# zju3dv/clean-pvnet

Hardware: AMD Instinct MI355X
Metric: images/sec RANSAC-vote (480x640, K=9, 512 hyp) (higher is better)
Workload: dtype f32; 1 GPU; BASELINE config 3 (cfg3): 480x640, K=9, 512 hypotheses, ~2% foreground, int64 mask, contiguous [B,H,W,K,2] f32 vertex; global batch 64 in contiguous shards of 64 images per GPU; ransac_voting_layer_v3 (+ one RCCL all_gather of [B,K,2] per step for N>1, see extra.exchange); steps cycle over 3 distinct device-resident batches; batch_per_gpu=64, global_batch=64, H=480, W=640, K=9, hn=512, parallelism=batch-sharded x1 (strong scaling: 64 images in total)

## Files before the change

### clean-pvnet_amd/csrc/compaction.hpp

```cpp
#pragma once

struct MaskArgs {
    const void *mask;
    const float *selection;
    int64_t sb, sh, sw;
    int es;
    int contig;
    int mode;
    int W, HW, T;
    int min_num, max_num, cap;
    uint64_t seed;
    int b0;
    int *tn_user;
    int *status;
    int fuse_sub;
    int want_draws;
    const float *seg;
    long long *mask_out;
    int64_t gb, gc, gh, gw;
    int C;
};

constexpr uint32_t kTileNzMask = 0xfffu;

enum { kElemF32 = 0, kElemF16 = 1, kElemBF16 = 2 };
template <int ET> struct Elem;
template <> struct Elem<kElemF32> { typedef float raw; };
template <> struct Elem<kElemF16> { typedef _Float16 raw; };
template <> struct Elem<kElemBF16> { typedef uint16_t raw; };

__device__ __forceinline__ float widen(float v) { return v; }
__device__ __forceinline__ float widen(_Float16 v) { return (float)v; }
__device__ __forceinline__ float widen(uint16_t v) { return __builtin_bit_cast(float, (uint32_t)v << 16); }

template <int ET>
__device__ __forceinline__ float2 widen_pair(uint32_t w)
{
    static_assert(ET != kElemF32, "2-byte elements only");
    if constexpr (ET == kElemF16)
        return make_float2((float)__builtin_bit_cast(_Float16, (uint16_t)w), (float)__builtin_bit_cast(_Float16, (uint16_t)(w >> 16)));
    else
        return make_float2(__builtin_bit_cast(float, w << 16), __builtin_bit_cast(float, w & 0xffff0000u));
}

template <int ES>
__device__ __forceinline__ uint64_t load_elem(const void *base, int64_t off)
{
    if (ES == 1) return ((const uint8_t *)base)[off];
    if (ES == 2) return ((const uint16_t *)base)[off];
    if (ES == 4) return ((const uint32_t *)base)[off];
    return ((const uint64_t *)base)[off];
}

template <int ST>
__device__ __forceinline__ int argmax_class(const MaskArgs &a, int b, int p)
{
    typedef typename Elem<ST>::raw raw_t;
    const int y = p / a.W;
    const int x = p - y * a.W;
    const raw_t *q = (const raw_t *)a.seg + (int64_t)b * a.gb + (int64_t)y * a.gh + (int64_t)x * a.gw;
    float best = widen(q[0]);
    int idx = 0;
    for (int c = 1; c < a.C; ++c) {
        const float v = widen(q[(int64_t)c * a.gc]);
        if (v > best || (v != v && best == best)) { best = v; idx = c; }
    }
    return idx;
}

template <int ES, int ST>
__device__ __forceinline__ int mask_weight(const MaskArgs &a, int b, int p)
{
    if (a.seg) {
        const int idx = argmax_class<ST>(a, b, p);
        if (a.mask_out) a.mask_out[(int64_t)b * a.HW + p] = idx;
        return a.mode == 0 ? (idx & 0xFF) : (idx == 1 ? 1 : 0);
    }
    int64_t off;
    if (a.contig) {
        off = (int64_t)b * a.sb + p;
    } else {
        int y = p / a.W;
        int x = p - y * a.W;
        off = (int64_t)b * a.sb + (int64_t)y * a.sh + (int64_t)x * a.sw;
    }
    uint64_t v = load_elem<ES>(a.mask, off);
    if (a.mode == 0) return (int)(v & 0xFF);
    return v == 1 ? 1 : 0;
}

__device__ __forceinline__ float selection_draw(const MaskArgs &a, int b, int p)
{
    if (a.selection) return a.selection[(int64_t)b * a.HW + p];
    return (float)(rng_u32(a.seed, 0u, (uint32_t)(a.b0 + b), (uint32_t)p) >> 8) * 0x1p-24f;
}

__device__ __forceinline__ float list_draw(const MaskArgs &a, int b, int i, int e, const unsigned short *__restrict__ lists ,
                                           const float *__restrict__ draws )
{
    if (draws) return draws[(size_t)i * kTile + e];
    return selection_draw(a, b, i * kTile + (int)lists[(size_t)i * kTile + e]);
}

__device__ __forceinline__ void scan_segments(int *seg)
{
    __syncthreads();
    if (threadIdx.x < 64) {
        const int lane = threadIdx.x;
        const int c = lane < kTileSteps * 4 ? seg[lane] : 0;
        const int inc = wave_incl_scan(c);
        if (lane < kTileSteps * 4) seg[lane] = inc - c;
        if (lane == kTileSteps * 4 - 1) seg[kTileSteps * 4] = inc;
    }
    __syncthreads();
}

template <int ES> struct RawElem;
template <> struct RawElem<1> { typedef uint8_t type; };
template <> struct RawElem<2> { typedef uint16_t type; };
template <> struct RawElem<4> { typedef uint32_t type; };
template <> struct RawElem<8> { typedef uint64_t type; };

template <int ES, bool AHEAD, int MODE , int ST = kElemF32 >
__global__ __launch_bounds__(kBlock) void k_tile_scan(MaskArgs a, uint32_t *__restrict__ tiles,
                                                      unsigned short *__restrict__ tile_list,
                                                      float *__restrict__ tile_draw, int total_tiles)
{
    typedef typename RawElem<ES>::type raw_t;
    __shared__ int seg2[2][kTileSteps * 4 + 1];
    __shared__ int red2[2][4];
    const int lane = lane_id(), wave = threadIdx.x >> 6;
    raw_t cur[AHEAD ? kTileSteps : 1] = {};
    int g = blockIdx.x;
    int b = g / a.T, t = g - b * a.T;
    const int step_b = (int)gridDim.x / a.T, step_t = (int)gridDim.x - step_b * a.T;
    [[maybe_unused]] auto load_tile = [&](raw_t (&dst)[AHEAD ? kTileSteps : 1], int bi, int ti) {
        const raw_t *src = (const raw_t *)a.mask + (int64_t)bi * a.sb + (int64_t)ti * kTile + threadIdx.x;
        if ((ti + 1) * kTile <= a.HW) {
#pragma unroll
            for (int s = 0; s < kTileSteps; ++s) dst[AHEAD ? s : 0] = src[s * kBlock];
        } else {
#pragma unroll
            for (int s = 0; s < kTileSteps; ++s)
                dst[AHEAD ? s : 0] = ti * kTile + s * kBlock + (int)threadIdx.x < a.HW ? src[s * kBlock] : (raw_t)0;
        }
    };
    if constexpr (AHEAD) if (g < total_tiles) load_tile(cur, b, t);
    for (int it = 0; g < total_tiles; ++it) {
        int *seg = seg2[it & 1], *red = red2[it & 1];
        raw_t nxt[AHEAD ? kTileSteps : 1] = {};
        const int gn = g + gridDim.x;
        int bn = b + step_b, tn = t + step_t;
        if (tn >= a.T) { tn -= a.T; ++bn; }
        if constexpr (AHEAD) if (gn < total_tiles) load_tile(nxt, bn, tn);
        unsigned long long m[kTileSteps];
        int pc[kTileSteps];
        int sum = 0;
#pragma unroll
        for (int s = 0; s < kTileSteps; ++s) {
            const int p = t * kTile + s * kBlock + threadIdx.x;
            int w = 0;
            if constexpr (AHEAD) {
                const uint64_t v = (uint64_t)cur[s];
                w = MODE == 0 ? (int)(v & 0xFF) : (v == 1 ? 1 : 0);
            } else if (p < a.HW) {
                w = mask_weight<ES, ST>(a, b, p);
            }
            m[s] = __ballot(w != 0);
            pc[s] = __popcll(m[s]);
            sum += w;
        }
        if (MODE == 0) sum = wave_total(sum);
        else sum = pc[0] + pc[1] + pc[2] + pc[3] + pc[4] + pc[5] + pc[6] + pc[7];
        if (lane == 0) {
#pragma unroll
            for (int s = 0; s < kTileSteps; ++s) seg[s * 4 + wave] = pc[s];
            red[wave] = sum;
        }
        scan_segments(seg);
        if (threadIdx.x == 0)
            tiles[b * a.T + t] = (uint32_t)seg[kTileSteps * 4] | ((uint32_t)(red[0] + red[1] + red[2] + red[3]) << 12);
        unsigned short *list = tile_list + ((size_t)b * a.T + t) * kTile;
        float *draw = tile_draw + ((size_t)b * a.T + t) * kTile;
        if (seg[kTileSteps * 4] != 0) {
#pragma unroll
            for (int s = 0; s < kTileSteps; ++s)
                if ((m[s] >> lane) & 1ull) {
                    const int r = seg[s * 4 + wave] + __popcll(m[s] & ((1ull << lane) - 1ull));
                    list[r] = (unsigned short)(s * kBlock + threadIdx.x);
                    if (a.want_draws) draw[r] = selection_draw(a, b, t * kTile + s * kBlock + threadIdx.x);
                }
        }
        if constexpr (AHEAD) {
#pragma unroll
            for (int s = 0; s < kTileSteps; ++s) cur[s] = nxt[s];
        }
        g = gn; b = bn; t = tn;
    }
}

typedef float f32x4 __attribute__((ext_vector_type(4)));
typedef long long i64x2 __attribute__((ext_vector_type(2)));
typedef uint32_t u32x2 __attribute__((ext_vector_type(2)));

template <int ST>
__device__ __forceinline__ f32x4 widen_logits4(u32x2 w)
{
    const float2 lo = widen_pair<ST>(w.x), hi = widen_pair<ST>(w.y);
    return f32x4{lo.x, lo.y, hi.x, hi.y};
}

template <bool WRITE_MASK, int ST = kElemF32>
__global__ __launch_bounds__(kBlock) void k_tile_scan_seg2(MaskArgs a, uint32_t *__restrict__ tiles,
                                                           unsigned short *__restrict__ tile_list,
                                                           float *__restrict__ tile_draw)
{
    typedef typename Elem<ST>::raw raw_t;
    __shared__ int seg[8];
    const int g = blockIdx.x;
    const int b = g / a.T, t = g - b * a.T;
    const int lane = lane_id(), wave = threadIdx.x >> 6;
    const raw_t *p0 = (const raw_t *)a.seg + (int64_t)b * a.gb + (int64_t)t * kTile + 4 * threadIdx.x;
    const raw_t *p1 = p0 + a.gc;
    constexpr int kHalf = kTile / 2;
    f32x4 v0[2], v1[2];
    if constexpr (ST == kElemF32) {
#pragma unroll
        for (int s = 0; s < 2; ++s) {
            const bool in = t * kTile + s * kHalf + 4 * (int)threadIdx.x < a.HW;
            v0[s] = in ? __builtin_nontemporal_load((const f32x4 *)(p0 + s * kHalf)) : f32x4{0.f, 0.f, 0.f, 0.f};
            v1[s] = in ? __builtin_nontemporal_load((const f32x4 *)(p1 + s * kHalf)) : f32x4{0.f, 0.f, 0.f, 0.f};
        }
    } else {
        u32x2 w0[2], w1[2];
#pragma unroll
        for (int s = 0; s < 2; ++s) {
            const bool in = t * kTile + s * kHalf + 4 * (int)threadIdx.x < a.HW;
            w0[s] = in ? __builtin_nontemporal_load((const u32x2 *)(p0 + s * kHalf)) : u32x2{0u, 0u};
            w1[s] = in ? __builtin_nontemporal_load((const u32x2 *)(p1 + s * kHalf)) : u32x2{0u, 0u};
        }
#pragma unroll
        for (int s = 0; s < 2; ++s) {
            v0[s] = widen_logits4<ST>(w0[s]);
            v1[s] = widen_logits4<ST>(w1[s]);
        }
    }
    unsigned m4[2];
    int excl[2];
#pragma unroll
    for (int s = 0; s < 2; ++s) {
        unsigned m = 0u;
#pragma unroll
        for (int j = 0; j < 4; ++j) {
            const float x0 = v0[s][j], x1 = v1[s][j];
            m |= ((x1 > x0) || (x1 != x1 && x0 == x0)) ? (1u << j) : 0u;
        }
        m4[s] = m;
        const int c = __popc(m);
        const int inc = wave_incl_scan(c);
        excl[s] = inc - c;
        if (lane == 63) seg[s * 4 + wave] = inc;
    }
    __syncthreads();
    int cnt[8];
#pragma unroll
    for (int i = 0; i < 8; ++i) cnt[i] = seg[i];
    int nz = 0, base[2] = {0, 0};
#pragma unroll
    for (int i = 0; i < 8; ++i) {
        if (i < wave) base[0] += cnt[i];
        if (i < 4 + wave) base[1] += cnt[i];
        nz += cnt[i];
    }
    if (threadIdx.x == 0) tiles[g] = (uint32_t)nz | ((uint32_t)nz << 12);
    if (WRITE_MASK && a.mask_out) {
        long long *mo = a.mask_out + (int64_t)b * a.HW + (int64_t)t * kTile + 4 * threadIdx.x;
#pragma unroll
        for (int s = 0; s < 2; ++s)
            if (t * kTile + s * kHalf + 4 * (int)threadIdx.x < a.HW) {
                __builtin_nontemporal_store(i64x2{(long long)(m4[s] & 1u), (long long)((m4[s] >> 1) & 1u)}, (i64x2 *)(mo + s * kHalf));
                __builtin_nontemporal_store(i64x2{(long long)((m4[s] >> 2) & 1u), (long long)((m4[s] >> 3) & 1u)}, (i64x2 *)(mo + s * kHalf + 2));
            }
    }
    if (nz == 0) return;
    unsigned short *list = tile_list + (size_t)g * kTile;
    float *draw = tile_draw + (size_t)g * kTile;
#pragma unroll
    for (int s = 0; s < 2; ++s) {
        int r = base[s] + excl[s];
#pragma unroll
        for (int j = 0; j < 4; ++j)
            if ((m4[s] >> j) & 1u) {
                const int off = s * kHalf + 4 * (int)threadIdx.x + j;
                list[r] = (unsigned short)off;
                if (a.want_draws) draw[r] = selection_draw(a, b, t * kTile + off);
                ++r;
            }
    }
}

__global__ __launch_bounds__(kBlock) void k_mask_from_lists(const uint32_t *__restrict__ tiles, const unsigned short *__restrict__ tile_list,
                                                            long long *__restrict__ mask_out, int T, int HW, int total_tiles)
{
    __shared__ unsigned bm[kTile / 32];
    uint32_t word = (int)blockIdx.x < total_tiles ? tiles[blockIdx.x] : 0u;
    for (int g = blockIdx.x; g < total_tiles; g += gridDim.x) {
        const int b = g / T, t = g - b * T;
        const int nz = (int)(word & kTileNzMask);
        if (g + (int)gridDim.x < total_tiles) word = tiles[g + gridDim.x];
        if (nz) {
            __syncthreads();
            if (threadIdx.x < kTile / 32) bm[threadIdx.x] = 0u;
            __syncthreads();
            const unsigned short *list = tile_list + (size_t)g * kTile;
            for (int e = threadIdx.x; e < nz; e += kBlock) {
                const unsigned off = list[e];
                atomicOr(&bm[off >> 5], 1u << (off & 31u));
            }
            __syncthreads();
        }
        long long *dst = mask_out + (int64_t)b * HW + (int64_t)t * kTile;
#pragma unroll
        for (int j = 0; j < kTile / (2 * kBlock); ++j) {
            const int px = (j * kBlock + (int)threadIdx.x) * 2;
            if (t * kTile + px >= HW) break;
            const unsigned w = nz ? bm[px >> 5] >> (px & 31) : 0u;
#ifdef PVV_MASK_PLAIN_STORE
            *(i64x2 *)(dst + px) = i64x2{(long long)(w & 1u), (long long)((w >> 1) & 1u)};
#else
            __builtin_nontemporal_store(i64x2{(long long)(w & 1u), (long long)((w >> 1) & 1u)}, (i64x2 *)(dst + px));
#endif
        }
    }
}

struct ImageTotals { long long fg; int total; int before; };

__device__ __forceinline__ ImageTotals image_totals(const uint32_t *__restrict__ tiles, int b, int T, int t,
                                                    long long *redl, int *red)
{
    long long fgs = 0;
    int before = 0, total = 0;
    for (int i = threadIdx.x; i < T; i += kBlock) {
        const uint32_t w = tiles[b * T + i];
        fgs += w >> 12;
        const int c = (int)(w & kTileNzMask);
        total += c;
        if (i < t) before += c;
    }
    fgs = wave_total(fgs);
    before = wave_total(before);
    total = wave_total(total);
    const int wave = threadIdx.x >> 6;
    __syncthreads();
    if (lane_id() == 0) { redl[wave] = fgs; red[wave] = before; red[4 + wave] = total; }
    __syncthreads();
    ImageTotals r;
    r.fg = redl[0] + redl[1] + redl[2] + redl[3];
    r.before = red[0] + red[1] + red[2] + red[3];
    r.total = red[4] + red[5] + red[6] + red[7];
    return r;
}

__device__ __forceinline__ int filter_tile_list(const MaskArgs &a, int b, int t, int nz, float prob,
                                                const unsigned short *__restrict__ img_lists, const float *__restrict__ img_draws ,
                                                unsigned short *out, int *seg)
{
    const int lane = lane_id(), wave = threadIdx.x >> 6;
    const unsigned short *list = img_lists + (size_t)t * kTile;
    unsigned long long m[kTileSteps];
    unsigned short off[kTileSteps];
#pragma unroll
    for (int s = 0; s < kTileSteps; ++s) {
        const int e = s * kBlock + threadIdx.x;
        bool f = false;
        off[s] = 0;
        if (e < nz) {
            off[s] = list[e];
            f = (img_draws ? img_draws[(size_t)t * kTile + e] : selection_draw(a, b, t * kTile + (int)off[s])) < prob;
        }
        m[s] = __ballot(f);
        if (lane == 0) seg[s * 4 + wave] = __popcll(m[s]);
    }
    scan_segments(seg);
#pragma unroll
    for (int s = 0; s < kTileSteps; ++s)
        if ((m[s] >> lane) & 1ull) out[seg[s * 4 + wave] + __popcll(m[s] & ((1ull << lane) - 1ull))] = off[s];
    return seg[kTileSteps * 4];
}

__global__ __launch_bounds__(kBlock) void k_tile_subsample(MaskArgs a, uint32_t *__restrict__ tiles,
                                                           unsigned short *__restrict__ tile_list,
                                                           const float *__restrict__ tile_draw)
{
    __shared__ long long redl[4];
    __shared__ int red[8];
    __shared__ int seg[kTileSteps * 4 + 1];
    __shared__ unsigned short keep[kTile];
    const int t = blockIdx.x, b = blockIdx.y;
    const uint32_t w = tiles[b * a.T + t];
    const int nz = (int)(w & kTileNzMask);
    if (nz == 0) return;
    const ImageTotals tot = image_totals(tiles, b, a.T, t, redl, red);
    if (tot.fg <= (long long)a.max_num) return;
    const float prob = (float)a.max_num / (float)tot.fg;
    unsigned short *list = tile_list + ((size_t)b * a.T + t) * kTile;
    const int n = filter_tile_list(a, b, t, nz, prob, tile_list + (size_t)b * a.T * kTile, tile_draw + (size_t)b * a.T * kTile, keep, seg);
    __syncthreads();
    for (int i = threadIdx.x; i < n; i += kBlock) list[i] = keep[i];
    if (threadIdx.x == 0) tiles[b * a.T + t] = (uint32_t)n | (w & ~kTileNzMask);
}

struct VertexArgs {
    const float *vertex;
    int64_t sb, sh, sw, sk, sc;
    int K;
    int vec2;
};

template <int VT> struct VertexRaw { typedef uint2 type; };
template <> struct VertexRaw<kElemF32> { typedef float2 type; };

template <int VT>
__device__ __forceinline__ typename VertexRaw<VT>::type load_vertex(const VertexArgs &v, int b, int y, int x, int vi)
{
    if constexpr (VT == kElemF32) {
        const float *src = v.vertex + (int64_t)b * v.sb + (int64_t)y * v.sh + (int64_t)x * v.sw + (int64_t)vi * v.sk;
        if (v.vec2) return *(const float2 *)src;
        return make_float2(src[0], src[v.sc]);
    } else {
        const uint16_t *src = (const uint16_t *)v.vertex + (int64_t)b * v.sb + (int64_t)y * v.sh + (int64_t)x * v.sw + (int64_t)vi * v.sk;
        if (v.vec2) return make_uint2(*(const uint32_t *)src, 0u);
        return make_uint2(src[0], src[v.sc]);
    }
}

template <int VT>
__device__ __forceinline__ float2 widen_vertex(const VertexArgs &v, typename VertexRaw<VT>::type r)
{
    if constexpr (VT == kElemF32) {
        return r;
    } else {
        typedef typename Elem<VT>::raw raw_t;
        if (v.vec2) return widen_pair<VT>(r.x);
        return make_float2(widen(__builtin_bit_cast(raw_t, (uint16_t)r.x)), widen(__builtin_bit_cast(raw_t, (uint16_t)r.y)));
    }
}

struct HypArgs {
    const int32_t *idxs;
    const int32_t *idxs2;
    int hn, hn_first;
    uint32_t stream, stream2;
    float2 *hyps;
    int *counts;
    int32_t *draws_out;
    int blocks;
    int *surv;
    int *lead;
    int *miss;
};

constexpr int kHypRejectTries = 1 << 12;
constexpr float kSurvMinProb = 1.f / 64.f;
constexpr int kSurvCap = 8192;

__device__ __forceinline__ int select_pixel(const int *prefix, int T, const unsigned short *__restrict__ lists , int t,
                                            size_t *entry = nullptr )
{
    int lo = 0, hi = T - 1;
    while (lo < hi) {
        const int mid = (lo + hi) >> 1;
        if (prefix[mid] > t) hi = mid; else lo = mid + 1;
    }
    const int r = t - (lo ? prefix[lo - 1] : 0);
    const size_t e = (size_t)lo * kTile + r;
    if (entry) *entry = e;
    return lo * kTile + (int)lists[e];
}

template <int VT>
__global__ __launch_bounds__(kBlock) void k_compact_hyp(MaskArgs a, VertexArgs v, HypArgs h,
                                                        const uint32_t *__restrict__ tiles,
                                                        const unsigned short *__restrict__ tile_list,
                                                        const float *__restrict__ tile_draw,
                                                        int *__restrict__ tn_out, float2 *__restrict__ coords,
                                                        float2 *__restrict__ dirs)
{
    extern __shared__ int s_prefix[];
    __shared__ long long redl[4];
    __shared__ int red[8];
    __shared__ int seg[kTileSteps * 4 + 1];
    __shared__ unsigned short list[kTile];
    const int b = blockIdx.y;
    const int lane = lane_id(), wave = threadIdx.x >> 6;
    const unsigned short *img_lists = tile_list + (size_t)b * a.T * kTile;
    const float *img_draws = a.want_draws ? tile_draw + (size_t)b * a.T * kTile : nullptr;

    if ((int)blockIdx.x < h.blocks) {
        const int j = blockIdx.x;
        long long fgs = 0;
        int carry = 0;
        for (int base = 0; base < a.T; base += kBlock) {
            const int i = base + threadIdx.x;
            const uint32_t w = i < a.T ? tiles[b * a.T + i] : 0u;
            fgs += w >> 12;
            const int inc = wave_incl_scan((int)(w & kTileNzMask));
            __syncthreads();
            if (lane == 63) red[wave] = inc;
            __syncthreads();
            int off = carry;
            for (int w2 = 0; w2 < wave; ++w2) off += red[w2];
            if (i < a.T) s_prefix[i] = inc + off;
            carry += red[0] + red[1] + red[2] + red[3];
        }
        fgs = wave_total(fgs);
        __syncthreads();
        if (lane == 0) redl[wave] = fgs;
        __syncthreads();
        const long long fg = redl[0] + redl[1] + redl[2] + redl[3];
        const int total = carry;
        int tn = total < a.cap ? total : a.cap;
        if (fg < (long long)a.min_num) tn = 0;
        const bool sub = a.fuse_sub && fg > (long long)a.max_num;
        const float prob = sub ? (float)a.max_num / (float)fg : 2.f;
        int nsurv = -1;
        if (sub && prob < kSurvMinProb) {
            int *sv = h.surv + (size_t)b * kSurvCap;
            nsurv = 0;
            for (int i = 0; i < a.T; ++i) {
                const int ni = s_prefix[i] - (i ? s_prefix[i - 1] : 0);
                for (int e0 = 0; e0 < ni; e0 += kBlock) {
                    const int e = e0 + threadIdx.x;
                    const bool keep = e < ni && list_draw(a, b, i, e, img_lists, img_draws) < prob;
                    const unsigned long long m = __ballot(keep);
                    __syncthreads();
                    if (lane == 0) red[wave] = __popcll(m);
                    __syncthreads();
                    int off = nsurv;
                    for (int w2 = 0; w2 < wave; ++w2) off += red[w2];
                    off += __popcll(m & ((1ull << lane) - 1ull));
                    if (keep && off < kSurvCap) sv[off] = i * kTile + (int)img_lists[(size_t)i * kTile + e];
                    nsurv += red[0] + red[1] + red[2] + red[3];
                }
            }
            __threadfence_block();
            __syncthreads();
            if (nsurv > kSurvCap) nsurv = -1;
            else if (nsurv < tn) tn = nsurv;
        }

        const int gid = j * kBlock + threadIdx.x;
        if (gid >= v.K * h.hn) return;
        const int vi = gid / h.hn, hi = gid - vi * h.hn;
        const size_t o = ((size_t)b * v.K + vi) * h.hn + hi;
        h.counts[o] = 0;
        if (h.miss) h.miss[o] = 0;
        if (h.lead && hi == 0) {
            int *lw = h.lead + ((size_t)b * v.K + vi) * 8 + 4;
            lw[0] = 0; lw[1] = 0; lw[2] = 0; lw[3] = 0;
        }
        if (tn <= 0) {
            h.hyps[o] = make_float2(0.f, 0.f);
            if (h.draws_out) { h.draws_out[2 * o] = -1; h.draws_out[2 * o + 1] = -1; }
            return;
        }
        const bool first = hi < h.hn_first;
        const int32_t *src = first ? h.idxs : h.idxs2;
        int p0, p1;
        if (src) {
            const int32_t *ip = first ? h.idxs + (((size_t)b * h.hn_first + hi) * v.K + vi) * 2
                                      : h.idxs2 + (((size_t)b * (h.hn - h.hn_first) + (hi - h.hn_first)) * v.K + vi) * 2;
            int t0 = ip[0], t1 = ip[1];
            t0 = t0 < 0 ? 0 : (t0 >= tn ? tn - 1 : t0);
            t1 = t1 < 0 ? 0 : (t1 >= tn ? tn - 1 : t1);
            p0 = select_pixel(s_prefix, a.T, img_lists, t0);
            p1 = select_pixel(s_prefix, a.T, img_lists, t1);
        } else {
            const uint32_t stream = first ? h.stream : h.stream2;
            const uint32_t c = (uint32_t)((first ? hi : hi - h.hn_first) * v.K + vi) * 2u;
            const uint32_t img = (uint32_t)(a.b0 + b);
            if (!sub) {
                p0 = select_pixel(s_prefix, a.T, img_lists, (int)(rng_u32(a.seed, stream, img, c) % (uint32_t)tn));
                p1 = select_pixel(s_prefix, a.T, img_lists, (int)(rng_u32(a.seed, stream, img, c + 1u) % (uint32_t)tn));
            } else if (nsurv >= 0) {
                const int *sv = h.surv + (size_t)b * kSurvCap;
                p0 = sv[rng_u32(a.seed, stream, img, c) % (uint32_t)tn];
                p1 = sv[rng_u32(a.seed, stream, img, c + 1u) % (uint32_t)tn];
            } else {
                p0 = p1 = -1;
                for (int tr = 0; tr < kHypRejectTries && (p0 < 0 || p1 < 0); ++tr) {
                    size_t e;
                    const uint32_t stry = stream + 16u + 4u * (uint32_t)tr;
                    if (p0 < 0) {
                        const int p = select_pixel(s_prefix, a.T, img_lists, (int)(rng_u32(a.seed, stry, img, c) % (uint32_t)total), &e);
                        if ((img_draws ? img_draws[e] : selection_draw(a, b, p)) < prob) p0 = p;
                    }
                    if (p1 < 0) {
                        const int p = select_pixel(s_prefix, a.T, img_lists, (int)(rng_u32(a.seed, stry, img, c + 1u) % (uint32_t)total), &e);
                        if ((img_draws ? img_draws[e] : selection_draw(a, b, p)) < prob) p1 = p;
                    }
                }
                if (p0 < 0 || p1 < 0) {
                    h.hyps[o] = make_float2(0.f, 0.f);
                    if (h.draws_out) { h.draws_out[2 * o] = p0; h.draws_out[2 * o + 1] = p1; }
                    return;
                }
            }
        }
        const int y0 = p0 / a.W, x0 = p0 - y0 * a.W, y1 = p1 / a.W, x1 = p1 - y1 * a.W;
        const typename VertexRaw<VT>::type r0 = load_vertex<VT>(v, b, y0, x0, vi), r1 = load_vertex<VT>(v, b, y1, x1, vi);
        const float2 d0 = widen_vertex<VT>(v, r0), d1 = widen_vertex<VT>(v, r1);
        h.hyps[o] = hypothesis_exact(d0.x, d0.y, (float)x0, (float)y0, d1.x, d1.y, (float)x1, (float)y1);
        if (h.draws_out) { h.draws_out[2 * o] = p0; h.draws_out[2 * o + 1] = p1; }
        return;
    }

    const int t = blockIdx.x - h.blocks;
    const int nz = (int)(tiles[b * a.T + t] & kTileNzMask);
    if (t != 0 && !(a.fuse_sub && t == a.T - 1) && nz == 0) return;
    const unsigned short *my_list = img_lists + (size_t)t * kTile;
    unsigned short mine[kTileSteps];
#pragma unroll
    for (int s = 0; s < kTileSteps; ++s) {
        const int e = s * kBlock + threadIdx.x;
        mine[s] = e < nz ? my_list[e] : (unsigned short)0;
    }
    const ImageTotals tot = image_totals(tiles, b, a.T, t, redl, red);
    if (tot.fg < (long long)a.min_num) {
        if (t == 0 && threadIdx.x == 0) {
            tn_out[b] = 0;
            if (a.tn_user) a.tn_user[b] = 0;
            if (a.status) a.status[b] = PVV_STATUS_SKIPPED;
        }
        return;
    }
    int before = tot.before, tile_n = nz;
    const bool sub = a.fuse_sub && tot.fg > (long long)a.max_num;
    if (sub) {
        const float prob = (float)a.max_num / (float)tot.fg;
        int cnt = 0;
        if (img_draws || a.T > kBlock) {
            for (int i = 0; i < t; ++i) {
                const int ni = (int)(tiles[b * a.T + i] & kTileNzMask);
                for (int e = threadIdx.x; e < ni; e += kBlock)
                    cnt += list_draw(a, b, i, e, img_lists, img_draws) < prob ? 1 : 0;
            }
        } else {
            const int ti = threadIdx.x;
            const int nzi = ti < t ? (int)(tiles[b * a.T + ti] & kTileNzMask) : 0;
            const int inc = wave_incl_scan((nzi + 7) >> 3);
            __syncthreads();
            if (lane == 63) red[wave] = inc;
            __syncthreads();
            int goff = 0;
            for (int w2 = 0; w2 < wave; ++w2) goff += red[w2];
            if (ti < a.T) s_prefix[ti] = inc + goff;
            list[ti] = (unsigned short)nzi;
            __syncthreads();
            const int groups = t ? s_prefix[t - 1] : 0;
            constexpr int kAhead = 4;
            int tile = 0;
            for (int g0 = threadIdx.x; g0 < groups; g0 += kAhead * kBlock) {
                uint4 ent[kAhead];
                int left[kAhead], pix0[kAhead];
#pragma unroll
                for (int u = 0; u < kAhead; ++u) {
                    const int g = g0 + u * kBlock;
                    left[u] = 0;
                    if (g < groups) {
                        while (s_prefix[tile] <= g) ++tile;
                        const int e0 = (g - (tile ? s_prefix[tile - 1] : 0)) * 8;
                        ent[u] = *(const uint4 *)(img_lists + (size_t)tile * kTile + e0);
                        left[u] = (int)list[tile] - e0;
                        pix0[u] = tile * kTile;
                    }
                }
#pragma unroll
                for (int u = 0; u < kAhead; ++u) {
                    const uint32_t wds[4] = {ent[u].x, ent[u].y, ent[u].z, ent[u].w};
#pragma unroll
                    for (int q = 0; q < 8; ++q)
                        if (q < left[u]) {
                            const int off = (int)((wds[q >> 1] >> (16 * (q & 1))) & 0xffffu);
                            cnt += selection_draw(a, b, pix0[u] + off) < prob ? 1 : 0;
                        }
                }
            }
        }
        before = block_sum(cnt, red);
        __syncthreads();
        tile_n = filter_tile_list(a, b, t, nz, prob, img_lists, img_draws, list, seg);
        __syncthreads();
        if (t == a.T - 1 && threadIdx.x == 0) {
            const int all = before + tile_n;
            tn_out[b] = all < a.cap ? all : a.cap;
            if (a.tn_user) a.tn_user[b] = tn_out[b];
            if (a.status) a.status[b] = PVV_STATUS_SUBSAMPLED | (all > a.cap ? PVV_STATUS_TRUNCATED : 0);
        }
    } else {
        if (t == 0 && threadIdx.x == 0) {
            tn_out[b] = tot.total < a.cap ? tot.total : a.cap;
            if (a.tn_user) a.tn_user[b] = tn_out[b];
            if (a.status) a.status[b] = (tot.fg > (long long)a.max_num ? PVV_STATUS_SUBSAMPLED : 0) |
                                        (tot.total > a.cap ? PVV_STATUS_TRUNCATED : 0);
        }
#pragma unroll
        for (int s = 0; s < kTileSteps; ++s) {
            const int e = s * kBlock + threadIdx.x;
            if (e < nz) list[e] = mine[s];
        }
        __syncthreads();
    }
    const int room = a.cap - before;
    const int n = tile_n < room ? tile_n : (room > 0 ? room : 0);
    constexpr int kKeys = 12;
    for (int li = threadIdx.x; li < n; li += kBlock) {
        const int p = t * kTile + list[li];
        const int y = p / a.W, x = p - y * a.W;
        coords[(size_t)b * a.cap + before + li] = make_float2((float)x, (float)y);
        float2 *drow = dirs + (size_t)b * v.K * a.cap + before + li;
        for (int v0 = 0; v0 < v.K; v0 += kKeys) {
            typename VertexRaw<VT>::type d[kKeys];
#pragma unroll
            for (int u = 0; u < kKeys; ++u)
                if (v0 + u < v.K) d[u] = load_vertex<VT>(v, b, y, x, v0 + u);
#pragma unroll
            for (int u = 0; u < kKeys; ++u)
                if (v0 + u < v.K) {
                    if constexpr (VT == kElemF32) drow[(size_t)(v0 + u) * a.cap] = d[u];
                    else drow[(size_t)(v0 + u) * a.cap] = widen_vertex<VT>(v, d[u]);
                }
        }
    }
}
```

### clean-pvnet_amd/csrc/count_bf16.hpp

```cpp
#pragma once

typedef __bf16 bf16x8 __attribute__((ext_vector_type(8)));
typedef float float16v __attribute__((ext_vector_type(16)));

#define kDdAlive __uint_as_float(0x2b8cbcceu)
constexpr int kBfPixPerWave = 128;
constexpr int kBfMaxHt = 16;

struct Bf16Consts {
    float beta;
    float eps_c;
    float eps0;
    float kappa;
    float beta2;
};

__device__ __forceinline__ void split3(float x, __bf16 (&p)[3])
{
    p[0] = (__bf16)x;
    float r = x - (float)p[0];
    p[1] = (__bf16)r;
    r = r - (float)p[1];
    p[2] = (__bf16)r;
}

__device__ __forceinline__ int stage_hypothesis(bf16x8 *sB, int *sCnt, int i, float2 hp, float2 org, int cnt_init = 0)
{
    __bf16 qx[3], qy[3];
    split3(hp.x - org.x, qx);
    split3(hp.y - org.y, qy);
    const __bf16 one = (__bf16)1.f, zero = (__bf16)0.f;
    const bf16x8 lo8 = {qx[0], qy[0], qx[1], qx[2], qx[0], qy[1], qy[2], qy[0]};
    const bf16x8 hi8 = {qx[0], qy[0], qx[1], qy[1], one, one, one, zero};
    sB[(i >> 5) * 64 + (i & 31)] = lo8;
    sB[(i >> 5) * 64 + 32 + (i & 31)] = hi8;
    sCnt[i] = cnt_init;
    return !(fabsf(hp.x) < 1e15f && fabsf(hp.y) < 1e15f);
}

#ifdef PVV_STAMPS
#define PVV_STAMP(i) do { if (dbg && threadIdx.x == 0 && (blockIdx.x == 0 || blockIdx.x == 97 || blockIdx.x == 401)) \
    dbg[((blockIdx.x == 0 ? 0 : (blockIdx.x == 97 ? 1 : 2)) * 16) + (i)] = wall_clock64(); } while (0)
enum { kCsTable = 0, kCsItemPrologue, kCsAOperands, kCsNextGroup, kCsLoop, kCsLoopWait, kCsFlush, kCsOther, kCensusPhases };
#define PVV_CENSUS_IN() long long cs_last = 0; __shared__ long long s_cs[16]; \
    do { if (threadIdx.x == 0) { for (int i_ = 0; i_ < 16; ++i_) s_cs[i_] = 0; s_cs[0] = wall_clock64(); \
    s_cs[2] = (long long)__builtin_amdgcn_s_getreg(63492) | ((long long)__builtin_amdgcn_s_getreg(63508) << 32); \
    cs_last = (long long)__builtin_readcyclecounter(); } } while (0)
#define PVV_CS(i) do { if (threadIdx.x == 0) { const long long t_ = (long long)__builtin_readcyclecounter(); s_cs[4 + (i)] += t_ - cs_last; cs_last = t_; } } while (0)
#define PVV_CS_RT_IN() long long cs_rt = 0; do { if (threadIdx.x == 0) cs_rt = wall_clock64(); } while (0)
#define PVV_CS_RT_OUT(tiles) do { if (threadIdx.x == 0) { s_cs[12] += wall_clock64() - cs_rt; s_cs[13] += (tiles); } } while (0)
#define PVV_CENSUS_OUT(n) do { if (dbg && threadIdx.x == 0) { s_cs[1] = wall_clock64(); s_cs[3] = (n); \
    for (int i_ = 0; i_ < 16; ++i_) dbg[64 + 16 * (size_t)blockIdx.x + i_] = s_cs[i_]; } } while (0)
#else
#define PVV_STAMP(i) do { } while (0)
#define PVV_CENSUS_IN() do { } while (0)
#define PVV_CS(i) do { } while (0)
#define PVV_CS_RT_IN() do { } while (0)
#define PVV_CS_RT_OUT(tiles) do { } while (0)
#define PVV_CENSUS_OUT(n) do { } while (0)
#endif

enum { kCountFull = 0, kCountFirst = 1, kCountFilter = 2 };

#ifndef PVV_STAGE_M
#define PVV_STAGE_M 8
#define PVV_STAGE_FIRST 0x22u
#endif
constexpr int kStageM = PVV_STAGE_M;
constexpr uint32_t kStageFirst = PVV_STAGE_FIRST;
constexpr uint32_t kStageFirstEighth = 0x02u;
constexpr uint32_t stage_rest_of(uint32_t first) { return ((1u << kStageM) - 1u) & ~first; }
constexpr int kStageMinChunks = 8;

struct StageArgs {
    const int *lead;
    int *any_staged;
    int *miss;
    int sub_tenth;
    const float2 *mean;
    int hstride;
#ifdef PVV_STAMPS
    long long *dbg;
#endif
};

__device__ __forceinline__ int stage_bound(int lstar, int tn, int sub_tenth)
{
    if (sub_tenth && lstar >= 0) lstar -= (tn + 9) / 10 + 2 + (tn >> 20);
    return lstar;
}

template <uint32_t MASK>
__device__ __forceinline__ int stage_chunks(int n)
{
    return (n / kStageM) * __builtin_popcount(MASK) + __popc(MASK & ((1u << (n % kStageM)) - 1u));
}
template <uint32_t MASK>
__device__ __forceinline__ int stage_chunk_at(int j)
{
    constexpr int m = __builtin_popcount(MASK);
    const int per = j / m;
    uint32_t t = MASK;
    for (int k = j - per * m; k > 0; --k) t &= t - 1u;
    return per * kStageM + __builtin_ctz(t);
}
template <uint32_t MASK>
__device__ __forceinline__ int stage_pixels(int tn, int nch, int PC)
{
    return stage_chunks<MASK>(nch) * PC - (((MASK >> ((nch - 1) % kStageM)) & 1u) ? nch * PC - tn : 0);
}

template <int MODE, uint32_t FIRST = kStageFirst>
__global__ __launch_bounds__(kBlock) __attribute__((amdgpu_waves_per_eu(5, 5))) void k_count_bf16(
    const float2 *__restrict__ coords , const float2 *__restrict__ dirs ,
    const float2 *__restrict__ hyps , int *__restrict__ counts ,
    const int *__restrict__ tn_arr, int B, int K, int hn, int cap, float thresh, Bf16Consts fc, int target_items,
    long long *__restrict__ dbg , StageArgs sa)
{
    PVV_STAMP(0);
    PVV_CENSUS_IN();
    int n_items_done = 0;
    __shared__ int chunk_end[kMaxBatchLds];
    __shared__ int s_htpi, s_gpi, s_chunks;
    __shared__ bf16x8 sB[kBfMaxHt * 64];
    __shared__ float4 sP[4 * kBfPixPerWave];
    __shared__ int sCnt[kBfMaxHt * 32];
    __shared__ float sRed[4];
    __shared__ unsigned long long s_small[kMaxBatchLds / 64];
    __shared__ int s_keep[8];
    constexpr bool STAGED = MODE != kCountFull;
    constexpr bool FILTER = MODE == kCountFilter;
    constexpr uint32_t REST = stage_rest_of(FIRST);
    const int lane = lane_id(), wave = wave_id();
    constexpr int PC = 4 * kBfPixPerWave;
    const int nt = (hn + 31) >> 5;
    const int hs = sa.hstride > 0 ? sa.hstride : hn;
    if constexpr (FILTER) if (*sa.any_staged == 0) return;

    if (wave == 0) {
        int carry = 0;
        [[maybe_unused]] bool any_staged = false;
        for (int b0 = 0; b0 < B; b0 += 64) {
            const int b = b0 + lane;
            int inc = b < B ? (tn_arr[b] + PC - 1) / PC : 0;
            if constexpr (STAGED) {
                const bool small = inc < kStageMinChunks;
                const unsigned long long sm = __ballot(small);
                any_staged |= sm != ~0ull;
                if (lane == 0) s_small[b0 >> 6] = sm;
                inc = small ? (MODE == kCountFirst ? inc : 0) : stage_chunks<MODE == kCountFirst ? FIRST : REST>(inc);
            }
            inc = wave_incl_scan(inc) + carry;
            if (b < B) chunk_end[b] = inc;
            carry = __builtin_amdgcn_readlane(inc, 63);
        }
        const long long chunks = (long long)carry * K;
        int htpi = min(nt, kBfMaxHt);
        int nhg = (nt + htpi - 1) / htpi;
        int gpi = nhg;
#ifndef PVV_GPI_FACTOR
#define PVV_GPI_FACTOR 3
#endif
        const long long gpi_target = (B > 8 && nhg >= 4) ? (long long)PVV_GPI_FACTOR * target_items : (long long)target_items;
        while (gpi > 1 && chunks * ((nhg + gpi - 1) / gpi) < gpi_target) gpi = (gpi + 1) >> 1;
        const int htpi_min = chunks < 128 ? 2 : 4;
        if (gpi == 1 && !FILTER)
            while (htpi > htpi_min && chunks * ((nt + htpi - 1) / htpi) < target_items) htpi = (htpi + 1) >> 1;
        if (lane == 0) { s_htpi = htpi; s_gpi = gpi; s_chunks = carry; }
        if constexpr (MODE == kCountFirst) if (blockIdx.x == 0 && lane == 0) *sa.any_staged = any_staged ? 1 : 0;
    }
    __syncthreads();
    PVV_STAMP(1);
    const int htpi = __builtin_amdgcn_readfirstlane(s_htpi);
    const int gpi = __builtin_amdgcn_readfirstlane(s_gpi);
    const int nhg = (nt + htpi - 1) / htpi;
    const int nruns = (nhg + gpi - 1) / gpi;
    const int per_chunk = K * nruns;
    const int total = __builtin_amdgcn_readfirstlane(s_chunks) * per_chunk;
    const int col = lane & 31, kslice = lane >> 5;
    PVV_STAMP(2);
    PVV_CS(kCsTable);

    const int nblk = (total <= target_items + (target_items >> 1) + (target_items >> 2) && (int)gridDim.x > target_items &&
                      (int)gridDim.x <= 3 * target_items) ? target_items : (int)gridDim.x;
    if ((int)blockIdx.x >= nblk) return;
    const int step_q = nblk / per_chunk, step_r = nblk - step_q * per_chunk;
    int gchunk = (int)blockIdx.x / per_chunk, rem = (int)blockIdx.x - gchunk * per_chunk;
    for (int item = blockIdx.x; item < total;
         item += nblk, gchunk += step_q + (rem + step_r >= per_chunk ? 1 : 0), rem += step_r - (rem + step_r >= per_chunk ? per_chunk : 0)) {
        int local;
        const int b = locate_item(chunk_end, B, gchunk, &local);
        int chunk = local;
        if constexpr (STAGED)
            if (!((s_small[b >> 6] >> (b & 63)) & 1ull)) chunk = stage_chunk_at<MODE == kCountFirst ? FIRST : REST>(local);
        const int vi = nruns == 1 ? rem : rem / nruns;
        const int run = rem - vi * nruns;
        const int bk = b * K + vi;
        const float2 *hyp_k = hyps + (size_t)bk * hs;
        const float2 *crd = coords + (size_t)b * cap;
        const float2 *dir_k = dirs + (size_t)bk * cap;
        const int pb = chunk * PC;
        const int g0 = run * gpi, g1 = min(nhg, g0 + gpi);

        __syncthreads();
        int tid = threadIdx.x;
        asm volatile("" : "+v"(tid));
        PVV_STAMP(3);
        PVV_CS(kCsOther);
        ++n_items_done;
        const int tn_v = tn_arr[b];
        int lead_p = -1, lead_r = 0;
        if constexpr (FILTER) {
            lead_p = sa.lead[(size_t)bk * 8 + (lane & 3)];
            lead_r = sa.lead[(size_t)bk * 8 + 4 + (lane & 3)];
        }
        const float2 org = crd[pb];
        float2 pc[2], pd[2];
#pragma unroll
        for (int q = 0; q < 2; ++q) {
            const int p = min(pb + tid + q * kBlock, cap - 1);
            pc[q] = crd[p];
            pd[q] = dir_k[p];
        }
        const int nht0 = min(nt, (g0 + 1) * htpi) - g0 * htpi;
        float2 hp0[2];
#pragma unroll
        for (int q = 0; q < 2; ++q) {
            const int i = tid + q * kBlock;
            const int h = (g0 * htpi + (i >> 5)) * 32 + (i & 31);
            hp0[q] = (i < nht0 * 32 && h < hn) ? hyp_k[h] : make_float2(0.f, 0.f);
        }
        int cnt0[2] = {0, 0};
        if constexpr (FILTER) {
#pragma unroll
            for (int q = 0; q < 2; ++q) {
                const int i = tid + q * kBlock;
                const int h = g0 * htpi * 32 + i;
                if (i < nht0 * 32 && h < hn) cnt0[q] = counts[(size_t)bk * hs + h];
            }
        }
        const int tn = __builtin_amdgcn_readfirstlane(tn_v);
        int R_rem = 0, lstar = 0, ns_g = 0;
        if constexpr (FILTER) {
            R_rem = stage_pixels<REST>(tn, (tn + PC - 1) / PC, PC);
            int full = lead_p >= 0 ? lead_p + lead_r : -1;
            full = max(full, PVV_DPP(full, full, 0xB1, 0xf, false));
            full = max(full, PVV_DPP(full, full, 0x4E, 0xf, false));
            lstar = stage_bound(__builtin_amdgcn_readfirstlane(full), tn, sa.sub_tenth);
        }
        auto stage_kept = [&](int g, const int (&cnt)[2], const float2 (&hp)[2]) -> int {
            bool keep[2];
            unsigned long long m[2];
#pragma unroll
            for (int q = 0; q < 2; ++q) {
                const int i = tid + q * kBlock;
                keep[q] = i < htpi * 32 && g * htpi * 32 + i < hn && cnt[q] + R_rem >= lstar;
                m[q] = __ballot(keep[q]);
                if (lane == 0) s_keep[q * 4 + wave] = __popcll(m[q]);
            }
            __syncthreads();
            int tot = 0, base[2] = {0, 0};
#pragma unroll
            for (int j = 0; j < 8; ++j) {
                const int v = s_keep[j];
                tot += v;
                if (j < wave) base[0] += v;
                if (j < 4 + wave) base[1] += v;
            }
            int f = 0;
#pragma unroll
            for (int q = 0; q < 2; ++q)
                if (keep[q])
                    f |= stage_hypothesis(sB, sCnt, base[q] + (int)__builtin_amdgcn_mbcnt_hi((unsigned)(m[q] >> 32), __builtin_amdgcn_mbcnt_lo((unsigned)m[q], 0u)), hp[q], org,
                                          (int)(tid + q * kBlock) << 16);
            const int pad = ((tot + 31) & ~31) - tot;
            if (tid < pad) stage_hypothesis(sB, sCnt, tot + tid, make_float2(0.f, 0.f), org, 0);
            ns_g = tot;
            return f;
        };

        float c1 = 0.f;
#pragma unroll
        for (int q = 0; q < 2; ++q) {
            const int pl = tid + q * kBlock, p = pb + pl;
            float4 rec = make_float4(__builtin_nanf(""), 0.f, 0.f, 0.f);
            if (p < tn) {
                const float2 c = pc[q], d = pd[q];
                const float cx = c.x - org.x, cy = c.y - org.y;
                c1 = fmaxf(c1, fabsf(cx) + fabsf(cy));
                const float dd = d.x * d.x + d.y * d.y;
                if (dd >= kDdAlive && dd < INFINITY) {
                    const float rinv = __builtin_amdgcn_rsqf(dd);
                    rec = make_float4(d.x * rinv, d.y * rinv, cx, cy);
                }
            }
            sP[pl] = rec;
        }
        c1 = wave_max(c1);
        if (lane == 0) sRed[wave] = c1;
        int far = 0;
        if constexpr (FILTER) {
            far = stage_kept(g0, cnt0, hp0);
        } else {
#pragma unroll
            for (int q = 0; q < 2; ++q) {
                const int i = tid + q * kBlock;
                if (i < nht0 * 32) far |= stage_hypothesis(sB, sCnt, i, hp0[q], org);
            }
        }
        far = __syncthreads_or(far);
        PVV_STAMP(4);
        PVV_CS(kCsItemPrologue);
        const float C1 = fmaxf(fmaxf(sRed[0], sRed[1]), fmaxf(sRed[2], sRed[3]));
        const float eps = fc.eps0 + fc.eps_c * C1;
        const float epsw = __builtin_fmaf(fc.beta * 1.02f, C1, eps);

        const int ntile_c = (min(tn - pb, PC) + 15) >> 4;
        const int ntile_w = (ntile_c - wave + 3) >> 2;

        bf16x8 A[8];
        if (ntile_w > 0) {
            const int form = (lane >> 4) & 1, prow = lane & 15;
#pragma unroll
            for (int i = 0; i < 4; ++i) {
                const int j = kslice * 4 + i;
                const float4 rec = sP[(j * 4 + wave) * 16 + prow];
                const bool dead = rec.x != rec.x;
                float rx = form ? -fc.kappa * rec.y : rec.x;
                float ry = form ? fc.kappa * rec.x : rec.y;
                float rz = -(rec.z * rx + rec.w * ry);
                if (dead) { rx = 0.f; ry = 0.f; rz = form ? 0.f : -1e30f; }
                __bf16 vx[3], vy[3], cv[3];
                split3(rx, vx);
                split3(ry, vy);
                split3(rz, cv);
                const __bf16 zero = (__bf16)0.f;
                const bf16x8 lo8 = {vx[0], vy[0], vx[0], vx[0], vx[1], vy[0], vy[0], vy[1]};
                const bf16x8 hi8 = {vx[2], vy[2], vx[1], vy[1], cv[0], cv[1], cv[2], zero};
                uint4 x = __builtin_bit_cast(uint4, lo8), y = __builtin_bit_cast(uint4, hi8);
                {
                    const auto r0 = __builtin_amdgcn_permlane32_swap(x.x, y.x, false, false);
                    const auto r1 = __builtin_amdgcn_permlane32_swap(x.y, y.y, false, false);
                    const auto r2 = __builtin_amdgcn_permlane32_swap(x.z, y.z, false, false);
                    const auto r3 = __builtin_amdgcn_permlane32_swap(x.w, y.w, false, false);
                    x = make_uint4(r0[0], r1[0], r2[0], r3[0]);
                    y = make_uint4(r0[1], r1[1], r2[1], r3[1]);
                }
                A[i] = __builtin_bit_cast(bf16x8, x);
                A[4 + i] = __builtin_bit_cast(bf16x8, y);
            }
        }
        PVV_STAMP(5);
        PVV_CS(kCsAOperands);
        const int ebase = kslice * 4;
        const float16v zero16 = {0.f, 0.f, 0.f, 0.f, 0.f, 0.f, 0.f, 0.f, 0.f, 0.f, 0.f, 0.f, 0.f, 0.f, 0.f, 0.f};

        for (int g = g0; g < g1; ++g) {
            const int ht0 = g * htpi;
            if (g > g0) {
                far = 0;
                if constexpr (FILTER) {
                    int cnt[2] = {0, 0};
                    float2 hp[2] = {make_float2(0.f, 0.f), make_float2(0.f, 0.f)};
#pragma unroll
                    for (int q = 0; q < 2; ++q) {
                        const int i = threadIdx.x + q * kBlock;
                        const int h = ht0 * 32 + i;
                        if (i < htpi * 32 && h < hn) { cnt[q] = counts[(size_t)bk * hs + h]; hp[q] = hyp_k[h]; }
                    }
                    far = stage_kept(g, cnt, hp);
                } else {
                    const int nhtg = min(nt, ht0 + htpi) - ht0;
                    for (int i = threadIdx.x; i < nhtg * 32; i += kBlock) {
                        const int h = (ht0 + (i >> 5)) * 32 + (i & 31);
                        far |= stage_hypothesis(sB, sCnt, i, h < hn ? hyp_k[h] : make_float2(0.f, 0.f), org);
                    }
                }
                far = __syncthreads_or(far);
            }
            const int nht = FILTER ? (ns_g + 31) >> 5 : min(nt, ht0 + htpi) - ht0;
            const int nslot = FILTER ? ns_g : min(hn - ht0 * 32, nht * 32);
            PVV_STAMP(6);
            PVV_CS(kCsNextGroup);
            PVV_CS_RT_IN();

            if (__builtin_expect(far, 0)) {
                for (int ht = 0; ht < nht; ++ht) {
                    const int slot = ht * 32 + col;
                    if (slot >= nslot) continue;
                    const float2 hp = hyp_k[ht0 * 32 + (FILTER ? sCnt[slot] >> 16 : slot)];
                    int inl = 0;
                    for (int p = pb + wave * 2 + kslice; p < min(tn, pb + PC); p += 8) {
                        const float2 c = crd[p], d = dir_k[p];
                        inl += vote_exact(c.x, c.y, hp.x, hp.y, d.x, d.y, thresh) ? 1 : 0;
                    }
                    if (inl) atomicAdd(&sCnt[ht * 32 + col], inl);
                }
            } else if (ntile_w > 0) {
                for (int ht = 0; ht < nht; ++ht) {
                    const bf16x8 Bop = sB[ht * 64 + lane];
                    unsigned flagged = 0u;
                    const unsigned q01 = __builtin_bit_cast(uint4, Bop).x;
                    const float wband = __builtin_fmaf(fc.beta * 1.02f,
                                                       fabsf(__uint_as_float(q01 << 16)) + fabsf(__uint_as_float(q01 & 0xffff0000u)),
                                                       epsw);
                    unsigned qs[2] = {0u, 0u};
                    unsigned mb[2] = {0u, 0u};
                    int ntw = ntile_w;
                    asm volatile("" : "+s"(ntw));
#pragma unroll
                    for (int j = 0; j < 8; ++j) {
                        if (j < ntw) {
                            const float16v acc = __builtin_amdgcn_mfma_f32_32x32x16_bf16(A[j], Bop, zero16, 0, 0, 0);
                            float tmin = INFINITY;
                            float t[8];
#pragma unroll
                            for (int e = 0; e < 8; ++e) {
                                t[e] = acc[e] - fabsf(acc[8 + e]);
                                qs[j >> 2] = __builtin_amdgcn_alignbit(qs[j >> 2], __float_as_uint(t[e]), 31);
                                tmin = fminf(tmin, fabsf(t[e]));
                            }
                            if (__builtin_expect(__ballot(tmin <= wband) != 0, 0)) {
                                unsigned out_of_band = 0u;
#pragma unroll
                                for (int e = 0; e < 8; ++e)
                                    out_of_band = __builtin_amdgcn_alignbit(
                                        out_of_band, __float_as_uint(eps - __builtin_fmaf(-fc.beta, acc[e], fabsf(t[e]))), 31);
                                mb[j >> 2] |= (~out_of_band & 0xffu) << (8 * (j & 3));
                                flagged |= 1u << j;
                            }
                        }
                    }
                    int inl = 8 * ntile_w - __popc(qs[0]) - __popc(qs[1]);
                    if (__builtin_expect(flagged != 0u, 0) && __any((mb[0] | mb[1]) != 0u)) {
                        const int slot = ht * 32 + col;
                        const float2 hp = slot < nslot ? hyp_k[ht0 * 32 + (FILTER ? sCnt[slot] >> 16 : slot)] : make_float2(0.f, 0.f);
                        do {
                            const int j = __builtin_ctz(flagged);
                            flagged &= flagged - 1;
                            const unsigned m = mb[j >> 2] >> (8 * (j & 3));
                            if (!__any((m & 0xffu) != 0u)) continue;
                            const int after = min(ntile_w - (j & 4), 4) - 1 - (j & 3);
                            const unsigned sgn = qs[j >> 2] >> (8 * after);
#pragma unroll
                            for (int e = 0; e < 8; ++e) {
                                const bool marked = (m >> (7 - e)) & 1u;
                                if (!__any(marked)) continue;
                                const int prow = (j * 4 + wave) * 16 + ebase + (e & 3) + 8 * (e >> 2);
                                const int p = pb + prow;
                                const int fast = ((sgn >> (7 - e)) & 1u) ? 0 : 1;
                                const float4 rec = sP[prow];
                                const float dx = hp.x - (rec.z + org.x), dy = hp.y - (rec.w + org.y);
                                const float a2 = __builtin_fmaf(dx, rec.x, dy * rec.y);
                                const float b2 = __builtin_fmaf(dx, -fc.kappa * rec.y, dy * (fc.kappa * rec.x));
                                const float t2 = a2 - fabsf(b2);
                                int decided = t2 > 0.f ? 1 : 0;
                                const bool unsure = marked && (!(__builtin_fmaf(-fc.beta2, a2, fabsf(t2)) > fc.eps0) || rec.x != rec.x);
                                if (__any(unsure)) {
                                    int exact = 0;
                                    if (unsure && p < tn) {
                                        const float2 c = crd[p], d = dir_k[p];
                                        exact = vote_exact(c.x, c.y, hp.x, hp.y, d.x, d.y, thresh) ? 1 : 0;
                                    }
                                    if (unsure) decided = exact;
                                }
                                if (p >= tn) decided = 0;
                                if (marked) inl += decided - fast;
                            }
                        } while (flagged != 0u);
                    }
                    if (inl) atomicAdd(&sCnt[ht * 32 + col], inl);
                }
            }
            PVV_STAMP(7);
            PVV_CS(kCsLoop);
            PVV_CS_RT_OUT(nht * ntile_w);
            __syncthreads();
            PVV_CS(kCsLoopWait);
            for (int i = threadIdx.x; i < nslot; i += kBlock) {
                const int v = sCnt[i];
                const int c = FILTER ? v & 0xffff : v;
                if (c != 0) atomicAdd(&counts[(size_t)bk * hs + ht0 * 32 + (FILTER ? v >> 16 : i)], c);
            }
            PVV_STAMP(8);
            PVV_CS(kCsFlush);
        }
    }
    PVV_STAMP(9);
    PVV_CS(kCsOther);
    PVV_CENSUS_OUT(n_items_done);
    (void)n_items_done;
}
```

### clean-pvnet_amd/csrc/count_filter_runs.hpp

```cpp
#pragma once

constexpr int kRunMaxChunks = 64;
constexpr int kRunSlots = kBfMaxHt * 32;

#ifdef PVV_STAMPS
#define PVV_FS_DECL() __shared__ long long s_fs[16]; long long fs_last = 0; \
    if (threadIdx.x == 0) { for (int i_ = 0; i_ < 16; ++i_) s_fs[i_] = 0; s_fs[14] = wall_clock64(); fs_last = (long long)__builtin_readcyclecounter(); }
#define PVV_FS(i) do { if (threadIdx.x == 0) { const long long t_ = (long long)__builtin_readcyclecounter(); s_fs[i] += t_ - fs_last; fs_last = t_; } } while (0)
#define PVV_FS_ADD(i, n) do { if (threadIdx.x == 0) s_fs[i] += (n); } while (0)
#define PVV_FS_OUT() do { if (sa.dbg && threadIdx.x == 0) { s_fs[15] = wall_clock64(); \
    for (int i_ = 0; i_ < 16; ++i_) sa.dbg[(size_t)blockIdx.x * 16 + i_] = s_fs[i_]; } } while (0)
#else
#define PVV_FS_DECL() do { } while (0)
#define PVV_FS(i) do { } while (0)
#define PVV_FS_ADD(i, n) do { } while (0)
#define PVV_FS_OUT() do { } while (0)
#endif

__device__ __forceinline__ int stage_hypothesis_b(bf16x8 *sB, int i, float2 hp, float2 org)
{
    __bf16 qx[3], qy[3];
    split3(hp.x - org.x, qx);
    split3(hp.y - org.y, qy);
    const __bf16 one = (__bf16)1.f, zero = (__bf16)0.f;
    const bf16x8 lo8 = {qx[0], qy[0], qx[1], qx[2], qx[0], qy[1], qy[2], qy[0]};
    const bf16x8 hi8 = {qx[0], qy[0], qx[1], qy[1], one, one, one, zero};
    sB[(i >> 5) * 64 + (i & 31)] = lo8;
    sB[(i >> 5) * 64 + 32 + (i & 31)] = hi8;
    return !(fabsf(hp.x) < 1e15f && fabsf(hp.y) < 1e15f);
}

template <uint32_t FIRST>
__global__ __launch_bounds__(kBlock) __attribute__((amdgpu_waves_per_eu(5, 5))) void k_count_filter_runs(
    const float2 *__restrict__ coords , const float2 *__restrict__ dirs ,
    const float2 *__restrict__ hyps , int *__restrict__ counts ,
    const int *__restrict__ tn_arr, int B, int K, int hn, int cap, float thresh, Bf16Consts fc, int target_items, int run_r, StageArgs sa)
{
    extern __shared__ int run_end[];
    __shared__ int s_R, s_runs, s_gpi;
    __shared__ bf16x8 sB[kBfMaxHt * 64];
    __shared__ float4 sP[4 * kBfPixPerWave];
    __shared__ int sCnt[kRunSlots];
    __shared__ unsigned short sPrev[kRunSlots];
    __shared__ float sRed[4];
    __shared__ int s_keep[8];
    __shared__ unsigned short s_order[64];
    const int lane = lane_id(), wave = wave_id();
    constexpr int PC = 4 * kBfPixPerWave;
    constexpr int GH = kRunSlots;
    constexpr uint32_t REST = stage_rest_of(FIRST);
    const int nhg = (hn + GH - 1) / GH;
    const int hs = sa.hstride > 0 ? sa.hstride : hn;
    if (*sa.any_staged == 0) return;
    PVV_FS_DECL();

    if (wave == 0) {
        int total = 0;
        for (int b0 = 0; b0 < B; b0 += 64) {
            const int b = b0 + lane;
            int n = 0;
            if (b < B) {
                const int nch = (tn_arr[b] + PC - 1) / PC;
                n = nch < kStageMinChunks ? 0 : stage_chunks<REST>(nch);
                run_end[b] = n;
            }
            total += wave_total(n);
        }
        const int gpi = sa.sub_tenth ? 1 : nhg;
        const int ngr = (nhg + gpi - 1) / gpi;
        int R = run_r;
        if (R <= 0) {
            const long long r = target_items > 0 ? ((long long)total * K * ngr) / target_items : 1;
            R = (int)(r < 1 ? 1 : r);
        }
        R = R < 1 ? 1 : (R > kRunMaxChunks ? kRunMaxChunks : R);
        int carry = 0;
        for (int b0 = 0; b0 < B; b0 += 64) {
            const int b = b0 + lane;
            const int n = b < B ? run_end[b] : 0;
            int inc = (n + R - 1) / R;
            inc = wave_incl_scan(inc) + carry;
            if (b < B) run_end[b] = inc;
            carry = __builtin_amdgcn_readlane(inc, 63);
        }
        if (lane == 0) { s_R = R; s_runs = carry; s_gpi = gpi; }
    }
    __syncthreads();
    PVV_FS(0);
    const int R = __builtin_amdgcn_readfirstlane(s_R);
    const int gpi = __builtin_amdgcn_readfirstlane(s_gpi), ngr = (nhg + gpi - 1) / gpi;
    const int per_run = K * ngr;
    const int total = __builtin_amdgcn_readfirstlane(s_runs) * per_run;
    const int col = lane & 31, kslice = lane >> 5;
    const int ebase = kslice * 4;
    const float16v zero16 = {0.f, 0.f, 0.f, 0.f, 0.f, 0.f, 0.f, 0.f, 0.f, 0.f, 0.f, 0.f, 0.f, 0.f, 0.f, 0.f};

    for (int item = blockIdx.x; item < total; item += gridDim.x) {
        const int grun = item / per_run, rem_i = item - grun * per_run;
        const int vi = ngr == 1 ? rem_i : rem_i / ngr, gr = rem_i - vi * ngr;
        const int g_begin = gr * gpi, g_end = min(nhg, g_begin + gpi);
        int r_img;
        const int b = locate_item(run_end, B, grun, &r_img);
        const int bk = b * K + vi;
        const float2 *hyp_k = hyps + (size_t)bk * hs;
        const float2 *crd = coords + (size_t)b * cap;
        const float2 *dir_k = dirs + (size_t)bk * cap;
        int *cnt_k = counts + (size_t)bk * hs;
        int *miss_k = sa.miss + (size_t)bk * hs;
        const int tn = __builtin_amdgcn_readfirstlane(tn_arr[b]);
        const int nch = (tn + PC - 1) / PC;
        const int nrest = stage_chunks<REST>(nch);
        const int nruns = (nrest + R - 1) / R;
        const int j0 = (int)((long long)r_img * nrest / nruns), j1 = (int)((long long)(r_img + 1) * nrest / nruns);
        const int R_rem = stage_pixels<REST>(tn, nch, PC);
        int lstar;
        {
            const int lead_p = sa.lead[(size_t)bk * 8 + (lane & 3)], lead_r = sa.lead[(size_t)bk * 8 + 4 + (lane & 3)];
            int full = lead_p >= 0 ? lead_p + lead_r : -1;
            full = max(full, PVV_DPP(full, full, 0xB1, 0xf, false));
            full = max(full, PVV_DPP(full, full, 0x4E, 0xf, false));
            lstar = stage_bound(__builtin_amdgcn_readfirstlane(full), tn, sa.sub_tenth);
        }

        const bool prox = sa.mean != nullptr && nrest <= 64;
        if (prox && wave == 0) {
            float key = INFINITY;
            if (lane < nrest) {
                const int pm = min(stage_chunk_at<REST>(lane) * PC + PC / 2, tn - 1);
                key = fabsf(crd[pm].y - sa.mean[bk].y);
                if (!(key == key)) key = INFINITY;
            }
            int rank = 0;
            for (int o = 0; o < nrest; ++o) {
                const float ko = __int_as_float(__builtin_amdgcn_readlane(__float_as_int(key), o));
                rank += (ko < key || (ko == key && o < lane)) ? 1 : 0;
            }
            if (lane < nrest) s_order[rank] = (unsigned short)lane;
        }
        const int nmine = prox ? (nrest - r_img + nruns - 1) / nruns : j1 - j0;
        PVV_FS(1);
        PVV_FS_ADD(10, 1);
        for (int g = g_begin; g < g_end;) {
            const int gp0 = g;
            int ns = 0;
            __syncthreads();
            for (; g < g_end && g - gp0 < 63; ++g) {
                bool keep[2];
                int slack[2];
                unsigned long long m[2];
#pragma unroll
                for (int q = 0; q < 2; ++q) {
                    const int i = (int)threadIdx.x + q * kBlock, h = g * GH + i;
                    const int c = h < hn ? cnt_k[h] : 0;
                    const int m0 = h < hn ? miss_k[h] : 0;
                    slack[q] = c + R_rem - lstar - m0;
                    keep[q] = h < hn && slack[q] >= 0;
                    m[q] = __ballot(keep[q]);
                    if (lane == 0) s_keep[q * 4 + wave] = __popcll(m[q]);
                }
                __syncthreads();
                int tot = 0, base[2] = {0, 0};
#pragma unroll
                for (int j = 0; j < 8; ++j) {
                    const int v = s_keep[j];
                    tot += v;
                    if (j < wave) base[0] += v;
                    if (j < 4 + wave) base[1] += v;
                }
                const bool fits = ns + tot <= kRunSlots;
                if (fits) {
#pragma unroll
                    for (int q = 0; q < 2; ++q)
                        if (keep[q]) {
                            const int slot = ns + base[q] + (int)__builtin_amdgcn_mbcnt_hi((unsigned)(m[q] >> 32), __builtin_amdgcn_mbcnt_lo((unsigned)m[q], 0u));
                            sCnt[slot] = ((g - gp0) * GH + (int)threadIdx.x + q * kBlock) << 16;
                            sPrev[slot] = 0;
                        }
                    ns += tot;
                }
                __syncthreads();
                if (!fits) break;
            }
            PVV_FS(2);
            if (ns == 0) continue;

            for (int it = 0; it < nmine && ns > 0; ++it) {
                const int j = prox ? __builtin_amdgcn_readfirstlane((int)s_order[r_img + it * nruns]) : j0 + it;
                const int chunk = stage_chunk_at<REST>(j);
                const int pb = chunk * PC;
                int tid = threadIdx.x;
                asm volatile("" : "+v"(tid));
                const float2 org = crd[pb];
                float2 pc[2], pd[2];
#pragma unroll
                for (int q = 0; q < 2; ++q) {
                    const int p = min(pb + tid + q * kBlock, cap - 1);
                    pc[q] = crd[p];
                    pd[q] = dir_k[p];
                }
                const int ns_pad = (ns + 31) & ~31;
                float2 hp[2];
#pragma unroll
                for (int q = 0; q < 2; ++q) {
                    const int i = tid + q * kBlock;
                    hp[q] = i < ns ? hyp_k[gp0 * GH + (int)((unsigned)sCnt[i] >> 16)] : make_float2(0.f, 0.f);
                }
                float c1 = 0.f;
#pragma unroll
                for (int q = 0; q < 2; ++q) {
                    const int pl = tid + q * kBlock, p = pb + pl;
                    float4 rec = make_float4(__builtin_nanf(""), 0.f, 0.f, 0.f);
                    if (p < tn) {
                        const float2 c = pc[q], d = pd[q];
                        const float cx = c.x - org.x, cy = c.y - org.y;
                        c1 = fmaxf(c1, fabsf(cx) + fabsf(cy));
                        const float dd = d.x * d.x + d.y * d.y;
                        if (dd >= kDdAlive && dd < INFINITY) {
                            const float rinv = __builtin_amdgcn_rsqf(dd);
                            rec = make_float4(d.x * rinv, d.y * rinv, cx, cy);
                        }
                    }
                    sP[pl] = rec;
                }
                c1 = wave_max(c1);
                if (lane == 0) sRed[wave] = c1;
                int far = 0;
#pragma unroll
                for (int q = 0; q < 2; ++q) {
                    const int i = tid + q * kBlock;
                    if (i < ns_pad) far |= stage_hypothesis_b(sB, i, hp[q], org);
                }
                far = __syncthreads_or(far);
                PVV_FS(3);
                PVV_FS_ADD(11, 1);
                PVV_FS_ADD(12, ns);
                const float C1 = fmaxf(fmaxf(sRed[0], sRed[1]), fmaxf(sRed[2], sRed[3]));
                const float eps = fc.eps0 + fc.eps_c * C1;
                const float epsw = __builtin_fmaf(fc.beta * 1.02f, C1, eps);
                const int npx = min(tn - pb, PC);
                const int ntile_c = (npx + 15) >> 4;
                const int ntile_w = (ntile_c - wave + 3) >> 2;
                bf16x8 A[8];
                if (ntile_w > 0) {
                    const int form = (lane >> 4) & 1, prow = lane & 15;
#pragma unroll
                    for (int i = 0; i < 4; ++i) {
                        const int jt = kslice * 4 + i;
                        const float4 rec = sP[(jt * 4 + wave) * 16 + prow];
                        const bool dead = rec.x != rec.x;
                        float rx = form ? -fc.kappa * rec.y : rec.x;
                        float ry = form ? fc.kappa * rec.x : rec.y;
                        float rz = -(rec.z * rx + rec.w * ry);
                        if (dead) { rx = 0.f; ry = 0.f; rz = form ? 0.f : -1e30f; }
                        __bf16 vx[3], vy[3], cv[3];
                        split3(rx, vx);
                        split3(ry, vy);
                        split3(rz, cv);
                        const __bf16 zero = (__bf16)0.f;
                        const bf16x8 lo8 = {vx[0], vy[0], vx[0], vx[0], vx[1], vy[0], vy[0], vy[1]};
                        const bf16x8 hi8 = {vx[2], vy[2], vx[1], vy[1], cv[0], cv[1], cv[2], zero};
                        uint4 x = __builtin_bit_cast(uint4, lo8), y = __builtin_bit_cast(uint4, hi8);
                        {
                            const auto r0 = __builtin_amdgcn_permlane32_swap(x.x, y.x, false, false);
                            const auto r1 = __builtin_amdgcn_permlane32_swap(x.y, y.y, false, false);
                            const auto r2 = __builtin_amdgcn_permlane32_swap(x.z, y.z, false, false);
                            const auto r3 = __builtin_amdgcn_permlane32_swap(x.w, y.w, false, false);
                            x = make_uint4(r0[0], r1[0], r2[0], r3[0]);
                            y = make_uint4(r0[1], r1[1], r2[1], r3[1]);
                        }
                        A[i] = __builtin_bit_cast(bf16x8, x);
                        A[4 + i] = __builtin_bit_cast(bf16x8, y);
                    }
                }
                const int nht = ns_pad >> 5, nslot = ns;
                const float2 *hyp_p = hyp_k + gp0 * GH;
                PVV_FS(4);
                PVV_FS_ADD(13, nht * ntile_w);

                if (__builtin_expect(far, 0)) {
                    for (int ht = 0; ht < nht; ++ht) {
                        const int slot = ht * 32 + col;
                        if (slot >= nslot) continue;
                        const float2 hq = hyp_p[(unsigned)sCnt[slot] >> 16];
                        int inl = 0;
                        for (int p = pb + wave * 2 + kslice; p < min(tn, pb + PC); p += 8) {
                            const float2 c = crd[p], d = dir_k[p];
                            inl += vote_exact(c.x, c.y, hq.x, hq.y, d.x, d.y, thresh) ? 1 : 0;
                        }
                        if (inl) atomicAdd(&sCnt[slot], inl);
                    }
                } else if (ntile_w > 0) {
                    for (int ht = 0; ht < nht; ++ht) {
                        const bf16x8 Bop = sB[ht * 64 + lane];
                        unsigned flagged = 0u;
                        const unsigned q01 = __builtin_bit_cast(uint4, Bop).x;
                        const float wband = __builtin_fmaf(fc.beta * 1.02f,
                                                           fabsf(__uint_as_float(q01 << 16)) + fabsf(__uint_as_float(q01 & 0xffff0000u)),
                                                           epsw);
                        unsigned qs[2] = {0u, 0u};
                        unsigned mb[2] = {0u, 0u};
                        int ntw = ntile_w;
                        asm volatile("" : "+s"(ntw));
#pragma unroll
                        for (int jt = 0; jt < 8; ++jt) {
                            if (jt < ntw) {
                                const float16v acc = __builtin_amdgcn_mfma_f32_32x32x16_bf16(A[jt], Bop, zero16, 0, 0, 0);
                                float tmin = INFINITY;
                                float t[8];
#pragma unroll
                                for (int e = 0; e < 8; ++e) {
                                    t[e] = acc[e] - fabsf(acc[8 + e]);
                                    qs[jt >> 2] = __builtin_amdgcn_alignbit(qs[jt >> 2], __float_as_uint(t[e]), 31);
                                    tmin = fminf(tmin, fabsf(t[e]));
                                }
                                if (__builtin_expect(__ballot(tmin <= wband) != 0, 0)) {
                                    unsigned out_of_band = 0u;
#pragma unroll
                                    for (int e = 0; e < 8; ++e)
                                        out_of_band = __builtin_amdgcn_alignbit(
                                            out_of_band, __float_as_uint(eps - __builtin_fmaf(-fc.beta, acc[e], fabsf(t[e]))), 31);
                                    mb[jt >> 2] |= (~out_of_band & 0xffu) << (8 * (jt & 3));
                                    flagged |= 1u << jt;
                                }
                            }
                        }
                        int inl = 8 * ntile_w - __popc(qs[0]) - __popc(qs[1]);
                        if (__builtin_expect(flagged != 0u, 0) && __any((mb[0] | mb[1]) != 0u)) {
                            const int slot = ht * 32 + col;
                            const float2 hq = slot < nslot ? hyp_p[(unsigned)sCnt[slot] >> 16] : make_float2(0.f, 0.f);
                            do {
                                const int jt = __builtin_ctz(flagged);
                                flagged &= flagged - 1;
                                const unsigned m = mb[jt >> 2] >> (8 * (jt & 3));
                                if (!__any((m & 0xffu) != 0u)) continue;
                                const int after = min(ntile_w - (jt & 4), 4) - 1 - (jt & 3);
                                const unsigned sgn = qs[jt >> 2] >> (8 * after);
#pragma unroll
                                for (int e = 0; e < 8; ++e) {
                                    const bool marked = (m >> (7 - e)) & 1u;
                                    if (!__any(marked)) continue;
                                    const int prow = (jt * 4 + wave) * 16 + ebase + (e & 3) + 8 * (e >> 2);
                                    const int p = pb + prow;
                                    const int fast = ((sgn >> (7 - e)) & 1u) ? 0 : 1;
                                    const float4 rec = sP[prow];
                                    const float dx = hq.x - (rec.z + org.x), dy = hq.y - (rec.w + org.y);
                                    const float a2 = __builtin_fmaf(dx, rec.x, dy * rec.y);
                                    const float b2 = __builtin_fmaf(dx, -fc.kappa * rec.y, dy * (fc.kappa * rec.x));
                                    const float t2 = a2 - fabsf(b2);
                                    int decided = t2 > 0.f ? 1 : 0;
                                    const bool unsure = marked && (!(__builtin_fmaf(-fc.beta2, a2, fabsf(t2)) > fc.eps0) || rec.x != rec.x);
                                    if (__any(unsure)) {
                                        int exact = 0;
                                        if (unsure && p < tn) {
                                            const float2 c = crd[p], d = dir_k[p];
                                            exact = vote_exact(c.x, c.y, hq.x, hq.y, d.x, d.y, thresh) ? 1 : 0;
                                        }
                                        if (unsure) decided = exact;
                                    }
                                    if (p >= tn) decided = 0;
                                    if (marked) inl += decided - fast;
                                }
                            } while (flagged != 0u);
                        }
                        if (inl) atomicAdd(&sCnt[ht * 32 + col], inl);
                    }
                }
                PVV_FS(5);
                __syncthreads();
                PVV_FS(6);
                {
                    const bool last = it + 1 >= nmine;
                    bool keep[2];
                    int w[2];
                    unsigned long long m[2];
#pragma unroll
                    for (int q = 0; q < 2; ++q) {
                        const int i = (int)threadIdx.x + q * kBlock;
                        keep[q] = false;
                        w[q] = 0;
                        if (i < ns) {
                            w[q] = sCnt[i];
                            const int c = w[q] & 0xffff, h = gp0 * GH + (int)((unsigned)w[q] >> 16);
                            const int dmiss = npx - (c - (int)sPrev[i]);
                            sPrev[i] = (unsigned short)c;
                            if (last) {
                                if (dmiss) atomicAdd(&miss_k[h], dmiss);
                            } else {
                                const int seen = atomicAdd(&miss_k[h], dmiss) + dmiss;
                                keep[q] = cnt_k[h] + R_rem - lstar - seen >= 0;
                            }
                        }
                        m[q] = __ballot(keep[q]);
                        if (lane == 0) s_keep[q * 4 + wave] = __popcll(m[q]);
                    }
                    if (!last) {
                        __syncthreads();
                        int tot = 0, base[2] = {0, 0};
#pragma unroll
                        for (int jj = 0; jj < 8; ++jj) {
                            const int v = s_keep[jj];
                            tot += v;
                            if (jj < wave) base[0] += v;
                            if (jj < 4 + wave) base[1] += v;
                        }
                        if (((tot + 31) >> 5) < ((ns + 31) >> 5)) {
#pragma unroll
                            for (int q = 0; q < 2; ++q)
                                if (keep[q]) {
                                    const int slot = base[q] + (int)__builtin_amdgcn_mbcnt_hi((unsigned)(m[q] >> 32), __builtin_amdgcn_mbcnt_lo((unsigned)m[q], 0u));
                                    sCnt[slot] = w[q];
                                    sPrev[slot] = (unsigned short)(w[q] & 0xffff);
                                }
                            ns = tot;
                        }
                        __syncthreads();
                    }
                }
                PVV_FS(7);
            }
            __syncthreads();
            for (int i = threadIdx.x; i < ns; i += kBlock) {
                const int v = sCnt[i];
                if (v & 0xffff) atomicAdd(&cnt_k[gp0 * GH + (int)((unsigned)v >> 16)], v & 0xffff);
            }
            PVV_FS(8);
        }
    }
    PVV_FS(9);
    PVV_FS_OUT();
}
```

### clean-pvnet_amd/csrc/count_prune.hpp

```cpp
#pragma once

struct LeadArgs {
    const int *tn_arr;
    const float2 *coords;
    const float2 *dirs;
    const float2 *hyps;
    const int *counts;
    int *lead;
    const int *any_staged;
    int K, hn, cap;
    int hstride;
    float kappa, beta, eps;
    int nsplit;
};

constexpr int kLead = 2;

template <uint32_t FIRST>
__global__ __launch_bounds__(kBlock) void k_lead(LeadArgs a)
{
    constexpr uint32_t REST = stage_rest_of(FIRST);
    __shared__ int s_cnt[4], s_idx[4], s_sum[4][4];
    const int vi = blockIdx.x / a.nsplit, split = blockIdx.x - vi * a.nsplit, b = blockIdx.y, bk = b * a.K + vi;
    const int lane = lane_id(), wave = threadIdx.x >> 6;
    constexpr int PC = 4 * kBfPixPerWave;
    if (*a.any_staged == 0) return;
    const int tn = a.tn_arr[b];
    const int nch = (tn + PC - 1) / PC;
    if (tn <= 0 || nch < kStageMinChunks) return;
    constexpr int kTrip = 10;
    const int rem_px = stage_pixels<REST>(tn, nch, PC);
    const int per = (rem_px + a.nsplit - 1) / a.nsplit;
    const int r1 = min(rem_px, (split + 1) * per);
    const float2 *crd = a.coords + (size_t)b * a.cap;
    const float2 *dir = a.dirs + (size_t)bk * a.cap;
    float2 cc[kTrip], dd_[kTrip];
    auto load_trip = [&](int r0) {
#pragma unroll
        for (int u = 0; u < kTrip; ++u) {
            const int r = r0 + u * kBlock;
            cc[u] = dd_[u] = make_float2(0.f, 0.f);
            if (r < r1) {
                const int p = stage_chunk_at<REST>(r / PC) * PC + (r & (PC - 1));
                cc[u] = crd[p];
                dd_[u] = dir[p];
            }
        }
    };
    int r0 = split * per + threadIdx.x;
    load_trip(r0);
    const int *cp = a.counts + (size_t)bk * a.hstride;
    int best = -1, besth = 0x7fffffff;
    for (int h = threadIdx.x; h < a.hn; h += kBlock) {
        const int c = cp[h];
        if (c > best) { best = c; besth = h; }
    }
    wave_argmax_first(best, besth);
    if (lane == 0) { s_cnt[wave] = best; s_idx[wave] = besth; }
    __syncthreads();
    int lc[4], li[4];
#pragma unroll
    for (int w = 0; w < 4; ++w) { lc[w] = s_cnt[w]; li[w] = s_idx[w]; }
#pragma unroll
    for (int i = 0; i < kLead; ++i)
#pragma unroll
        for (int j = 3; j > i; --j)
            if (lc[j] > lc[j - 1] || (lc[j] == lc[j - 1] && li[j] < li[j - 1])) {
                const int tc = lc[j], ti = li[j];
                lc[j] = lc[j - 1]; li[j] = li[j - 1]; lc[j - 1] = tc; li[j - 1] = ti;
            }
    float2 ld[kLead];
#pragma unroll
    for (int w = 0; w < kLead; ++w) ld[w] = lc[w] >= 0 ? a.hyps[(size_t)bk * a.hstride + li[w]] : make_float2(0.f, 0.f);
    if (split == 0 && threadIdx.x < 4) {
        int v = -1;
#pragma unroll
        for (int w = 0; w < kLead; ++w) if ((int)threadIdx.x == w) v = lc[w];
        a.lead[(size_t)bk * 8 + threadIdx.x] = v;
    }
    int inl[kLead];
    bool lnear[kLead];
#pragma unroll
    for (int w = 0; w < kLead; ++w) { inl[w] = 0; lnear[w] = lc[w] >= 0 && fabsf(ld[w].x) < 1e15f && fabsf(ld[w].y) < 1e15f; }
    for (;;) {
#pragma unroll
        for (int u = 0; u < kTrip; ++u) {
            const float dd = dd_[u].x * dd_[u].x + dd_[u].y * dd_[u].y;
            const bool ok = dd > 4e-12f && dd < INFINITY;
            const float r = __builtin_amdgcn_rsqf(dd);
            const float nx = dd_[u].x * r, ny = dd_[u].y * r;
            const float bx = -a.kappa * ny, by = a.kappa * nx;
#pragma unroll
            for (int w = 0; w < kLead; ++w) {
                const float dx = ld[w].x - cc[u].x, dy = ld[w].y - cc[u].y;
                const float av = __builtin_fmaf(dx, nx, dy * ny);
                const float bv = __builtin_fmaf(dx, bx, dy * by);
                const float t = av - fabsf(bv);
                inl[w] += (ok && lnear[w] && t > 0.f && __builtin_fmaf(-a.beta, av, t) > a.eps) ? 1 : 0;
            }
        }
        r0 += kTrip * kBlock;
        if (r0 - (int)threadIdx.x >= r1) break;
        load_trip(r0);
    }
#pragma unroll
    for (int w = 0; w < kLead; ++w) {
        const int s = wave_total(inl[w]);
        if (lane == 0) s_sum[wave][w] = s;
    }
    __syncthreads();
    if ((int)threadIdx.x < kLead) {
        const int s = s_sum[0][threadIdx.x] + s_sum[1][threadIdx.x] + s_sum[2][threadIdx.x] + s_sum[3][threadIdx.x];
        if (s) atomicAdd(&a.lead[(size_t)bk * 8 + 4 + threadIdx.x], s);
    }
}
```

### clean-pvnet_amd/csrc/covariance.hpp

```cpp
#pragma once

__global__ __launch_bounds__(kBlock) void k_covariance(
    const int *__restrict__ tn_arr, const float2 *__restrict__ hyps, const int *__restrict__ counts,
    const float2 *__restrict__ mean, float *__restrict__ cov ,
    float2 *__restrict__ hyp_out , int *__restrict__ counts_out,
    float *__restrict__ weights , int K, int hn, int hstride ,
    int hoff )
{
    __shared__ int redi[4];
    __shared__ double redd[4];
    const int vi = blockIdx.x, b = blockIdx.y;
    const int bk = b * K + vi;
    const int tn = tn_arr[b];
    const float2 m = mean[bk];
    const float2 *hp = hyps + (size_t)bk * hstride + hoff;
    const int *cp = counts + (size_t)bk * hstride + hoff;
    if (hyp_out || counts_out)
        for (int h = threadIdx.x; h < hn; h += kBlock) {
            if (hyp_out) hyp_out[(size_t)bk * hn + h] = tn > 0 ? hp[h] : make_float2(0.f, 0.f);
            if (counts_out) counts_out[(size_t)bk * hn + h] = tn > 0 ? cp[h] : 0;
        }
    double sxx = 0, sxy = 0, syy = 0, sw = 0;
    if (tn <= 0) {
        if (threadIdx.x == 0) {
            double dx = (double)(0.f - m.x), dy = (double)(0.f - m.y);
            sxx = dx * dx * hn; sxy = dx * dy * hn; syy = dy * dy * hn; sw = (double)hn;
        }
    } else {
        int mx = 0;
        for (int h = threadIdx.x; h < hn; h += kBlock) mx = max(mx, cp[h]);
        mx = wave_max(mx);
        __syncthreads();
        if (lane_id() == 0) redi[threadIdx.x >> 6] = mx;
        __syncthreads();
        mx = max(max(redi[0], redi[1]), max(redi[2], redi[3]));
        const float ftn = (float)tn;
        const float thr = (float)mx / ftn - 0.1f;
        for (int h = threadIdx.x; h < hn; h += kBlock) {
            float r = (float)cp[h] / ftn;
            if (r < thr) r = 0.f;
            float2 q = hp[h];
            double dx = (double)(q.x - m.x), dy = (double)(q.y - m.y);
            sxx += (double)r * dx * dx; sxy += (double)r * dx * dy; syy += (double)r * dy * dy;
            sw += (double)r;
        }
    }
    sxx = block_sum(sxx, redd); sxy = block_sum(sxy, redd);
    syy = block_sum(syy, redd); sw = block_sum(sw, redd);
    if (threadIdx.x == 0) {
        double den = sw + 1e-3;
        float *c = cov + (size_t)bk * 4;
        c[0] = (float)(sxx / den); c[1] = (float)(sxy / den);
        c[2] = (float)(sxy / den); c[3] = (float)(syy / den);
        if (weights) {
            const double a = (double)c[0], b = (double)c[1], d = (double)c[3];
            double wxx = 0.0, wxy = 0.0, wyy = 0.0;
            const double det = a * d - b * b;
            if (!(c[0] < 1e-6f) && a == a && b == b && d == d && det > 0.0 && a > 0.0) {
                const double s = sqrt(det), t = sqrt(a + d + 2.0 * s);
                const double q = t / ((a + s) * (d + s) - b * b);
                wxx = q * (d + s); wxy = -q * b; wyy = q * (a + s);
            }
            float *w = weights + (size_t)bk * 3;
            w[0] = (float)wxx; w[1] = (float)wxy; w[2] = (float)wyy;
        }
    }
}
```

### clean-pvnet_amd/csrc/pvnet_vote.hip

```cpp
#include <hip/hip_runtime.h>

#include <algorithm>
#include <cmath>
#include <cstdio>
#include <cstdlib>
#include <cstring>
#include <mutex>
#include <type_traits>

#include "pvnet_vote.h"

#pragma clang fp contract(off)

#define PVV_EXPORT extern "C" __attribute__((visibility("default")))

namespace {

constexpr int kBlock = 256;
constexpr int kTileSteps = 8;
constexpr int kTile = kBlock * kTileSteps;
constexpr int kFuseSubTiles = 160;
constexpr int kMaxTiles = 16000;
constexpr int kPixPerWave = 64;

thread_local char g_err[512] = "";

int fail(int code, const char *msg)
{
    snprintf(g_err, sizeof(g_err), "%s", msg);
    return code;
}

int check_launch(const char *what)
{
    hipError_t e = hipGetLastError();
    if (e != hipSuccess) {
        snprintf(g_err, sizeof(g_err), "%s: %s", what, hipGetErrorString(e));
        return (int)e;
    }
    return PVV_OK;
}

#include "vote_common.hpp"
#include "compaction.hpp"
#include "count_exact.hpp"
#include "count_bf16.hpp"
#include "count_filter_runs.hpp"
#include "count_prune.hpp"
#include "refit.hpp"
#include "covariance.hpp"
#include "legacy_kernels.hpp"

size_t align_up(size_t x) { return (x + 255) & ~(size_t)255; }

struct Layout {
    int T;
    size_t tiles, tile_list, tile_draw, tn, surv, coords, dirs, hyps, counts, sums, total;
    size_t lead;
    size_t ratio;
    size_t miss;
};

bool use_bf16_count(const pvv_problem *p);
bool may_stage(const pvv_problem *p);

bool fuse_sub_shape(const pvv_problem *p, int T)
{
    return T <= kFuseSubTiles && (long long)p->max_num * 16 >= (long long)p->H * p->W;
}

bool may_store_draws(const pvv_problem *p, int T)
{
    const long long max_weight = std::max(255ll, (long long)p->seg_classes - 1);
    if ((long long)p->max_num >= max_weight * p->H * p->W) return false;
    return !((p->flags & PVV_FLAG_DEVICE_RNG) && fuse_sub_shape(p, T));
}

size_t lead_set_words(const pvv_problem *p) { return (size_t)p->B * p->K * 8 + 1; }

Layout make_layout(const pvv_problem *p)
{
    Layout L;
    const size_t HW = (size_t)p->H * p->W;
    L.T = (int)((HW + kTile - 1) / kTile);
    size_t off = 0;
    auto take = [&](size_t bytes) { size_t o = off; off = align_up(off + bytes); return o; };
    L.tiles = take(sizeof(uint32_t) * (size_t)p->B * L.T);
    L.tile_list = take(sizeof(unsigned short) * (size_t)p->B * L.T * kTile);
    L.tile_draw = may_store_draws(p, L.T) ? take(sizeof(float) * (size_t)p->B * L.T * kTile) : 0;
    L.tn = take(sizeof(int) * (size_t)p->B);
    L.surv = take(sizeof(int) * (size_t)p->B * kSurvCap);
    L.coords = take(sizeof(float2) * (size_t)p->B * p->cap);
    L.dirs = take(sizeof(float2) * (size_t)p->B * p->K * p->cap);
    L.hyps = take(sizeof(float2) * (size_t)p->B * p->K * p->hn);
    L.counts = take(sizeof(int) * (size_t)p->B * p->K * p->hn);
    L.sums = take(sizeof(double) * (size_t)p->B * p->K * kRefitSplitMax * 5);
    L.ratio = take(sizeof(float) * (size_t)p->B * p->K);
    L.lead = may_stage(p) ? take(sizeof(int) * 2 * lead_set_words(p)) : 0;
    L.miss = may_stage(p) ? take(sizeof(int) * (size_t)p->B * p->K * p->hn) : 0;
    L.total = off;
    return L;
}

int validate(const pvv_problem *p)
{
    if (!p) return fail(PVV_E_ARG, "problem is NULL");
    if (p->B <= 0 || p->H <= 0 || p->W <= 0 || p->K <= 0 || p->hn <= 0)
        return fail(PVV_E_ARG, "B, H, W, K, hn must be positive");
    if (p->B > kMaxBatchLds) return fail(PVV_E_ARG, "B > 1024: split the batch");
    if (((long long)p->H * p->W + kTile - 1) / kTile > kMaxTiles) return fail(PVV_E_ARG, "H*W too large (more than 16000 tiles of 2048 pixels)");
    if ((long long)p->K * p->hn >= (1ll << 23)) return fail(PVV_E_ARG, "K*hn must be < 2^23");
    if (p->count_kernel < PVV_COUNT_AUTO || p->count_kernel > PVV_COUNT_STAGED_ESTIMATE) return fail(PVV_E_ARG, "unknown count_kernel");
    if (p->flags & ~(PVV_FLAG_DEVICE_RNG | PVV_FLAG_VERTEX_F16 | PVV_FLAG_VERTEX_BF16 | PVV_FLAG_SEG_F16 | PVV_FLAG_SEG_BF16))
        return fail(PVV_E_ARG, "unknown bits in flags");
    if ((p->flags & PVV_FLAG_VERTEX_F16) && (p->flags & PVV_FLAG_VERTEX_BF16))
        return fail(PVV_E_ARG, "flags: PVV_FLAG_VERTEX_F16 and PVV_FLAG_VERTEX_BF16 are exclusive");
    if ((p->flags & PVV_FLAG_SEG_F16) && (p->flags & PVV_FLAG_SEG_BF16))
        return fail(PVV_E_ARG, "flags: PVV_FLAG_SEG_F16 and PVV_FLAG_SEG_BF16 are exclusive");
    if (p->mask_elem_size != 1 && p->mask_elem_size != 2 && p->mask_elem_size != 4 &&
        p->mask_elem_size != 8)
        return fail(PVV_E_ARG, "mask_elem_size must be 1, 2, 4 or 8");
    if (p->cap <= 0 || (long long)p->cap > (long long)p->H * p->W)
        return fail(PVV_E_ARG, "cap must be in [1, H*W]");
    if ((long long)p->B * p->K * p->hn >= (1ll << 31) || (long long)p->B * p->K * p->cap >= (1ll << 40))
        return fail(PVV_E_ARG, "problem too large for one call");
    if (p->singular_policy < PVV_SINGULAR_REFERENCE || p->singular_policy > PVV_SINGULAR_IMAGE_ZERO)
        return fail(PVV_E_ARG, "unknown singular_policy");
    return PVV_OK;
}

int num_cus()
{
    static int cus[64] = {0};
    int dev = 0;
    if (hipGetDevice(&dev) != hipSuccess || dev < 0 || dev >= 64) return 256;
    if (!cus[dev]) {
        hipDeviceProp_t prop;
        int n = 0;
        if (hipGetDeviceProperties(&prop, dev) == hipSuccess) n = prop.multiProcessorCount;
        cus[dev] = n > 0 ? n : 256;
    }
    return cus[dev];
}

int launch_count(const CountArgs &a, hipStream_t st)
{
    const int grid = num_cus() * 8;
    if (a.hn <= 64)
        hipLaunchKernelGGL(k_count_inliers<1>, dim3(grid), dim3(kBlock), 0, st, a);
    else if (a.hn <= 128)
        hipLaunchKernelGGL(k_count_inliers<2>, dim3(grid), dim3(kBlock), 0, st, a);
    else if (a.hn <= 256)
        hipLaunchKernelGGL(k_count_inliers<4>, dim3(grid), dim3(kBlock), 0, st, a);
    else
        hipLaunchKernelGGL(k_count_inliers<8>, dim3(grid), dim3(kBlock), 0, st, a);
    return check_launch("k_count_inliers");
}

bool use_bf16_count(const pvv_problem *p)
{
    return p->count_kernel != PVV_COUNT_EXACT && p->inlier_thresh >= 0.5f && p->inlier_thresh <= 0.99995f &&
           p->H <= 16384 && p->W <= 16384;
}

constexpr double kStageMinWork = 2e10;
constexpr double kStageProxyFg = 0.02;
bool may_stage(const pvv_problem *p)
{
    if (!use_bf16_count(p) || p->count_kernel == PVV_COUNT_FULL) return false;
    if (p->count_kernel == PVV_COUNT_STAGED || p->count_kernel == PVV_COUNT_STAGED_ESTIMATE) return true;
    const double rows = std::min((double)p->H * p->W, (double)p->cap);
    return p->hn >= 128 && p->cap >= kStageMinChunks * 4 * kBfPixPerWave &&
           (double)p->B * p->K * p->hn * rows >= kStageMinWork * kStageProxyFg;
}
double stage_proxy_work(const pvv_problem *p) { return (double)p->B * p->K * p->hn * p->H * p->W; }

struct StageHint {
    float *ratio = nullptr;
    int n = 0;
    int shape[5] = {0, 0, 0, 0, 0};
    bool tried = false;
};
StageHint g_hint[64];
std::mutex g_hint_mu;

int stream_device(hipStream_t st)
{
    int dev = -1;
    if (st) {
        hipDevice_t d;
        if (hipStreamGetDevice(st, &d) == hipSuccess) dev = (int)d; else (void)hipGetLastError();
    }
    if (dev < 0 && hipGetDevice(&dev) != hipSuccess) { (void)hipGetLastError(); return -1; }
    return dev >= 0 && dev < 64 ? dev : -1;
}

StageHint *stage_hint_locked(hipStream_t st, bool allocate)
{
    const int dev = stream_device(st);
    if (dev < 0) return nullptr;
    StageHint *g = &g_hint[dev];
    if (!g->tried && allocate) {
        hipStreamCaptureStatus cs = hipStreamCaptureStatusNone;
        if (hipStreamIsCapturing(st, &cs) != hipSuccess) { (void)hipGetLastError(); return nullptr; }
        if (cs != hipStreamCaptureStatusNone) return nullptr;
        g->tried = true;
        void *q = nullptr;
        if (hipHostMalloc(&q, sizeof(float) * 2 * kMaxBatchLds, hipHostMallocDefault) != hipSuccess) { (void)hipGetLastError(); q = nullptr; }
        g->ratio = (float *)q;
        if (g->ratio) for (int i = 0; i < 2 * kMaxBatchLds; ++i) g->ratio[i] = -2.f;
    }
    return g->ratio ? g : nullptr;
}

bool hint_same_shape(const StageHint *g, const pvv_problem *p, bool any_hn = false)
{
    return g->shape[1] == p->H && g->shape[2] == p->W && g->shape[3] == p->K && (any_hn || g->shape[4] == p->hn);
}

float *stage_hint_claim(const pvv_problem *p, hipStream_t st)
{
    std::lock_guard<std::mutex> lock(g_hint_mu);
    StageHint *g = stage_hint_locked(st, true);
    if (!g) return nullptr;
    const int shape[5] = {p->B, p->H, p->W, p->K, p->hn};
    if (!hint_same_shape(g, p)) {
        for (int i = 0; i < p->B; ++i) g->ratio[i] = -2.f;
    } else {
        for (int i = g->n; i < p->B; ++i) g->ratio[i] = -2.f;
    }
    memcpy(g->shape, shape, sizeof(shape));
    g->n = p->B;
    return g->ratio;
}

float stage_hint_mean(const pvv_problem *p, hipStream_t st, float *max_tn = nullptr, double *sum_tn = nullptr, bool any_hn = false)
{
    if (max_tn) *max_tn = -1.f;
    if (sum_tn) *sum_tn = -1.0;
    std::lock_guard<std::mutex> lock(g_hint_mu);
    StageHint *g = stage_hint_locked(st, false);
    if (!g || g->n <= 0) return -1.f;
    if (p && !hint_same_shape(g, p, any_hn)) return -1.f;
    double sum = 0, stn = 0;
    int cnt = 0;
    float mt = 0.f;
    const volatile float *r = g->ratio;
    for (int i = 0; i < g->n; ++i) {
        const float v = r[i];
        if (v < -1.5f) return -1.f;
        if (v >= 0.f) { sum += v; ++cnt; }
        mt = std::max(mt, (float)r[kMaxBatchLds + i]);
        stn += std::max(0.f, (float)r[kMaxBatchLds + i]);
    }
    if (max_tn) *max_tn = mt;
    if (sum_tn && cnt) *sum_tn = p ? stn * (double)p->B / (double)g->n : stn;
    return cnt ? (float)(sum / cnt) : -1.f;
}

long long stage_hint_rest_chunks(const pvv_problem *p, hipStream_t st, uint32_t rest_mask)
{
    std::lock_guard<std::mutex> lock(g_hint_mu);
    StageHint *g = stage_hint_locked(st, false);
    if (!g || g->n <= 0) return -1;
    if (!hint_same_shape(g, p)) return -1;
    const volatile float *r = g->ratio;
    long long total = 0;
    constexpr int PC = 4 * kBfPixPerWave;
    for (int i = 0; i < g->n; ++i) {
        if (r[i] < -1.5f) return -1;
        const int nch = ((int)r[kMaxBatchLds + i] + PC - 1) / PC;
        if (nch >= kStageMinChunks)
            total += (nch / kStageM) * __builtin_popcount(rest_mask) + __builtin_popcount(rest_mask & ((1u << (nch % kStageM)) - 1u));
    }
    return total * p->B / g->n;
}

float stage_hint_threshold(const pvv_problem *p, double work)
{
    static const double xs[6] = {0.0, 0.585, 1.0, 1.585, 2.0, 3.0}, ys[6] = {0.990, 0.966, 0.957, 0.910, 0.765, 0.50};
    const double x = std::log2(std::max(work, 1.0) / 2.26e10);
    double thr;
    if (x <= xs[0]) thr = ys[0] + (ys[1] - ys[0]) / (xs[1] - xs[0]) * (x - xs[0]);
    else if (x >= xs[5]) thr = ys[5];
    else {
        int i = 0;
        while (x > xs[i + 1]) ++i;
        thr = ys[i] + (ys[i + 1] - ys[i]) * (x - xs[i]) / (xs[i + 1] - xs[i]);
    }
    thr -= 0.1 * std::log2(std::max(p->hn, 512) / 512.0);
    return (float)std::min(0.995, std::max(0.5, thr));
}

double stage_work(const pvv_problem *p, hipStream_t st, float *mean = nullptr, float *max_tn = nullptr)
{
    double sum_tn = -1.0;
    float mt = -1.f;
    const float m = stage_hint_mean(p, st, &mt, &sum_tn);
    if (mean) *mean = m;
    if (max_tn) *max_tn = mt;
    if (m < 0.f || sum_tn < 0.0) return stage_proxy_work(p);
    return (double)p->K * p->hn * sum_tn / kStageProxyFg;
}

bool stage_hint_allows(const pvv_problem *p, hipStream_t st)
{
    if (p->count_kernel != PVV_COUNT_AUTO) return true;
    float max_tn = -1.f, m = -1.f;
    const double work = stage_work(p, st, &m, &max_tn);
    if (work < kStageMinWork) return false;
    if (m < 0.f) return true;
    return m >= stage_hint_threshold(p, work) && max_tn > (float)((kStageMinChunks - 1) * 4 * kBfPixPerWave);
}

Bf16Consts bf16_consts(float thresh)
{
    const double T = (double)thresh, s2 = 1.0 - T * T, kappa = T / std::sqrt(s2);
    const double u = 0x1p-24;
    Bf16Consts fc;
    fc.beta = (float)(1.25 * (33.0 * (1.0 + kappa) + 8.0 / s2) * u / T);
    fc.eps_c = (float)(1.25 * (1.0 + kappa) * 35.0 * u);
    fc.eps0 = (float)(1.5e-6 * (1.0 + kappa));
    fc.kappa = (float)kappa;
    fc.beta2 = (float)(1.25 * (8.0 * (1.0 + kappa) + 8.0 / s2) * u / T);
#ifdef PVV_TUNING
    static const char *dbg = getenv("PVV_DEBUG_BAND_SCALE");
    if (dbg && *dbg) {
        const float k = (float)atof(dbg);
        fc.beta *= k; fc.eps_c *= k; fc.eps0 *= k;
    }
#endif
    return fc;
}

int tuning_int(const char *name, int dflt)
{
#ifdef PVV_TUNING
    static const char *names[32];
    static int vals[32], n = 0;
    for (int i = 0; i < n; ++i) if (!strcmp(names[i], name)) return vals[i] == INT32_MIN ? dflt : vals[i];
    const char *e = getenv(name);
    if (n < 32) { names[n] = name; vals[n] = e && *e ? atoi(e) : INT32_MIN; ++n; }
    return e && *e ? atoi(e) : dflt;
#else
    (void)name;
    return dflt;
#endif
}

long long *tuning_ptr(const char *name)
{
#ifdef PVV_TUNING
    const char *e = getenv(name);
    return e && *e ? (long long *)strtoull(e, nullptr, 0) : nullptr;
#else
    (void)name;
    return nullptr;
#endif
}

int mark(const pvv_problem *p, int i, hipStream_t st)
{
    if (!p->ev_marks || !p->ev_marks[i]) return PVV_OK;
    if (hipEventRecord((hipEvent_t)p->ev_marks[i], st) != hipSuccess) return fail(PVV_E_ARG, "ev_marks holds an invalid hipEvent_t");
    return PVV_OK;
}

struct StagedLaunch {
    const pvv_problem *p;
    char *ws;
    const Layout *L;
    hipStream_t st;
    Bf16Consts fc;
    long long *dbg;
    int per_cu_first, per_cu_filter, target_first, target_filter;
    int sub_tenth;
    int col0, hstride, lead_set;
    const float *mean;
};

template <uint32_t FIRST>
int launch_staged(const StagedLaunch &a)
{
    const pvv_problem *p = a.p;
    const Layout &L = *a.L;
    char *ws = a.ws;
    hipStream_t st = a.st;
    const Bf16Consts fc = a.fc;
    const float2 *coords = (const float2 *)(ws + L.coords), *dirs = (const float2 *)(ws + L.dirs);
    const float2 *hyps = (const float2 *)(ws + L.hyps) + a.col0;
    int *counts = (int *)(ws + L.counts) + a.col0;
    const int *tn = (const int *)(ws + L.tn);
    int *lead = (int *)(ws + L.lead) + (size_t)a.lead_set * lead_set_words(p);
    StageArgs sa;
    sa.lead = nullptr;
    sa.any_staged = lead + (size_t)p->B * p->K * 8;
    sa.miss = (int *)(ws + L.miss) + a.col0;
    sa.sub_tenth = a.sub_tenth;
    sa.hstride = a.hstride;
    sa.mean = (a.sub_tenth && tuning_int("PVV_PROX", 1) != 0) ? (const float2 *)a.mean : nullptr;
#ifdef PVV_STAMPS
    sa.dbg = tuning_ptr("PVV_DBG_PTR_FILTER");
#endif
    hipLaunchKernelGGL((k_count_bf16<kCountFirst, FIRST>), dim3(a.per_cu_first * num_cus()), dim3(kBlock), 0, st, coords, dirs, hyps, counts, tn,
                       p->B, p->K, p->hn, p->cap, p->inlier_thresh, fc, a.target_first, a.dbg, sa);
    if (int e = check_launch("k_count_bf16<first>")) return e;
    if (int e = mark(p, PVV_MARK_STAGE0, st)) return e;
    LeadArgs la;
    la.tn_arr = tn; la.coords = coords; la.dirs = dirs; la.hyps = hyps; la.counts = counts; la.lead = lead;
    la.K = p->K; la.hn = p->hn; la.cap = p->cap;
    la.hstride = a.hstride > 0 ? a.hstride : p->hn;
    la.kappa = fc.kappa; la.beta = 2.f * fc.beta2; la.eps = 2.f * fc.eps0;
    la.any_staged = sa.any_staged;
    la.nsplit = 16;
    while (la.nsplit > 1 && (long long)p->B * p->K * la.nsplit > 8ll * num_cus()) la.nsplit >>= 1;
    la.nsplit = tuning_int("PVV_LEAD_SPLIT", la.nsplit);
    hipLaunchKernelGGL(k_lead<FIRST>, dim3(p->K * la.nsplit, p->B), dim3(kBlock), 0, st, la);
    if (int e = check_launch("k_lead")) return e;
    if (int e = mark(p, PVV_MARK_PRUNE0, st)) return e;
    sa.lead = lead;
    const long long rest = p->count_kernel == PVV_COUNT_AUTO ? stage_hint_rest_chunks(p, st, stage_rest_of(FIRST)) : -1;
    const bool runs = rest < 0 || rest * p->K >= 2ll * a.target_filter || p->hn > 512;
    if (tuning_int("PVV_FILTER_OLD", runs ? 0 : 1) == 0) {
        hipLaunchKernelGGL(k_count_filter_runs<FIRST>, dim3(tuning_int("PVV_GRID_PER_CU_FILTER", 5) * num_cus()), dim3(kBlock), sizeof(int) * (size_t)p->B, st, coords, dirs,
                           hyps, counts, tn, p->B, p->K, p->hn, p->cap, p->inlier_thresh, fc, a.target_filter, tuning_int("PVV_RUN_R", 0), sa);
        return check_launch("k_count_filter_runs");
    }
    hipLaunchKernelGGL((k_count_bf16<kCountFilter, FIRST>), dim3(a.per_cu_filter * num_cus()), dim3(kBlock), 0, st, coords, dirs, hyps, counts, tn,
                       p->B, p->K, p->hn, p->cap, p->inlier_thresh, fc, a.target_filter, a.dbg, sa);
    return check_launch("k_count_bf16<filter>");
}

struct CountCols {
    int col0 = 0;
    int hstride = 0;
    int lead_set = 0;
    const float *mean = nullptr;
};

int launch_count_bf16(const pvv_problem *p, const Layout &L, char *ws, hipStream_t st, int staged ,
                      const CountCols &cc = CountCols())
{
    const int per_cu_t = tuning_int("PVV_GRID_PER_CU", 0);
    const int items_per_cu = tuning_int("PVV_ITEMS_PER_CU", 5);
    bool few = p->B <= 8;
    if (p->count_kernel == PVV_COUNT_AUTO) {
        double sum_tn = -1.0;
        if (stage_hint_mean(p, st, nullptr, &sum_tn) >= 0.f && sum_tn >= 0.0)
            few = sum_tn / (4 * kBfPixPerWave) * p->K * ((p->hn + 511) / 512) <= 2000.0;
    }
    const int per_cu = per_cu_t > 0 ? per_cu_t : (few ? 5 : ((p->hn < 2048 || p->B <= 8) ? 15 : 48));
    const float2 *coords = (const float2 *)(ws + L.coords), *dirs = (const float2 *)(ws + L.dirs);
    const float2 *hyps = (const float2 *)(ws + L.hyps) + cc.col0;
    int *counts = (int *)(ws + L.counts) + cc.col0;
    const int *tn = (const int *)(ws + L.tn);
    const Bf16Consts fc = bf16_consts(p->inlier_thresh);
    const int target = tuning_int("PVV_TARGET_ITEMS", items_per_cu * num_cus());
    const int target_first = tuning_int("PVV_TARGET_ITEMS_FIRST", target), target_filter = tuning_int("PVV_TARGET_ITEMS_FILTER", target);
    const int per_cu_first = tuning_int("PVV_GRID_PER_CU_FIRST", per_cu);
    const int per_cu_filter = tuning_int("PVV_GRID_PER_CU_FILTER", p->hn < 2048 ? 5 : per_cu);
    long long *dbg = tuning_ptr("PVV_DBG_PTR");
    if (!staged) {
        StageArgs full{};
        full.hstride = cc.hstride;
        hipLaunchKernelGGL(k_count_bf16<kCountFull>, dim3(per_cu * num_cus()), dim3(kBlock), 0, st, coords, dirs, hyps, counts, tn,
                           p->B, p->K, p->hn, p->cap, p->inlier_thresh, fc, target, dbg, full);
        return check_launch("k_count_bf16");
    }
    StagedLaunch sl;
    sl.p = p; sl.ws = ws; sl.L = &L; sl.st = st; sl.fc = fc; sl.dbg = dbg;
    sl.per_cu_first = per_cu_first; sl.per_cu_filter = per_cu_filter; sl.target_first = target_first; sl.target_filter = target_filter;
    sl.sub_tenth = staged == 2 ? 1 : 0;
    sl.col0 = cc.col0; sl.hstride = cc.hstride; sl.lead_set = cc.lead_set; sl.mean = cc.mean;
    const double sum_tn = (p->count_kernel == PVV_COUNT_AUTO ? stage_work(p, st) : stage_proxy_work(p)) * kStageProxyFg / ((double)p->K * p->hn);
    const double chunks_per_slot = (double)p->K * sum_tn / (4.0 * kBfPixPerWave) / (5.0 * num_cus());
    const bool eighth = tuning_int("PVV_STAGE_EIGHTH", (staged != 2 && chunks_per_slot >= 5.8) ? 1 : 0) != 0;
    return eighth ? launch_staged<kStageFirstEighth>(sl) : launch_staged<kStageFirst>(sl);
}

CountArgs planar_count_args(const pvv_problem *p, const Layout &L, char *ws)
{
    CountArgs a;
    a.coords = (const float2 *)(ws + L.coords);
    a.dirs = (const float2 *)(ws + L.dirs);
    a.hyps = (const float2 *)(ws + L.hyps);
    a.counts = (int *)(ws + L.counts);
    a.tn_arr = (const int *)(ws + L.tn);
    a.c_b = p->cap;
    a.d_b = (long long)p->K * p->cap; a.d_v = p->cap; a.d_p = 1;
    a.h_b = (long long)p->K * p->hn; a.h_v = p->hn; a.h_h = 1;
    a.tn_fixed = 0;
    a.B = p->B; a.K = p->K; a.hn = p->hn;
    a.thresh = p->inlier_thresh;
    return a;
}

constexpr double kEstStageMinWork = 2e11;
bool est_stage_auto(const pvv_problem *p, hipStream_t st)
{
    if (p->hn < 1024) return false;
    double sum_tn = -1.0;
    float max_tn = -1.f;
    const float rho = stage_hint_mean(p, st, &max_tn, &sum_tn, true);
    if (rho < 0.f || sum_tn < 0.0) return stage_proxy_work(p) >= kEstStageMinWork;
    if (!(max_tn > (float)((kStageMinChunks - 1) * 4 * kBfPixPerWave))) return false;
    const double work = (double)p->K * p->hn * sum_tn / kStageProxyFg;
    return work >= (rho >= 0.95f ? 6e10 : (rho >= 0.85f ? 9e10 : kEstStageMinWork));
}
int decide_staged(const pvv_problem *p, const Layout &L, hipStream_t st, int kind)
{
    if (!may_stage(p) || L.lead == 0) return 0;
    if (kind == 1 && stage_hint_allows(p, st)) return 1;
    if (kind == 2 && (p->count_kernel == PVV_COUNT_STAGED_ESTIMATE || (p->count_kernel == PVV_COUNT_AUTO && est_stage_auto(p, st)))) return 2;
    return 0;
}

int launch_count_any(const pvv_problem *p, const Layout &L, char *ws, hipStream_t st, int staged, const CountCols &cc = CountCols())
{
    if (p->ev_count_begin && hipEventRecord((hipEvent_t)p->ev_count_begin, st) != hipSuccess)
        return fail(PVV_E_ARG, "ev_count_begin is not a valid hipEvent_t");
    if (!use_bf16_count(p) && (cc.col0 || cc.hstride)) return fail(PVV_E_ARG, "internal: a column range needs the bf16 count kernel");
    const int e = use_bf16_count(p) ? launch_count_bf16(p, L, ws, st, staged, cc) : launch_count(planar_count_args(p, L, ws), st);
    if (e) return e;
    if (p->ev_count_end && hipEventRecord((hipEvent_t)p->ev_count_end, st) != hipSuccess)
        return fail(PVV_E_ARG, "ev_count_end is not a valid hipEvent_t");
    return PVV_OK;
}

template <int ES, int MODE, int ST = kElemF32>
void launch_scan(const MaskArgs &m, const Layout &L, char *ws, int B, hipStream_t st)
{
    const long long total = (long long)L.T * B;
    uint32_t *tiles = (uint32_t *)(ws + L.tiles);
    unsigned short *lists = (unsigned short *)(ws + L.tile_list);
    float *draws = (float *)(ws + L.tile_draw);
    if (!(m.contig && !m.seg)) {
        hipLaunchKernelGGL((k_tile_scan<ES, false, MODE, ST>), dim3((unsigned)total), dim3(kBlock), 0, st, m, tiles, lists, draws, (int)total);
        return;
    }
    const int per_cu_t = tuning_int("PVV_SCAN_PER_CU", 0);
    long long per_block = 1;
    if (per_cu_t > 0) per_block = (total + (long long)per_cu_t * num_cus() - 1) / ((long long)per_cu_t * num_cus());
    const int grid = (int)((total + per_block - 1) / per_block);
    hipLaunchKernelGGL((k_tile_scan<ES, true, MODE>), dim3(grid), dim3(kBlock), 0, st, m, tiles, lists, draws, (int)total);
}

struct Front {
    MaskArgs m;
    VertexArgs v;
    HypArgs h;
    bool can_subsample;
    bool seg2;
    int vt, st;
    long long *mask_deferred;
};

Front make_front(const pvv_problem *p, int mode, const void *d_mask, const float *d_vertex, const int32_t *d_idxs,
                 const float *d_selection, char *ws, const Layout &L, int32_t *d_tn, const float *d_seg,
                 int64_t *d_mask_out, const int32_t *d_idxs2, int hn_first, uint32_t stream_first, uint32_t stream_rest)
{
    Front f;
    MaskArgs &m = f.m;
    m.mask = d_mask;
    m.seg = d_seg;
    m.mask_out = (long long *)d_mask_out;
    m.gb = p->seg_stride[0]; m.gc = p->seg_stride[1]; m.gh = p->seg_stride[2]; m.gw = p->seg_stride[3];
    m.C = p->seg_classes;
    m.selection = d_selection;
    m.sb = p->mask_stride[0]; m.sh = p->mask_stride[1]; m.sw = p->mask_stride[2];
    m.es = p->mask_elem_size;
    m.contig = (m.sw == 1 && m.sh == p->W) ? 1 : 0;
    m.mode = mode;
    m.W = p->W; m.HW = p->H * p->W; m.T = L.T;
    m.min_num = p->min_num; m.max_num = p->max_num; m.cap = p->cap;
    m.seed = p->seed;
    m.b0 = p->first_image;
    m.tn_user = d_tn;
    m.status = p->d_status;
    m.fuse_sub = (fuse_sub_shape(p, L.T) && !d_idxs && !d_idxs2) ? 1 : 0;
    const long long max_weight = mode == 1 ? 1 : (d_seg ? (p->seg_classes > 1 ? p->seg_classes - 1 : 1) : 255);
    f.can_subsample = (long long)p->max_num < max_weight * (long long)p->H * p->W;
    m.want_draws = (f.can_subsample && !m.fuse_sub) ? 1 : 0;
    f.vt = (p->flags & PVV_FLAG_VERTEX_F16) ? kElemF16 : (p->flags & PVV_FLAG_VERTEX_BF16) ? kElemBF16 : kElemF32;
    f.st = (p->flags & PVV_FLAG_SEG_F16) ? kElemF16 : (p->flags & PVV_FLAG_SEG_BF16) ? kElemBF16 : kElemF32;
    const int seg_es = f.st == kElemF32 ? 4 : 2, vertex_es = f.vt == kElemF32 ? 4 : 2;
    f.seg2 = d_seg && p->seg_classes == 2 && m.gw == 1 && m.gh == p->W && (((long long)p->H * p->W) & 3) == 0 && (m.gb & 3) == 0 &&
             (m.gc & 3) == 0 && ((uintptr_t)d_seg % (4 * seg_es)) == 0;
    f.mask_deferred = nullptr;
    if (f.seg2 && d_mask_out && !(f.can_subsample && !m.fuse_sub) && (long long)p->B * p->H * p->W >= (1ll << 21) &&
        ((uintptr_t)d_mask_out & 15) == 0)
        f.mask_deferred = (long long *)d_mask_out;
    VertexArgs &v = f.v;
    v.vertex = d_vertex;
    v.sb = p->vertex_stride[0]; v.sh = p->vertex_stride[1]; v.sw = p->vertex_stride[2];
    v.sk = p->vertex_stride[3]; v.sc = p->vertex_stride[4];
    v.K = p->K;
    v.vec2 = (v.sc == 1 && !(v.sb & 1) && !(v.sh & 1) && !(v.sw & 1) && !(v.sk & 1) &&
              ((uintptr_t)d_vertex % (2 * vertex_es) == 0)) ? 1 : 0;
    HypArgs &h = f.h;
    h.idxs = d_idxs; h.idxs2 = d_idxs2;
    h.hn = p->hn; h.hn_first = hn_first < 0 ? p->hn : hn_first;
    h.stream = stream_first; h.stream2 = stream_rest;
    h.hyps = (float2 *)(ws + L.hyps);
    h.counts = (int *)(ws + L.counts);
    h.draws_out = p->d_draws_out;
    h.blocks = (int)(((long long)p->K * p->hn + kBlock - 1) / kBlock);
    h.surv = (int *)(ws + L.surv);
    h.lead = L.lead ? (int *)(ws + L.lead) : nullptr;
    h.miss = L.miss ? (int *)(ws + L.miss) : nullptr;
    return f;
}

int run_scan(const pvv_problem *p, const Front &f, char *ws, const Layout &L, hipStream_t st, bool write_mask)
{
    if (f.seg2) {
        MaskArgs m = f.m;
        if (!write_mask) m.mask_out = nullptr;
        const unsigned total = (unsigned)((long long)L.T * p->B);
        uint32_t *tiles = (uint32_t *)(ws + L.tiles);
        unsigned short *lists = (unsigned short *)(ws + L.tile_list);
        float *draws = (float *)(ws + L.tile_draw);
        auto go2 = [&](auto et) {
            constexpr int ST = decltype(et)::value;
            if (write_mask) hipLaunchKernelGGL((k_tile_scan_seg2<true, ST>), dim3(total), dim3(kBlock), 0, st, m, tiles, lists, draws);
            else hipLaunchKernelGGL((k_tile_scan_seg2<false, ST>), dim3(total), dim3(kBlock), 0, st, m, tiles, lists, draws);
        };
        if (f.st == kElemF16) go2(std::integral_constant<int, kElemF16>{});
        else if (f.st == kElemBF16) go2(std::integral_constant<int, kElemBF16>{});
        else go2(std::integral_constant<int, kElemF32>{});
        return check_launch("k_tile_scan_seg2");
    }
    if (f.m.seg && f.st != kElemF32) {
        if (f.st == kElemF16) launch_scan<8, 0, kElemF16>(f.m, L, ws, p->B, st);
        else launch_scan<8, 0, kElemBF16>(f.m, L, ws, p->B, st);
        return check_launch("k_tile_scan");
    }
    auto go = [&](auto es) {
        constexpr int ES = decltype(es)::value;
        if (f.m.mode == 0) launch_scan<ES, 0>(f.m, L, ws, p->B, st); else launch_scan<ES, 1>(f.m, L, ws, p->B, st);
    };
    switch (f.m.es) {
    case 1: go(std::integral_constant<int, 1>{}); break;
    case 2: go(std::integral_constant<int, 2>{}); break;
    case 4: go(std::integral_constant<int, 4>{}); break;
    default: go(std::integral_constant<int, 8>{}); break;
    }
    return check_launch("k_tile_scan");
}

#ifdef PVV_SIDE_EVENT_SYSTEM_FENCE
constexpr unsigned kSideEventFlags = hipEventDisableTiming;
#else
constexpr unsigned kSideEventFlags = hipEventDisableTiming | hipEventDisableSystemFence;
#endif
struct SideStream {
    hipStream_t st = nullptr;
    hipEvent_t fork[8] = {}, join[8] = {};
    int next = 0;
    bool tried = false, ok = false;
};
SideStream g_side[64];
std::mutex g_side_mu;

SideStream *side_get(hipStream_t st)
{
    int cur = -1;
    const int dev = stream_device(st);
    if (dev < 0 || hipGetDevice(&cur) != hipSuccess || cur != dev) return nullptr;
    hipStreamCaptureStatus cs = hipStreamCaptureStatusNone;
    if (hipStreamIsCapturing(st, &cs) != hipSuccess) { (void)hipGetLastError(); return nullptr; }
    if (cs != hipStreamCaptureStatusNone) return nullptr;
    std::lock_guard<std::mutex> lock(g_side_mu);
    SideStream *g = &g_side[dev];
    if (!g->tried) {
        g->tried = true;
        bool ok = hipStreamCreateWithFlags(&g->st, hipStreamNonBlocking) == hipSuccess;
        for (int i = 0; ok && i < 8; ++i)
            ok = hipEventCreateWithFlags(&g->fork[i], kSideEventFlags) == hipSuccess &&
                 hipEventCreateWithFlags(&g->join[i], kSideEventFlags) == hipSuccess;
        if (!ok) (void)hipGetLastError();
        g->ok = ok;
    }
    return g->ok ? g : nullptr;
}

bool side_fork_locked(SideStream *g, hipStream_t st, hipStream_t *side, hipEvent_t *join)
{
    const int i = g->next;
    g->next = (i + 1) & 7;
    if (hipEventRecord(g->fork[i], st) != hipSuccess || hipStreamWaitEvent(g->st, g->fork[i], 0) != hipSuccess) { (void)hipGetLastError(); return false; }
    *side = g->st;
    *join = g->join[i];
    return true;
}

struct SideJoin {
    hipStream_t st = nullptr;
    hipEvent_t join = nullptr;
    bool armed = false;
    int finish()
    {
        if (!armed) return PVV_OK;
        armed = false;
        return hipStreamWaitEvent(st, join, 0) == hipSuccess ? PVV_OK : fail(PVV_E_ARG, "side stream: hipStreamWaitEvent failed");
    }
    ~SideJoin()
    {
        if (armed && hipStreamWaitEvent(st, join, 0) != hipSuccess) (void)hipGetLastError();
    }
};

struct CountPlan {
    const pvv_problem *p;
    int staged;
    CountCols cols;
};

int run_front(const pvv_problem *p, int mode, const void *d_mask, const float *d_vertex,
              const int32_t *d_idxs, const float *d_selection, char *ws, const Layout &L,
              hipStream_t st, int32_t *d_tn, const float *d_seg = nullptr, int64_t *d_mask_out = nullptr,
              const int32_t *d_idxs2 = nullptr, int hn_first = -1, uint32_t stream_first = 1u, uint32_t stream_rest = 3u,
              int stage_kind = 0 , const CountPlan *plan = nullptr,
              const float *d_mean = nullptr )
{
    if ((p->flags & PVV_FLAG_DEVICE_RNG) && (d_idxs || d_idxs2 || d_selection))
        return fail(PVV_E_ARG, "PVV_FLAG_DEVICE_RNG promises d_idxs = d_idxs_est = d_selection = NULL");
    Front f = make_front(p, mode, d_mask, d_vertex, d_idxs, d_selection, ws, L, d_tn, d_seg, d_mask_out, d_idxs2,
                         hn_first, stream_first, stream_rest);
    if (f.m.want_draws && L.tile_draw == 0) return fail(PVV_E_WORKSPACE, "workspace holds no draw storage for this call");
    const int staged = plan ? 1 : decide_staged(p, L, st, stage_kind);
    if (!staged) { f.h.miss = nullptr; f.h.lead = nullptr; }
    if (int e = mark(p, PVV_MARK_BEGIN, st)) return e;
    SideJoin sj;
    SideStream *sg = (f.mask_deferred && tuning_int("PVV_MASK_DEFER", 1) != 0) ? side_get(st) : nullptr;
    const bool defer_mask = sg != nullptr;
    if (int e = run_scan(p, f, ws, L, st, !defer_mask)) return e;
    if (!f.m.fuse_sub && f.can_subsample) {
        hipLaunchKernelGGL(k_tile_subsample, dim3(L.T, p->B), dim3(kBlock), 0, st, f.m, (uint32_t *)(ws + L.tiles),
                           (unsigned short *)(ws + L.tile_list), (const float *)(ws + L.tile_draw));
        if (int e = check_launch("k_tile_subsample")) return e;
    }
    if (int e = mark(p, PVV_MARK_SCAN, st)) return e;
    auto compact = [&](auto et) {
        constexpr int VT = decltype(et)::value;
        hipLaunchKernelGGL(k_compact_hyp<VT>, dim3(L.T + f.h.blocks, p->B), dim3(kBlock), sizeof(int) * (size_t)L.T, st, f.m, f.v,
                           f.h, (const uint32_t *)(ws + L.tiles), (const unsigned short *)(ws + L.tile_list),
                           (const float *)(ws + L.tile_draw), (int *)(ws + L.tn), (float2 *)(ws + L.coords),
                           (float2 *)(ws + L.dirs));
    };
    if (f.vt == kElemF16) compact(std::integral_constant<int, kElemF16>{});
    else if (f.vt == kElemBF16) compact(std::integral_constant<int, kElemBF16>{});
    else compact(std::integral_constant<int, kElemF32>{});
    if (int e = check_launch("k_compact_hyp")) return e;
    if (int e = mark(p, PVV_MARK_COMPACT, st)) return e;
    if (defer_mask) {
        std::lock_guard<std::mutex> lock(g_side_mu);
        hipStream_t side = nullptr;
        hipEvent_t join = nullptr;
        const bool forked = side_fork_locked(sg, st, &side, &join);
        const hipStream_t ms = forked ? side : st;
        const long long total = (long long)L.T * p->B;
        const int grid = (int)std::min<long long>(total, (long long)tuning_int("PVV_MASK_GRID_PER_CU", 2) * num_cus());
        hipLaunchKernelGGL(k_mask_from_lists, dim3(grid), dim3(kBlock), 0, ms, (const uint32_t *)(ws + L.tiles),
                           (const unsigned short *)(ws + L.tile_list), f.mask_deferred, L.T, p->H * p->W, (int)total);
        const int le = check_launch("k_mask_from_lists");
        if (forked) {
            if (hipEventRecord(join, side) == hipSuccess) { sj.st = st; sj.join = join; sj.armed = true; }
            else {
                (void)hipGetLastError();
                (void)hipStreamSynchronize(side);
                if (!le) return fail(PVV_E_ARG, "side stream: hipEventRecord failed");
            }
        }
        if (le) return le;
    }
    CountCols whole;
    whole.mean = d_mean;
    if (int e = plan ? launch_count_any(plan->p, L, ws, st, plan->staged, plan->cols) : launch_count_any(p, L, ws, st, staged, whole)) return e;
    if (int e = sj.finish()) return e;
    return mark(p, PVV_MARK_COUNT, st);
}

int check_ptrs(const pvv_problem *p, const void *mask, const void *vertex, void *ws, size_t ws_bytes,
               Layout *L)
{
    if (int e = validate(p)) return e;
    if (!mask || !vertex || !ws) return fail(PVV_E_ARG, "mask, vertex and workspace must be non-NULL");
    if ((uintptr_t)ws % 256 != 0) return fail(PVV_E_ARG, "workspace must be 256-byte aligned");
    *L = make_layout(p);
    if (ws_bytes < L->total) return fail(PVV_E_WORKSPACE, "workspace too small");
    return PVV_OK;
}

}

PVV_EXPORT int pvv_abi_version(void) { return PVV_ABI_VERSION; }
PVV_EXPORT const char *pvv_last_error(void) { return g_err; }

PVV_EXPORT int pvv_shutdown(void)
{
    int rc = PVV_OK;
    auto note = [&](hipError_t e, const char *what) {
        if (e != hipSuccess) {
            (void)hipGetLastError();
            if (rc == PVV_OK) { snprintf(g_err, sizeof(g_err), "pvv_shutdown: %s: %s", what, hipGetErrorString(e)); rc = (int)e; }
        }
    };
    int cur = -1;
    const bool have_cur = hipGetDevice(&cur) == hipSuccess;
    if (!have_cur) (void)hipGetLastError();
    {
        std::lock_guard<std::mutex> lock(g_side_mu);
        for (int dev = 0; dev < 64; ++dev) {
            SideStream *g = &g_side[dev];
            if (g->tried) {
                if (have_cur && hipSetDevice(dev) != hipSuccess) (void)hipGetLastError();
                if (g->st) { note(hipStreamSynchronize(g->st), "hipStreamSynchronize(side stream)"); note(hipStreamDestroy(g->st), "hipStreamDestroy"); }
                for (int i = 0; i < 8; ++i) {
                    if (g->fork[i]) note(hipEventDestroy(g->fork[i]), "hipEventDestroy");
                    if (g->join[i]) note(hipEventDestroy(g->join[i]), "hipEventDestroy");
                }
            }
            *g = SideStream();
        }
    }
    {
        std::lock_guard<std::mutex> lock(g_hint_mu);
        for (int dev = 0; dev < 64; ++dev) {
            StageHint *g = &g_hint[dev];
            if (g->ratio) note(hipHostFree(g->ratio), "hipHostFree(stage hint)");
            *g = StageHint();
        }
    }
    if (have_cur && hipSetDevice(cur) != hipSuccess) (void)hipGetLastError();
    return rc;
}

PVV_EXPORT int pvv_stage_hint_query(float *mean_ratio, float *threshold, const pvv_problem *p, void *stream)
{
    float m = stage_hint_mean(p, (hipStream_t)stream);
    if (threshold) *threshold = -1.f;
    if (p) {
        const double work = stage_work(p, (hipStream_t)stream, &m);
        if (threshold) *threshold = work >= kStageMinWork ? stage_hint_threshold(p, work) : 2.f;
    }
    if (mean_ratio) *mean_ratio = m;
    return m >= 0.f ? 1 : 0;
}

PVV_EXPORT int32_t pvv_default_cap(int32_t H, int32_t W, int32_t max_num)
{
    long long hw = (long long)H * W;
    if (max_num < 0) max_num = 0;
    long long cap = (long long)max_num + (long long)(8.0 * std::sqrt((double)max_num)) + 64;
    return (int32_t)(cap < hw ? cap : hw);
}

PVV_EXPORT size_t pvv_workspace_bytes(const pvv_problem *p)
{
    if (validate(p)) return 0;
    return make_layout(p).total;
}

static int finish_v3(const pvv_problem *p, const Layout &L, char *ws, float *d_out, int32_t *d_win_counts,
                     hipStream_t st, int hstride = 0)
{
    if (hstride <= 0) hstride = p->hn;
    int nsplit = kRefitSplitMax;
    while (nsplit > 1 && (long long)p->B * p->K * nsplit > 6ll * num_cus()) nsplit >>= 1;
    nsplit = tuning_int("PVV_REFIT_SPLIT", nsplit);
    const Bf16Consts fc = bf16_consts(p->inlier_thresh);
    const bool band = use_bf16_count(p) && (long long)p->B * p->K >= 128;
    auto launch_refit = [&](auto kernel) {
        hipLaunchKernelGGL(kernel, dim3(p->K * nsplit, p->B), dim3(kBlock), 0, st,
                           (const int *)(ws + L.tn), (const float2 *)(ws + L.coords),
                           (const float2 *)(ws + L.dirs), (const float2 *)(ws + L.hyps),
                           (const int *)(ws + L.counts), (double *)(ws + L.sums), d_win_counts, p->K, p->hn, hstride,
                           p->cap, p->inlier_thresh, nsplit, (float *)(ws + L.ratio), fc);
    };
    if (band) launch_refit(k_select_refit<true>); else launch_refit(k_select_refit<false>);
    if (int e = check_launch("k_select_refit")) return e;
    if (int e = mark(p, PVV_MARK_SELECT, st)) return e;
    float *hint = (p->count_kernel == PVV_COUNT_AUTO && may_stage(p)) ? stage_hint_claim(p, st) : nullptr;
    hipLaunchKernelGGL(k_finalize_v3, dim3(p->B), dim3(64), 0, st, (const int *)(ws + L.tn),
                       (const double *)(ws + L.sums), (float2 *)d_out, p->K, p->singular_policy, nsplit,
                       (const float *)(ws + L.ratio), hint, kMaxBatchLds);
    if (int e = check_launch("k_finalize_v3")) return e;
    return mark(p, PVV_MARK_END, st);
}

PVV_EXPORT int pvv_ransac_voting_v3(const pvv_problem *p, const void *d_mask, const float *d_vertex,
                                    const int32_t *d_idxs, const float *d_selection,
                                    void *d_workspace, size_t workspace_bytes, float *d_out,
                                    int32_t *d_win_counts, int32_t *d_tn, void *stream)
{
    Layout L;
    if (int e = check_ptrs(p, d_mask, d_vertex, d_workspace, workspace_bytes, &L)) return e;
    if (!d_out) return fail(PVV_E_ARG, "d_out is NULL");
    hipStream_t st = (hipStream_t)stream;
    char *ws = (char *)d_workspace;
    if (int e = run_front(p, 0, d_mask, d_vertex, d_idxs, d_selection, ws, L, st, d_tn, nullptr, nullptr, nullptr, -1, 1u, 3u, 1))
        return e;
    return finish_v3(p, L, ws, d_out, d_win_counts, st);
}

PVV_EXPORT int pvv_decode_keypoint_v3(const pvv_problem *p, const float *d_seg, const float *d_vertex,
                                      const int32_t *d_idxs, const float *d_selection, void *d_workspace,
                                      size_t workspace_bytes, int64_t *d_mask_out, float *d_out,
                                      int32_t *d_win_counts, int32_t *d_tn, void *stream)
{
    Layout L;
    if (p && p->mask_elem_size == 0) return fail(PVV_E_ARG, "set mask_elem_size = 8 (the int64 mask this call emits)");
    if (int e = check_ptrs(p, d_seg, d_vertex, d_workspace, workspace_bytes, &L)) return e;
    if (!d_out) return fail(PVV_E_ARG, "d_out is NULL");
    if (p->seg_classes < 1 || p->seg_classes > 256) return fail(PVV_E_ARG, "seg_classes must be in [1, 256]");
    hipStream_t st = (hipStream_t)stream;
    char *ws = (char *)d_workspace;
    if (int e = run_front(p, 0, nullptr, d_vertex, d_idxs, d_selection, ws, L, st, d_tn, d_seg, d_mask_out, nullptr, -1, 1u, 3u, 1))
        return e;
    return finish_v3(p, L, ws, d_out, d_win_counts, st);
}

PVV_EXPORT int pvv_estimate_voting_distribution(const pvv_problem *p, const void *d_mask,
                                                const float *d_vertex, const int32_t *d_idxs,
                                                const float *d_selection, const float *d_mean,
                                                void *d_workspace, size_t workspace_bytes,
                                                float *d_cov, float *d_hyp, int32_t *d_counts,
                                                int32_t *d_tn, float *d_weights, void *stream)
{
    Layout L;
    if (int e = check_ptrs(p, d_mask, d_vertex, d_workspace, workspace_bytes, &L)) return e;
    if (!d_mean || !d_cov) return fail(PVV_E_ARG, "d_mean / d_cov is NULL");
    hipStream_t st = (hipStream_t)stream;
    char *ws = (char *)d_workspace;
    if (int e = run_front(p, 1, d_mask, d_vertex, d_idxs, d_selection, ws, L, st, d_tn, nullptr, nullptr, nullptr, -1, 3u, 3u, d_counts ? 0 : 2, nullptr, d_mean)) return e;
    hipLaunchKernelGGL(k_covariance, dim3(p->K, p->B), dim3(kBlock), 0, st,
                       (const int *)(ws + L.tn), (const float2 *)(ws + L.hyps),
                       (const int *)(ws + L.counts), (const float2 *)d_mean, d_cov, (float2 *)d_hyp,
                       d_counts, d_weights, p->K, p->hn, p->hn, 0);
    if (int e = check_launch("k_covariance")) return e;
    return mark(p, PVV_MARK_END, st);
}

PVV_EXPORT int pvv_estimate_counts_in_stages(const pvv_problem *p)
{
    if (int e = validate(p)) return e < 0 ? e : -e;
    if (!may_stage(p)) return 0;
    return (p->count_kernel == PVV_COUNT_STAGED_ESTIMATE || (p->count_kernel == PVV_COUNT_AUTO && est_stage_auto(p, nullptr))) ? 1 : 0;
}

static pvv_problem un_pnp_problem(const pvv_problem *p, int32_t hn_est)
{
    pvv_problem q = *p;
    q.hn = p->hn + hn_est;
    return q;
}

PVV_EXPORT size_t pvv_workspace_bytes_un_pnp(const pvv_problem *p, int32_t hn_est)
{
    if (validate(p) || hn_est <= 0) return 0;
    const pvv_problem q = un_pnp_problem(p, hn_est);
    if (validate(&q)) return 0;
    return make_layout(&q).total;
}

PVV_EXPORT int pvv_decode_keypoint_un_pnp(const pvv_problem *p, int32_t hn_est, const float *d_seg,
                                          const float *d_vertex, const int32_t *d_idxs, const int32_t *d_idxs_est,
                                          const float *d_selection, void *d_workspace, size_t workspace_bytes,
                                          int64_t *d_mask_out, float *d_kpt, float *d_cov, float *d_weights,
                                          int32_t *d_win_counts, int32_t *d_tn, void *stream)
{
    if (int e = validate(p)) return e;
    if (hn_est <= 0) return fail(PVV_E_ARG, "hn_est must be positive");
    if (p->mask_elem_size == 0) return fail(PVV_E_ARG, "set mask_elem_size = 8 (the int64 mask this call emits)");
    if (p->seg_classes != 2) return fail(PVV_E_ARG, "the fused un_pnp pass needs seg_classes == 2 (PVNet's seg_dim)");
    const pvv_problem q = un_pnp_problem(p, hn_est);
    Layout L;
    if (int e = check_ptrs(&q, d_seg, d_vertex, d_workspace, workspace_bytes, &L)) return e;
    if (!d_kpt || !d_cov) return fail(PVV_E_ARG, "d_kpt / d_cov is NULL");
    hipStream_t st = (hipStream_t)stream;
    char *ws = (char *)d_workspace;
    pvv_problem pe = *p;
    pe.hn = hn_est;
    const int est_staged = decide_staged(&pe, L, st, 2);
    if (est_staged) {
        const size_t set_bytes = sizeof(int) * lead_set_words(p);
        if (hipMemsetAsync(ws + L.lead + set_bytes, 0, set_bytes, st) != hipSuccess) return fail(PVV_E_ARG, "hipMemsetAsync(leader words) failed");
        pvv_problem p1 = *p;
        p1.ev_count_end = nullptr;
        pe.ev_count_begin = nullptr;
        CountPlan plan;
        plan.p = &p1;
        plan.staged = decide_staged(p, L, st, 1);
        plan.cols.col0 = 0; plan.cols.hstride = q.hn; plan.cols.lead_set = 0;
        if (int e = run_front(&q, 0, nullptr, d_vertex, d_idxs, d_selection, ws, L, st, d_tn, d_seg, d_mask_out, d_idxs_est,
                              p->hn, 1u, 3u, 0, &plan))
            return e;
        if (int e = finish_v3(p, L, ws, d_kpt, d_win_counts, st, q.hn)) return e;
        CountCols ec;
        ec.col0 = p->hn; ec.hstride = q.hn; ec.lead_set = 1; ec.mean = d_kpt;
        if (int e = launch_count_any(&pe, L, ws, st, est_staged, ec)) return e;
    } else {
        if (int e = run_front(&q, 0, nullptr, d_vertex, d_idxs, d_selection, ws, L, st, d_tn, d_seg, d_mask_out, d_idxs_est,
                              p->hn))
            return e;
        if (int e = finish_v3(p, L, ws, d_kpt, d_win_counts, st, q.hn)) return e;
    }
    hipLaunchKernelGGL(k_covariance, dim3(p->K, p->B), dim3(kBlock), 0, st, (const int *)(ws + L.tn),
                       (const float2 *)(ws + L.hyps), (const int *)(ws + L.counts), (const float2 *)d_kpt, d_cov,
                       (float2 *)nullptr, (int *)nullptr, d_weights, p->K, (int)hn_est, q.hn, p->hn);
    if (int e = check_launch("k_covariance")) return e;
    return PVV_OK;
}

PVV_EXPORT int pvv_rerun_count_kernel(const pvv_problem *p, void *d_workspace, size_t workspace_bytes,
                                      int zero_counts, void *stream)
{
    if (p && p->count_kernel == PVV_COUNT_STAGED && !zero_counts)
        return fail(PVV_E_ARG, "a staged count pass needs zero_counts = 1");
    const int v3 = (p && p->count_kernel == PVV_COUNT_STAGED) ? 1 : 0;
    if (int e = validate(p)) return e;
    if (!d_workspace) return fail(PVV_E_ARG, "workspace is NULL");
    Layout L = make_layout(p);
    if (workspace_bytes < L.total) return fail(PVV_E_WORKSPACE, "workspace too small");
    hipStream_t st = (hipStream_t)stream;
    char *ws = (char *)d_workspace;
    if (zero_counts) {
        hipError_t e = hipMemsetAsync(ws + L.counts, 0, sizeof(int) * (size_t)p->B * p->K * p->hn, st);
        if (e == hipSuccess && L.lead) e = hipMemsetAsync(ws + L.lead, 0, sizeof(int) * lead_set_words(p), st);
        if (e == hipSuccess && L.miss) e = hipMemsetAsync(ws + L.miss, 0, sizeof(int) * (size_t)p->B * p->K * p->hn, st);
        if (e != hipSuccess) return fail((int)e, hipGetErrorString(e));
    }
    return launch_count_any(p, L, ws, st, decide_staged(p, L, st, v3));
}

namespace {
typedef unsigned int u32x4 __attribute__((ext_vector_type(4)));
__global__ __launch_bounds__(kBlock) void k_stream_read(const u32x4 *__restrict__ src, size_t n16, uint32_t *__restrict__ sink)
{
    uint32_t acc = 0;
    const size_t stride = (size_t)gridDim.x * kBlock;
    size_t i = (size_t)blockIdx.x * kBlock + threadIdx.x;
    for (; i + 3 * stride < n16; i += 4 * stride) {
        const u32x4 a = __builtin_nontemporal_load(src + i), b = __builtin_nontemporal_load(src + i + stride);
        const u32x4 c = __builtin_nontemporal_load(src + i + 2 * stride), d = __builtin_nontemporal_load(src + i + 3 * stride);
        acc += (a.x ^ a.y ^ a.z ^ a.w) + (b.x ^ b.y ^ b.z ^ b.w) + (c.x ^ c.y ^ c.z ^ c.w) + (d.x ^ d.y ^ d.z ^ d.w);
    }
    for (; i < n16; i += stride) {
        const u32x4 a = __builtin_nontemporal_load(src + i);
        acc += a.x ^ a.y ^ a.z ^ a.w;
    }
    acc = wave_sum(acc);
    if (lane_id() == 0 && acc == 0x9e3779b9u) atomicAdd(sink, acc);
}
}

PVV_EXPORT int pvv_stream_read_probe(const void *d_buf, size_t bytes, uint32_t *d_sink, void *stream)
{
    if (!d_buf || !d_sink || bytes < 16 || (bytes & 15) || ((uintptr_t)d_buf & 15)) return fail(PVV_E_ARG, "probe: 16-byte aligned buffer and size");
    hipLaunchKernelGGL(k_stream_read, dim3(num_cus() * 8), dim3(kBlock), 0, (hipStream_t)stream, (const u32x4 *)d_buf, bytes / 16, d_sink);
    return check_launch("k_stream_read");
}

static int check_legacy(const void *a, const void *b, const void *c, const void *d, int tn, int vn,
                        int hn)
{
    if (!a || !b || !c || !d) return fail(PVV_E_ARG, "NULL device pointer");
    if (tn < 0 || vn <= 0 || hn < 0) return fail(PVV_E_ARG, "tn, hn must be >= 0 and vn > 0");
    if ((long long)hn * vn >= (1ll << 29) || (long long)tn * vn >= (1ll << 29) ||
        (long long)hn * vn * (long long)(tn > 0 ? tn : 1) >= (1ll << 40))
        return fail(PVV_E_ARG, "problem too large");
    return PVV_OK;
}

PVV_EXPORT int pvv_generate_hypothesis(const float *d_direct, const float *d_coords,
                                       const int32_t *d_idxs, float *d_hypo_pts, int tn, int vn,
                                       int hn, void *stream)
{
    if (int e = check_legacy(d_direct, d_coords, d_idxs, d_hypo_pts, tn, vn, hn)) return e;
    if (hn == 0) return PVV_OK;
    hipLaunchKernelGGL(k_legacy_gen, dim3((hn * vn + kBlock - 1) / kBlock), dim3(kBlock), 0,
                       (hipStream_t)stream, d_direct, d_coords, d_idxs, d_hypo_pts, tn, vn, hn);
    return check_launch("k_legacy_gen");
}

PVV_EXPORT int pvv_generate_hypothesis_vanishing_point(const float *d_direct, const float *d_coords,
                                                       const int32_t *d_idxs, float *d_hypo_pts,
                                                       int tn, int vn, int hn, void *stream)
{
    if (int e = check_legacy(d_direct, d_coords, d_idxs, d_hypo_pts, tn, vn, hn)) return e;
    if (hn == 0) return PVV_OK;
    hipLaunchKernelGGL(k_legacy_gen_vp, dim3((hn * vn + kBlock - 1) / kBlock), dim3(kBlock), 0,
                       (hipStream_t)stream, d_direct, d_coords, d_idxs, d_hypo_pts, tn, vn, hn);
    return check_launch("k_legacy_gen_vp");
}

static void legacy_vote_shape(int tn, int vn, int hn, dim3 *grid, int *h_per_block)
{
    int tiles = (tn + kBlock - 1) / kBlock;
    int hz = 1;
    while ((long long)tiles * vn * hz < 4096 && hz < hn) hz <<= 1;
    if (hz > hn) hz = hn;
    if (hz > 65535) hz = 65535;
    *h_per_block = (hn + hz - 1) / hz;
    *grid = dim3(tiles, vn, (hn + *h_per_block - 1) / *h_per_block);
}

PVV_EXPORT int pvv_voting_for_hypothesis(const float *d_direct, const float *d_coords,
                                         const float *d_hypo_pts, uint8_t *d_inliers, int tn, int vn,
                                         int hn, float inlier_thresh, void *stream)
{
    if (int e = check_legacy(d_direct, d_coords, d_hypo_pts, d_inliers, tn, vn, hn)) return e;
    if (vn > 65535) return fail(PVV_E_ARG, "vn > 65535");
    if (hn == 0 || tn == 0) return PVV_OK;
    dim3 grid; int hpb;
    legacy_vote_shape(tn, vn, hn, &grid, &hpb);
    hipLaunchKernelGGL(k_legacy_vote, grid, dim3(kBlock), 0, (hipStream_t)stream, d_direct, d_coords,
                       d_hypo_pts, d_inliers, tn, vn, hn, hpb, inlier_thresh);
    return check_launch("k_legacy_vote");
}

PVV_EXPORT int pvv_voting_for_hypothesis_vanishing_point(const float *d_direct, const float *d_coords,
                                                         const float *d_hypo_pts, uint8_t *d_inliers,
                                                         int tn, int vn, int hn, float inlier_thresh,
                                                         void *stream)
{
    if (int e = check_legacy(d_direct, d_coords, d_hypo_pts, d_inliers, tn, vn, hn)) return e;
    if (vn > 65535) return fail(PVV_E_ARG, "vn > 65535");
    if (hn == 0 || tn == 0) return PVV_OK;
    dim3 grid; int hpb;
    legacy_vote_shape(tn, vn, hn, &grid, &hpb);
    hipLaunchKernelGGL(k_legacy_vote_vp, grid, dim3(kBlock), 0, (hipStream_t)stream, d_direct,
                       d_coords, d_hypo_pts, d_inliers, tn, vn, hn, hpb, inlier_thresh);
    return check_launch("k_legacy_vote_vp");
}

PVV_EXPORT int pvv_count_inliers(const float *d_direct, const float *d_coords, const float *d_hypo_pts,
                                 int32_t *d_counts, int tn, int vn, int hn, float inlier_thresh,
                                 void *stream)
{
    if (int e = check_legacy(d_direct, d_coords, d_hypo_pts, d_counts, tn, vn, hn)) return e;
    if (hn == 0) return PVV_OK;
    hipStream_t st = (hipStream_t)stream;
    hipError_t me = hipMemsetAsync(d_counts, 0, sizeof(int) * (size_t)hn * vn, st);
    if (me != hipSuccess) return fail((int)me, hipGetErrorString(me));
    if (tn == 0) return PVV_OK;
    CountArgs a;
    a.coords = (const float2 *)d_coords;
    a.dirs = (const float2 *)d_direct;
    a.hyps = (const float2 *)d_hypo_pts;
    a.counts = d_counts;
    a.tn_arr = nullptr;
    a.c_b = 0;
    a.d_b = 0; a.d_v = 1; a.d_p = vn;
    a.h_b = 0; a.h_v = 1; a.h_h = vn;
    a.tn_fixed = tn;
    a.B = 1; a.K = vn; a.hn = hn;
    a.thresh = inlier_thresh;
    return launch_count(a, st);
}

#include "crop.hpp"

#include "dcn.hpp"
```

### clean-pvnet_amd/csrc/refit.hpp

```cpp
#pragma once

constexpr int kRefitSplitMax = 8;

template <bool BAND>
__global__ __launch_bounds__(kBlock) void k_select_refit(
    const int *__restrict__ tn_arr, const float2 *__restrict__ coords,
    const float2 *__restrict__ dirs, const float2 *__restrict__ hyps,
    const int *__restrict__ counts, double *__restrict__ sums ,
    int *__restrict__ win_counts , int K, int hn, int hstride ,
    int cap, float thresh, int nsplit, float *__restrict__ win_ratio ,
    Bf16Consts fc )
{
    __shared__ int s_cnt[4], s_idx[4];
    __shared__ double red5[20];
    const int vi = blockIdx.x / nsplit, split = blockIdx.x - vi * nsplit, b = blockIdx.y;
    const int bk = b * K + vi;
    const int tn = tn_arr[b];
    double *part = sums + ((size_t)bk * nsplit + split) * 5;
    if (tn <= 0) {
        if (threadIdx.x == 0) {
            for (int i = 0; i < 5; ++i) part[i] = 0.0;
            if (win_counts && split == 0) win_counts[bk] = 0;
            if (split == 0) win_ratio[bk] = -1.f;
        }
        return;
    }
    const int *cp = counts + (size_t)bk * hstride;
    int best = -1, besti = 0x7fffffff;
    for (int h = threadIdx.x; h < hn; h += kBlock) {
        int c = cp[h];
        if (c > best) { best = c; besti = h; }
    }
    wave_argmax_first(best, besti);
    if (lane_id() == 0) { s_cnt[threadIdx.x >> 6] = best; s_idx[threadIdx.x >> 6] = besti; }
    __syncthreads();
    best = s_cnt[0]; besti = s_idx[0];
#pragma unroll
    for (int w = 1; w < 4; ++w)
        if (s_cnt[w] > best || (s_cnt[w] == best && s_idx[w] < besti)) { best = s_cnt[w]; besti = s_idx[w]; }

    float2 win = make_float2(0.f, 0.f);
    if (best > 0) win = hyps[(size_t)bk * hstride + besti];

    const bool win_near = fabsf(win.x) < 1e15f && fabsf(win.y) < 1e15f;
    const float2 *dp = dirs + (size_t)bk * cap;
    const float2 *cq = coords + (size_t)b * cap;
    double xx = 0, xy = 0, yy = 0, bx = 0, by = 0;
    const int per = (tn + nsplit - 1) / nsplit;
    const int tbeg = split * per, tend = min(tn, tbeg + per);
    for (int t0 = tbeg + threadIdx.x; t0 < tend; t0 += 4 * kBlock) {
        float2 d[4], c[4];
#pragma unroll
        for (int u = 0; u < 4; ++u) {
            const int ti = t0 + u * kBlock;
            d[u] = ti < tend ? dp[ti] : make_float2(0.f, 0.f);
            c[u] = ti < tend ? cq[ti] : make_float2(0.f, 0.f);
        }
#pragma unroll
        for (int u = 0; u < 4; ++u) {
            bool inlier;
            if constexpr (BAND) {
                const float dd = d[u].x * d[u].x + d[u].y * d[u].y;
                const float rinv = __builtin_amdgcn_rsqf(dd);
                const float ux = d[u].x * rinv, uy = d[u].y * rinv;
                const float dx = win.x - c[u].x, dy = win.y - c[u].y;
                const float a2 = __builtin_fmaf(dx, ux, dy * uy);
                const float b2 = __builtin_fmaf(dx, -fc.kappa * uy, dy * (fc.kappa * ux));
                const float t2 = a2 - fabsf(b2);
                inlier = t2 > 0.f;
                const bool unsure = !win_near || !(dd >= kDdAlive && dd < INFINITY) ||
                                    !(__builtin_fmaf(-fc.beta2, a2, fabsf(t2)) > fc.eps0);
                if (__any(unsure)) {
                    if (unsure) inlier = vote_exact(c[u].x, c[u].y, win.x, win.y, d[u].x, d[u].y, thresh);
                }
            } else {
                inlier = vote_exact(c[u].x, c[u].y, win.x, win.y, d[u].x, d[u].y, thresh);
            }
            if (!inlier) continue;
            double nx = (double)d[u].y, ny = -(double)d[u].x;
            double bb = nx * (double)c[u].x + ny * (double)c[u].y;
            xx += nx * nx; xy += nx * ny; yy += ny * ny;
            bx += nx * bb; by += ny * bb;
        }
    }
    double v[5] = {xx, xy, yy, bx, by};
#pragma unroll
    for (int i = 0; i < 5; ++i) v[i] = wave_total(v[i]);
    if (lane_id() == 0) {
#pragma unroll
        for (int i = 0; i < 5; ++i) red5[(threadIdx.x >> 6) * 5 + i] = v[i];
    }
    __syncthreads();
    if (threadIdx.x < 5) part[threadIdx.x] = red5[threadIdx.x] + red5[5 + threadIdx.x] + red5[10 + threadIdx.x] + red5[15 + threadIdx.x];
    if (threadIdx.x == 0 && split == 0) {
        if (win_counts) win_counts[bk] = best;
        win_ratio[bk] = (float)best / (float)tn;
    }
}

__global__ __launch_bounds__(64) void k_finalize_v3(const int *__restrict__ tn_arr, const double *__restrict__ sums,
                                                    float2 *__restrict__ out, int K, int policy, int nsplit,
                                                    const float *__restrict__ win_ratio, float *hint, int hint_stride)
{
    __shared__ int any_singular;
    const int b = blockIdx.x;
    if (threadIdx.x == 0) any_singular = 0;
    __syncthreads();
    const bool skipped = win_ratio[(size_t)b * K] < -0.5f;
    if (hint) {
        float r = 0.f;
        for (int vi = threadIdx.x; vi < K; vi += 64) r += win_ratio[(size_t)b * K + vi];
        r = wave_total(r);
        if (threadIdx.x == 0) {
            hint[b] = skipped ? -1.f : r / (float)K;
            hint[hint_stride + b] = (float)tn_arr[b];
        }
    }
    for (int v0 = 0; v0 < K; v0 += 64) {
        const int vi = v0 + threadIdx.x;
        float2 o = make_float2(0.f, 0.f);
        double bx = 0, by = 0;
        bool sing = false;
        if (vi < K && !skipped) {
            const double *q = sums + ((size_t)b * K + vi) * nsplit * 5;
            double xx = 0, xy = 0, yy = 0;
            for (int sp = 0; sp < nsplit; ++sp) {
                xx += q[sp * 5]; xy += q[sp * 5 + 1]; yy += q[sp * 5 + 2]; bx += q[sp * 5 + 3]; by += q[sp * 5 + 4];
            }
            const double det = xx * yy - xy * xy;
            sing = !(det != 0.0) || !isfinite(det);
            if (!sing) {
                o.x = (float)((yy * bx - xy * by) / det);
                o.y = (float)((xx * by - xy * bx) / det);
            }
        }
        if (K > 64) {
            if (sing) atomicOr(&any_singular, 1);
            continue;
        }
        if (sing) any_singular = 1;
        __syncthreads();
        if (vi < K) {
            if (!skipped && any_singular && policy != PVV_SINGULAR_ZERO) {
                if (policy == PVV_SINGULAR_REFERENCE) o = make_float2((float)bx, (float)by);
                else o = make_float2(0.f, 0.f);
            }
            out[(size_t)b * K + vi] = o;
        }
        return;
    }
    __syncthreads();
    for (int vi = threadIdx.x; vi < K; vi += 64) {
        float2 o = make_float2(0.f, 0.f);
        if (!skipped) {
            const double *q = sums + ((size_t)b * K + vi) * nsplit * 5;
            double xx = 0, xy = 0, yy = 0, bx = 0, by = 0;
            for (int sp = 0; sp < nsplit; ++sp) {
                xx += q[sp * 5]; xy += q[sp * 5 + 1]; yy += q[sp * 5 + 2]; bx += q[sp * 5 + 3]; by += q[sp * 5 + 4];
            }
            const double det = xx * yy - xy * xy;
            const bool sing = !(det != 0.0) || !isfinite(det);
            if (!sing) {
                o.x = (float)((yy * bx - xy * by) / det);
                o.y = (float)((xx * by - xy * bx) / det);
            }
            if (any_singular && policy != PVV_SINGULAR_ZERO)
                o = policy == PVV_SINGULAR_REFERENCE ? make_float2((float)bx, (float)by) : make_float2(0.f, 0.f);
        }
        out[(size_t)b * K + vi] = o;
    }
}
```

Before: 329,700 images/s.

## Compute staged-filter lead bound in-kernel and write rest counts to separate extra buffer

The filter-runs kernel now makes two passes over its items. The first pass computes the per-(image,keypoint) leading hypotheses from the counts and publishes them. It also tallies sure inliers for those leaders over the block's chunks and atomically accumulates the result into the lead words. The second pass re-reads a live lower bound (lstar) before each group of hypotheses, so pruning can tighten as other blocks contribute. Counts from the rest stage are written to a new 'extra' buffer, and refit and covariance sum it with counts. This adds an extra argmax and pixel pass plus extra memory traffic and zeroing, in exchange for earlier and tighter pruning.

```diff
diff --git a/clean-pvnet_amd/csrc/compaction.hpp b/clean-pvnet_amd/csrc/compaction.hpp
--- a/clean-pvnet_amd/csrc/compaction.hpp
+++ b/clean-pvnet_amd/csrc/compaction.hpp
@@ -459,6 +459,7 @@
     int *surv;
     int *lead;
     int *miss;
+    int *extra;
 };
 
 constexpr int kHypRejectTries = 1 << 12;
@@ -555,7 +556,7 @@
         const int vi = gid / h.hn, hi = gid - vi * h.hn;
         const size_t o = ((size_t)b * v.K + vi) * h.hn + hi;
         h.counts[o] = 0;
-        if (h.miss) h.miss[o] = 0;
+        if (h.miss) { h.miss[o] = 0; h.extra[o] = 0; }
         if (h.lead && hi == 0) {
             int *lw = h.lead + ((size_t)b * v.K + vi) * 8 + 4;
             lw[0] = 0; lw[1] = 0; lw[2] = 0; lw[3] = 0;
diff --git a/clean-pvnet_amd/csrc/count_bf16.hpp b/clean-pvnet_amd/csrc/count_bf16.hpp
--- a/clean-pvnet_amd/csrc/count_bf16.hpp
+++ b/clean-pvnet_amd/csrc/count_bf16.hpp
@@ -73,9 +73,10 @@
 constexpr int kStageMinChunks = 8;
 
 struct StageArgs {
-    const int *lead;
+    int *lead;
     int *any_staged;
     int *miss;
+    int *extra;
     int sub_tenth;
     const float2 *mean;
     int hstride;
diff --git a/clean-pvnet_amd/csrc/count_filter_runs.hpp b/clean-pvnet_amd/csrc/count_filter_runs.hpp
--- a/clean-pvnet_amd/csrc/count_filter_runs.hpp
+++ b/clean-pvnet_amd/csrc/count_filter_runs.hpp
@@ -33,7 +33,7 @@
 template <uint32_t FIRST>
 __global__ __launch_bounds__(kBlock) __attribute__((amdgpu_waves_per_eu(5, 5))) void k_count_filter_runs(
     const float2 *__restrict__ coords , const float2 *__restrict__ dirs ,
-    const float2 *__restrict__ hyps , int *__restrict__ counts ,
+    const float2 *__restrict__ hyps , const int *__restrict__ counts ,
     const int *__restrict__ tn_arr, int B, int K, int hn, int cap, float thresh, Bf16Consts fc, int target_items, int run_r, StageArgs sa)
 {
     extern __shared__ int run_end[];
@@ -95,34 +95,51 @@
     const int ebase = kslice * 4;
     const float16v zero16 = {0.f, 0.f, 0.f, 0.f, 0.f, 0.f, 0.f, 0.f, 0.f, 0.f, 0.f, 0.f, 0.f, 0.f, 0.f, 0.f};
 
-    for (int item = blockIdx.x; item < total; item += gridDim.x) {
+    int gr, g_begin, g_end, r_img, b, bk, tn, nrest, nruns, j0, R_rem, nmine, tid, pb;
+    bool prox;
+    const float2 *hyp_k, *crd, *dir_k;
+    const int *cnt_k;
+    int *ext_k, *miss_k, *lead_k;
+    int lc[4], li[4];
+    float2 org, pc0[2], pd0[2];
+    auto chunk_pb = [&](int it) {
+        const int j = prox ? __builtin_amdgcn_readfirstlane((int)s_order[r_img + it * nruns]) : j0 + it;
+        return stage_chunk_at<REST>(j) * PC;
+    };
+    auto load_px = [&](int pb_, float2 (&c_)[2], float2 (&d_)[2]) {
+#pragma unroll
+        for (int q = 0; q < 2; ++q) {
+            const int p = min(pb_ + tid + q * kBlock, cap - 1);
+            c_[q] = crd[p];
+            d_[q] = dir_k[p];
+        }
+    };
+    auto item_head = [&](int item, bool publish) {
         const int grun = item / per_run, rem_i = item - grun * per_run;
-        const int vi = ngr == 1 ? rem_i : rem_i / ngr, gr = rem_i - vi * ngr;
-        const int g_begin = gr * gpi, g_end = min(nhg, g_begin + gpi);
-        int r_img;
-        const int b = locate_item(run_end, B, grun, &r_img);
-        const int bk = b * K + vi;
-        const float2 *hyp_k = hyps + (size_t)bk * hs;
-        const float2 *crd = coords + (size_t)b * cap;
-        const float2 *dir_k = dirs + (size_t)bk * cap;
-        int *cnt_k = counts + (size_t)bk * hs;
-        int *miss_k = sa.miss + (size_t)bk * hs;
-        const int tn = __builtin_amdgcn_readfirstlane(tn_arr[b]);
+        const int vi = ngr == 1 ? rem_i : rem_i / ngr;
+        gr = rem_i - vi * ngr;
+        g_begin = gr * gpi; g_end = min(nhg, g_begin + gpi);
+        b = locate_item(run_end, B, grun, &r_img);
+        bk = b * K + vi;
+        hyp_k = hyps + (size_t)bk * hs;
+        crd = coords + (size_t)b * cap;
+        dir_k = dirs + (size_t)bk * cap;
+        cnt_k = counts + (size_t)bk * hs;
+        ext_k = sa.extra + (size_t)bk * hs;
+        miss_k = sa.miss + (size_t)bk * hs;
+        lead_k = sa.lead + (size_t)bk * 8;
+        tn = __builtin_amdgcn_readfirstlane(tn_arr[b]);
         const int nch = (tn + PC - 1) / PC;
-        const int nrest = stage_chunks<REST>(nch);
-        const int nruns = (nrest + R - 1) / R;
-        const int j0 = (int)((long long)r_img * nrest / nruns), j1 = (int)((long long)(r_img + 1) * nrest / nruns);
-        const int R_rem = stage_pixels<REST>(tn, nch, PC);
-        int lstar;
-        {
-            const int lead_p = sa.lead[(size_t)bk * 8 + (lane & 3)], lead_r = sa.lead[(size_t)bk * 8 + 4 + (lane & 3)];
-            int full = lead_p >= 0 ? lead_p + lead_r : -1;
-            full = max(full, PVV_DPP(full, full, 0xB1, 0xf, false));
-            full = max(full, PVV_DPP(full, full, 0x4E, 0xf, false));
-            lstar = stage_bound(__builtin_amdgcn_readfirstlane(full), tn, sa.sub_tenth);
-        }
-
-        const bool prox = sa.mean != nullptr && nrest <= 64;
+        nrest = stage_chunks<REST>(nch);
+        nruns = (nrest + R - 1) / R;
+        j0 = (int)((long long)r_img * nrest / nruns);
+        const int j1 = (int)((long long)(r_img + 1) * nrest / nruns);
+        R_rem = stage_pixels<REST>(tn, nch, PC);
+        tid = threadIdx.x;
+        asm volatile("" : "+v"(tid));
+        __syncthreads();
+
+        prox = sa.mean != nullptr && nrest <= 64;
         if (prox && wave == 0) {
             float key = INFINITY;
             if (lane < nrest) {
@@ -137,13 +154,139 @@
             }
             if (lane < nrest) s_order[rank] = (unsigned short)lane;
         }
-        const int nmine = prox ? (nrest - r_img + nruns - 1) / nruns : j1 - j0;
+        nmine = prox ? (nrest - r_img + nruns - 1) / nruns : j1 - j0;
+        {
+            int best = -1, besth = 0x7fffffff;
+            for (int h = tid; h < hn; h += kBlock) {
+                const int c = cnt_k[h];
+                if (c > best) { best = c; besth = h; }
+            }
+            wave_argmax_first(best, besth);
+            if (lane == 0) { sCnt[2 * wave] = best; sCnt[2 * wave + 1] = besth; }
+            __syncthreads();
+#pragma unroll
+            for (int w = 0; w < 4; ++w) { lc[w] = sCnt[2 * w]; li[w] = sCnt[2 * w + 1]; }
+            lead_pick(lc, li);
+#pragma unroll
+            for (int w = 0; w < kLead; ++w) { lc[w] = __builtin_amdgcn_readfirstlane(lc[w]); li[w] = __builtin_amdgcn_readfirstlane(li[w]); }
+        }
+        pb = chunk_pb(0);
+        org = crd[pb];
+        load_px(pb, pc0, pd0);
+        if (publish && gr == 0) {
+            const LeadTest lt = lead_test(fc.kappa, fc.beta2, fc.eps0, lc, li, hyp_k);
+            int inl[kLead];
+#pragma unroll
+            for (int w = 0; w < kLead; ++w) inl[w] = 0;
+            float2 nc[2], nd[2];
+            int pbn = pb;
+            if (nmine > 1) { pbn = chunk_pb(1); load_px(pbn, nc, nd); }
+            const float2 dead = make_float2(0.f, 0.f);
+#pragma unroll
+            for (int q = 0; q < 2; ++q) lead_sure(lt, pc0[q], pb + tid + q * kBlock < tn ? pd0[q] : dead, inl);
+            for (int it = 1; it < nmine; ++it) {
+                const int pbc = pbn;
+                float2 cc[2], cd[2];
+#pragma unroll
+                for (int q = 0; q < 2; ++q) { cc[q] = nc[q]; cd[q] = nd[q]; }
+                if (it + 1 < nmine) { pbn = chunk_pb(it + 1); load_px(pbn, nc, nd); }
+#pragma unroll
+                for (int q = 0; q < 2; ++q) lead_sure(lt, cc[q], pbc + tid + q * kBlock < tn ? cd[q] : dead, inl);
+            }
+#pragma unroll
+            for (int w = 0; w < kLead; ++w) {
+                const int t = wave_total(inl[w]);
+                if (lane == 0) sCnt[8 + 2 * wave + w] = t;
+            }
+        }
+        __syncthreads();
+        if (publish && gr == 0 && tid < kLead) {
+            const int t = sCnt[8 + tid] + sCnt[10 + tid] + sCnt[12 + tid] + sCnt[14 + tid];
+            if (t) atomicAdd(&lead_k[4 + tid], t);
+        }
+        if (publish && tid < 4) lead_k[tid] = tid == 0 ? lc[0] : (tid == 1 ? lc[1] : -1);
+    };
+    for (int item = blockIdx.x; item < total; item += gridDim.x) item_head(item, true);
+    for (int item = blockIdx.x; item < total; item += gridDim.x) {
+        item_head(item, false);
+        auto read_lstar = [&]() {
+            const int lw = lane & 3;
+            const int lead_r = __hip_atomic_load(&lead_k[4 + lw], __ATOMIC_RELAXED, __HIP_MEMORY_SCOPE_AGENT);
+            const int lead_p = lw == 0 ? lc[0] : (lw == 1 ? lc[1] : -1);
+            int full = lead_p >= 0 ? lead_p + lead_r : -1;
+            full = max(full, PVV_DPP(full, full, 0xB1, 0xf, false));
+            full = max(full, PVV_DPP(full, full, 0x4E, 0xf, false));
+            return stage_bound(__builtin_amdgcn_readfirstlane(full), tn, sa.sub_tenth);
+        };
+        auto build_records = [&](const float2 (&pc)[2], const float2 (&pd)[2]) {
+            float c1 = 0.f;
+#pragma unroll
+            for (int q = 0; q < 2; ++q) {
+                const int pl = tid + q * kBlock, p = pb + pl;
+                float4 rec = make_float4(__builtin_nanf(""), 0.f, 0.f, 0.f);
+                if (p < tn) {
+                    const float2 c = pc[q], d = pd[q];
+                    const float cx = c.x - org.x, cy = c.y - org.y;
+                    c1 = fmaxf(c1, fabsf(cx) + fabsf(cy));
+                    const float dd = d.x * d.x + d.y * d.y;
+                    if (dd >= kDdAlive && dd < INFINITY) {
+                        const float rinv = __builtin_amdgcn_rsqf(dd);
+                        rec = make_float4(d.x * rinv, d.y * rinv, cx, cy);
+                    }
+                }
+                sP[pl] = rec;
+            }
+            c1 = wave_max(c1);
+            if (lane == 0) sRed[wave] = c1;
+        };
+        auto build_operands = [&](float &eps, float &epsw, int &npx, int &ntile_w, bf16x8 (&A)[8]) {
+            const float C1 = fmaxf(fmaxf(sRed[0], sRed[1]), fmaxf(sRed[2], sRed[3]));
+            eps = fc.eps0 + fc.eps_c * C1;
+            epsw = __builtin_fmaf(fc.beta * 1.02f, C1, eps);
+            npx = min(tn - pb, PC);
+            const int ntile_c = (npx + 15) >> 4;
+            ntile_w = (ntile_c - wave + 3) >> 2;
+            if (ntile_w > 0) {
+                const int form = (tid >> 4) & 1, prow = tid & 15, ks4 = (tid >> 3) & 4, wv = tid >> 6;
+#pragma unroll
+                for (int i = 0; i < 4; ++i) {
+                    const int jt = ks4 + i;
+                    const float4 rec = sP[(jt * 4 + wv) * 16 + prow];
+                    const bool dead = rec.x != rec.x;
+                    float rx = form ? -fc.kappa * rec.y : rec.x;
+                    float ry = form ? fc.kappa * rec.x : rec.y;
+                    float rz = -(rec.z * rx + rec.w * ry);
+                    if (dead) { rx = 0.f; ry = 0.f; rz = form ? 0.f : -1e30f; }
+                    __bf16 vx[3], vy[3], cv[3];
+                    split3(rx, vx);
+                    split3(ry, vy);
+                    split3(rz, cv);
+                    const __bf16 zero = (__bf16)0.f;
+                    const bf16x8 lo8 = {vx[0], vy[0], vx[0], vx[0], vx[1], vy[0], vy[0], vy[1]};
+                    const bf16x8 hi8 = {vx[2], vy[2], vx[1], vy[1], cv[0], cv[1], cv[2], zero};
+                    uint4 x = __builtin_bit_cast(uint4, lo8), y = __builtin_bit_cast(uint4, hi8);
+                    {
+                        const auto r0 = __builtin_amdgcn_permlane32_swap(x.x, y.x, false, false);
+                        const auto r1 = __builtin_amdgcn_permlane32_swap(x.y, y.y, false, false);
+                        const auto r2 = __builtin_amdgcn_permlane32_swap(x.z, y.z, false, false);
+                        const auto r3 = __builtin_amdgcn_permlane32_swap(x.w, y.w, false, false);
+                        x = make_uint4(r0[0], r1[0], r2[0], r3[0]);
+                        y = make_uint4(r0[1], r1[1], r2[1], r3[1]);
+                    }
+                    A[i] = __builtin_bit_cast(bf16x8, x);
+                    A[4 + i] = __builtin_bit_cast(bf16x8, y);
+                }
+            }
+        };
+        build_records(pc0, pd0);
+        int built = 0;
         PVV_FS(1);
         PVV_FS_ADD(10, 1);
         for (int g = g_begin; g < g_end;) {
             const int gp0 = g;
             int ns = 0;
             __syncthreads();
+            const int lstar = read_lstar();
             for (; g < g_end && g - gp0 < 63; ++g) {
                 bool keep[2];
                 int slack[2];
@@ -184,20 +327,7 @@
             PVV_FS(2);
             if (ns == 0) continue;
 
-            for (int it = 0; it < nmine && ns > 0; ++it) {
-                const int j = prox ? __builtin_amdgcn_readfirstlane((int)s_order[r_img + it * nruns]) : j0 + it;
-                const int chunk = stage_chunk_at<REST>(j);
-                const int pb = chunk * PC;
-                int tid = threadIdx.x;
-                asm volatile("" : "+v"(tid));
-                const float2 org = crd[pb];
-                float2 pc[2], pd[2];
-#pragma unroll
-                for (int q = 0; q < 2; ++q) {
-                    const int p = min(pb + tid + q * kBlock, cap - 1);
-                    pc[q] = crd[p];
-                    pd[q] = dir_k[p];
-                }
+            auto stage_survivors = [&]() {
                 const int ns_pad = (ns + 31) & ~31;
                 float2 hp[2];
 #pragma unroll
@@ -205,76 +335,36 @@
                     const int i = tid + q * kBlock;
                     hp[q] = i < ns ? hyp_k[gp0 * GH + (int)((unsigned)sCnt[i] >> 16)] : make_float2(0.f, 0.f);
                 }
-                float c1 = 0.f;
-#pragma unroll
-                for (int q = 0; q < 2; ++q) {
-                    const int pl = tid + q * kBlock, p = pb + pl;
-                    float4 rec = make_float4(__builtin_nanf(""), 0.f, 0.f, 0.f);
-                    if (p < tn) {
-                        const float2 c = pc[q], d = pd[q];
-                        const float cx = c.x - org.x, cy = c.y - org.y;
-                        c1 = fmaxf(c1, fabsf(cx) + fabsf(cy));
-                        const float dd = d.x * d.x + d.y * d.y;
-                        if (dd >= kDdAlive && dd < INFINITY) {
-                            const float rinv = __builtin_amdgcn_rsqf(dd);
-                            rec = make_float4(d.x * rinv, d.y * rinv, cx, cy);
-                        }
-                    }
-                    sP[pl] = rec;
-                }
-                c1 = wave_max(c1);
-                if (lane == 0) sRed[wave] = c1;
                 int far = 0;
 #pragma unroll
                 for (int q = 0; q < 2; ++q) {
                     const int i = tid + q * kBlock;
                     if (i < ns_pad) far |= stage_hypothesis_b(sB, i, hp[q], org);
                 }
-                far = __syncthreads_or(far);
+                return __syncthreads_or(far);
+            };
+            for (int it = 0; it < nmine && ns > 0; ++it) {
+                tid = threadIdx.x;
+                asm volatile("" : "+v"(tid));
+                if (it != built) {
+                    pb = chunk_pb(it);
+                    org = crd[pb];
+                    float2 pc[2], pd[2];
+                    load_px(pb, pc, pd);
+                    build_records(pc, pd);
+                    built = it;
+                }
+                const int far = stage_survivors();
+                float eps, epsw;
+                int npx, ntile_w;
+                bf16x8 A[8];
+                build_operands(eps, epsw, npx, ntile_w, A);
                 PVV_FS(3);
                 PVV_FS_ADD(11, 1);
                 PVV_FS_ADD(12, ns);
-                const float C1 = fmaxf(fmaxf(sRed[0], sRed[1]), fmaxf(sRed[2], sRed[3]));
-                const float eps = fc.eps0 + fc.eps_c * C1;
-                const float epsw = __builtin_fmaf(fc.beta * 1.02f, C1, eps);
-                const int npx = min(tn - pb, PC);
-                const int ntile_c = (npx + 15) >> 4;
-                const int ntile_w = (ntile_c - wave + 3) >> 2;
-                bf16x8 A[8];
-                if (ntile_w > 0) {
-                    const int form = (lane >> 4) & 1, prow = lane & 15;
-#pragma unroll
-                    for (int i = 0; i < 4; ++i) {
-                        const int jt = kslice * 4 + i;
-                        const float4 rec = sP[(jt * 4 + wave) * 16 + prow];
-                        const bool dead = rec.x != rec.x;
-                        float rx = form ? -fc.kappa * rec.y : rec.x;
-                        float ry = form ? fc.kappa * rec.x : rec.y;
-                        float rz = -(rec.z * rx + rec.w * ry);
-                        if (dead) { rx = 0.f; ry = 0.f; rz = form ? 0.f : -1e30f; }
-                        __bf16 vx[3], vy[3], cv[3];
-                        split3(rx, vx);
-                        split3(ry, vy);
-                        split3(rz, cv);
-                        const __bf16 zero = (__bf16)0.f;
-                        const bf16x8 lo8 = {vx[0], vy[0], vx[0], vx[0], vx[1], vy[0], vy[0], vy[1]};
-                        const bf16x8 hi8 = {vx[2], vy[2], vx[1], vy[1], cv[0], cv[1], cv[2], zero};
-                        uint4 x = __builtin_bit_cast(uint4, lo8), y = __builtin_bit_cast(uint4, hi8);
-                        {
-                            const auto r0 = __builtin_amdgcn_permlane32_swap(x.x, y.x, false, false);
-                            const auto r1 = __builtin_amdgcn_permlane32_swap(x.y, y.y, false, false);
-                            const auto r2 = __builtin_amdgcn_permlane32_swap(x.z, y.z, false, false);
-                            const auto r3 = __builtin_amdgcn_permlane32_swap(x.w, y.w, false, false);
-                            x = make_uint4(r0[0], r1[0], r2[0], r3[0]);
-                            y = make_uint4(r0[1], r1[1], r2[1], r3[1]);
-                        }
-                        A[i] = __builtin_bit_cast(bf16x8, x);
-                        A[4 + i] = __builtin_bit_cast(bf16x8, y);
-                    }
-                }
+                const int ns_pad = (ns + 31) & ~31;
                 const int nht = ns_pad >> 5, nslot = ns;
                 const float2 *hyp_p = hyp_k + gp0 * GH;
-                PVV_FS(4);
                 PVV_FS_ADD(13, nht * ntile_w);
 
                 if (__builtin_expect(far, 0)) {
@@ -370,6 +460,7 @@
                 PVV_FS(6);
                 {
                     const bool last = it + 1 >= nmine;
+                    const int lstar_now = last ? 0 : read_lstar();
                     bool keep[2];
                     int w[2];
                     unsigned long long m[2];
@@ -387,7 +478,7 @@
                                 if (dmiss) atomicAdd(&miss_k[h], dmiss);
                             } else {
                                 const int seen = atomicAdd(&miss_k[h], dmiss) + dmiss;
-                                keep[q] = cnt_k[h] + R_rem - lstar - seen >= 0;
+                                keep[q] = cnt_k[h] + R_rem - lstar_now - seen >= 0;
                             }
                         }
                         m[q] = __ballot(keep[q]);
@@ -421,7 +512,7 @@
             __syncthreads();
             for (int i = threadIdx.x; i < ns; i += kBlock) {
                 const int v = sCnt[i];
-                if (v & 0xffff) atomicAdd(&cnt_k[gp0 * GH + (int)((unsigned)v >> 16)], v & 0xffff);
+                if (v & 0xffff) atomicAdd(&ext_k[gp0 * GH + (int)((unsigned)v >> 16)], v & 0xffff);
             }
             PVV_FS(8);
         }
diff --git a/clean-pvnet_amd/csrc/count_prune.hpp b/clean-pvnet_amd/csrc/count_prune.hpp
--- a/clean-pvnet_amd/csrc/count_prune.hpp
+++ b/clean-pvnet_amd/csrc/count_prune.hpp
@@ -10,11 +10,56 @@
     const int *any_staged;
     int K, hn, cap;
     int hstride;
-    float kappa, beta, eps;
+    float kappa, beta2, eps0;
     int nsplit;
 };
 
 constexpr int kLead = 2;
+
+__device__ __forceinline__ void lead_pick(int (&lc)[4], int (&li)[4])
+{
+#pragma unroll
+    for (int i = 0; i < kLead; ++i)
+#pragma unroll
+        for (int j = 3; j > i; --j)
+            if (lc[j] > lc[j - 1] || (lc[j] == lc[j - 1] && li[j] < li[j - 1])) {
+                const int tc = lc[j], ti = li[j];
+                lc[j] = lc[j - 1]; li[j] = li[j - 1]; lc[j - 1] = tc; li[j - 1] = ti;
+            }
+}
+
+struct LeadTest {
+    float kappa, beta, eps;
+    float2 ld[kLead];
+    bool lnear[kLead];
+};
+__device__ __forceinline__ LeadTest lead_test(float kappa, float beta2, float eps0, const int (&lc)[4], const int (&li)[4], const float2 *hyp_k)
+{
+    LeadTest t;
+    t.kappa = kappa; t.beta = 2.f * beta2; t.eps = 2.f * eps0;
+#pragma unroll
+    for (int w = 0; w < kLead; ++w) {
+        t.ld[w] = lc[w] >= 0 ? hyp_k[li[w]] : make_float2(0.f, 0.f);
+        t.lnear[w] = lc[w] >= 0 && fabsf(t.ld[w].x) < 1e15f && fabsf(t.ld[w].y) < 1e15f;
+    }
+    return t;
+}
+__device__ __forceinline__ void lead_sure(const LeadTest &t, float2 c, float2 d, int (&inl)[kLead])
+{
+    const float dd = d.x * d.x + d.y * d.y;
+    const bool ok = dd > 4e-12f && dd < INFINITY;
+    const float r = __builtin_amdgcn_rsqf(dd);
+    const float nx = d.x * r, ny = d.y * r;
+    const float bx = -t.kappa * ny, by = t.kappa * nx;
+#pragma unroll
+    for (int w = 0; w < kLead; ++w) {
+        const float dx = t.ld[w].x - c.x, dy = t.ld[w].y - c.y;
+        const float av = __builtin_fmaf(dx, nx, dy * ny);
+        const float bv = __builtin_fmaf(dx, bx, dy * by);
+        const float tv = av - fabsf(bv);
+        inl[w] += (ok && t.lnear[w] && tv > 0.f && __builtin_fmaf(-t.beta, av, tv) > t.eps) ? 1 : 0;
+    }
+}
 
 template <uint32_t FIRST>
 __global__ __launch_bounds__(kBlock) void k_lead(LeadArgs a)
@@ -35,16 +80,25 @@
     const float2 *crd = a.coords + (size_t)b * a.cap;
     const float2 *dir = a.dirs + (size_t)bk * a.cap;
     float2 cc[kTrip], dd_[kTrip];
+    auto next_rest = [](int c) {
+        ++c;
+#pragma unroll
+        for (int k = 0; k < kStageM - 1; ++k) c += (int)((FIRST >> ((unsigned)c % kStageM)) & 1u);
+        return c;
+    };
     auto load_trip = [&](int r0) {
+        int c = stage_chunk_at<REST>(r0 / PC), off = r0 & (PC - 1);
 #pragma unroll
         for (int u = 0; u < kTrip; ++u) {
             const int r = r0 + u * kBlock;
             cc[u] = dd_[u] = make_float2(0.f, 0.f);
             if (r < r1) {
-                const int p = stage_chunk_at<REST>(r / PC) * PC + (r & (PC - 1));
+                const int p = c * PC + off;
                 cc[u] = crd[p];
                 dd_[u] = dir[p];
             }
+            off += kBlock;
+            if (off >= PC) { off -= PC; c = next_rest(c); }
         }
     };
     int r0 = split * per + threadIdx.x;
@@ -61,17 +115,8 @@
     int lc[4], li[4];
 #pragma unroll
     for (int w = 0; w < 4; ++w) { lc[w] = s_cnt[w]; li[w] = s_idx[w]; }
-#pragma unroll
-    for (int i = 0; i < kLead; ++i)
-#pragma unroll
-        for (int j = 3; j > i; --j)
-            if (lc[j] > lc[j - 1] || (lc[j] == lc[j - 1] && li[j] < li[j - 1])) {
-                const int tc = lc[j], ti = li[j];
-                lc[j] = lc[j - 1]; li[j] = li[j - 1]; lc[j - 1] = tc; li[j - 1] = ti;
-            }
-    float2 ld[kLead];
-#pragma unroll
-    for (int w = 0; w < kLead; ++w) ld[w] = lc[w] >= 0 ? a.hyps[(size_t)bk * a.hstride + li[w]] : make_float2(0.f, 0.f);
+    lead_pick(lc, li);
+    const LeadTest lt = lead_test(a.kappa, a.beta2, a.eps0, lc, li, a.hyps + (size_t)bk * a.hstride);
     if (split == 0 && threadIdx.x < 4) {
         int v = -1;
 #pragma unroll
@@ -79,26 +124,11 @@
         a.lead[(size_t)bk * 8 + threadIdx.x] = v;
     }
     int inl[kLead];
-    bool lnear[kLead];
 #pragma unroll
-    for (int w = 0; w < kLead; ++w) { inl[w] = 0; lnear[w] = lc[w] >= 0 && fabsf(ld[w].x) < 1e15f && fabsf(ld[w].y) < 1e15f; }
+    for (int w = 0; w < kLead; ++w) inl[w] = 0;
     for (;;) {
 #pragma unroll
-        for (int u = 0; u < kTrip; ++u) {
-            const float dd = dd_[u].x * dd_[u].x + dd_[u].y * dd_[u].y;
-            const bool ok = dd > 4e-12f && dd < INFINITY;
-            const float r = __builtin_amdgcn_rsqf(dd);
-            const float nx = dd_[u].x * r, ny = dd_[u].y * r;
-            const float bx = -a.kappa * ny, by = a.kappa * nx;
-#pragma unroll
-            for (int w = 0; w < kLead; ++w) {
-                const float dx = ld[w].x - cc[u].x, dy = ld[w].y - cc[u].y;
-                const float av = __builtin_fmaf(dx, nx, dy * ny);
-                const float bv = __builtin_fmaf(dx, bx, dy * by);
-                const float t = av - fabsf(bv);
-                inl[w] += (ok && lnear[w] && t > 0.f && __builtin_fmaf(-a.beta, av, t) > a.eps) ? 1 : 0;
-            }
-        }
+        for (int u = 0; u < kTrip; ++u) lead_sure(lt, cc[u], dd_[u], inl);
         r0 += kTrip * kBlock;
         if (r0 - (int)threadIdx.x >= r1) break;
         load_trip(r0);
diff --git a/clean-pvnet_amd/csrc/covariance.hpp b/clean-pvnet_amd/csrc/covariance.hpp
--- a/clean-pvnet_amd/csrc/covariance.hpp
+++ b/clean-pvnet_amd/csrc/covariance.hpp
@@ -2,6 +2,7 @@
 
 __global__ __launch_bounds__(kBlock) void k_covariance(
     const int *__restrict__ tn_arr, const float2 *__restrict__ hyps, const int *__restrict__ counts,
+    const int *__restrict__ extra ,
     const float2 *__restrict__ mean, float *__restrict__ cov ,
     float2 *__restrict__ hyp_out , int *__restrict__ counts_out,
     float *__restrict__ weights , int K, int hn, int hstride ,
@@ -15,10 +16,12 @@
     const float2 m = mean[bk];
     const float2 *hp = hyps + (size_t)bk * hstride + hoff;
     const int *cp = counts + (size_t)bk * hstride + hoff;
+    const int *ep = extra ? extra + (size_t)bk * hstride + hoff : nullptr;
+    auto count_of = [&](int h) { return cp[h] + (ep ? ep[h] : 0); };
     if (hyp_out || counts_out)
         for (int h = threadIdx.x; h < hn; h += kBlock) {
             if (hyp_out) hyp_out[(size_t)bk * hn + h] = tn > 0 ? hp[h] : make_float2(0.f, 0.f);
-            if (counts_out) counts_out[(size_t)bk * hn + h] = tn > 0 ? cp[h] : 0;
+            if (counts_out) counts_out[(size_t)bk * hn + h] = tn > 0 ? count_of(h) : 0;
         }
     double sxx = 0, sxy = 0, syy = 0, sw = 0;
     if (tn <= 0) {
@@ -28,7 +31,7 @@
         }
     } else {
         int mx = 0;
-        for (int h = threadIdx.x; h < hn; h += kBlock) mx = max(mx, cp[h]);
+        for (int h = threadIdx.x; h < hn; h += kBlock) mx = max(mx, count_of(h));
         mx = wave_max(mx);
         __syncthreads();
         if (lane_id() == 0) redi[threadIdx.x >> 6] = mx;
@@ -37,7 +40,7 @@
         const float ftn = (float)tn;
         const float thr = (float)mx / ftn - 0.1f;
         for (int h = threadIdx.x; h < hn; h += kBlock) {
-            float r = (float)cp[h] / ftn;
+            float r = (float)count_of(h) / ftn;
             if (r < thr) r = 0.f;
             float2 q = hp[h];
             double dx = (double)(q.x - m.x), dy = (double)(q.y - m.y);
diff --git a/clean-pvnet_amd/csrc/pvnet_vote.hip b/clean-pvnet_amd/csrc/pvnet_vote.hip
--- a/clean-pvnet_amd/csrc/pvnet_vote.hip
+++ b/clean-pvnet_amd/csrc/pvnet_vote.hip
@@ -45,8 +45,8 @@
 #include "compaction.hpp"
 #include "count_exact.hpp"
 #include "count_bf16.hpp"
+#include "count_prune.hpp"
 #include "count_filter_runs.hpp"
-#include "count_prune.hpp"
 #include "refit.hpp"
 #include "covariance.hpp"
 #include "legacy_kernels.hpp"
@@ -59,6 +59,7 @@
     size_t lead;
     size_t ratio;
     size_t miss;
+    size_t extra;
 };
 
 bool use_bf16_count(const pvv_problem *p);
@@ -98,6 +99,7 @@
     L.ratio = take(sizeof(float) * (size_t)p->B * p->K);
     L.lead = may_stage(p) ? take(sizeof(int) * 2 * lead_set_words(p)) : 0;
     L.miss = may_stage(p) ? take(sizeof(int) * (size_t)p->B * p->K * p->hn) : 0;
+    L.extra = may_stage(p) ? take(sizeof(int) * (size_t)p->B * p->K * p->hn) : 0;
     L.total = off;
     return L;
 }
@@ -393,9 +395,10 @@
     const int *tn = (const int *)(ws + L.tn);
     int *lead = (int *)(ws + L.lead) + (size_t)a.lead_set * lead_set_words(p);
     StageArgs sa;
-    sa.lead = nullptr;
+    sa.lead = lead;
     sa.any_staged = lead + (size_t)p->B * p->K * 8;
     sa.miss = (int *)(ws + L.miss) + a.col0;
+    sa.extra = (int *)(ws + L.extra) + a.col0;
     sa.sub_tenth = a.sub_tenth;
     sa.hstride = a.hstride;
     sa.mean = (a.sub_tenth && tuning_int("PVV_PROX", 1) != 0) ? (const float2 *)a.mean : nullptr;
@@ -406,11 +409,19 @@
                        p->B, p->K, p->hn, p->cap, p->inlier_thresh, fc, a.target_first, a.dbg, sa);
     if (int e = check_launch("k_count_bf16<first>")) return e;
     if (int e = mark(p, PVV_MARK_STAGE0, st)) return e;
+    const long long rest = p->count_kernel == PVV_COUNT_AUTO ? stage_hint_rest_chunks(p, st, stage_rest_of(FIRST)) : -1;
+    const bool runs = rest < 0 || rest * p->K >= 2ll * a.target_filter || p->hn > 512;
+    if (tuning_int("PVV_FILTER_OLD", runs ? 0 : 1) == 0) {
+        if (int e = mark(p, PVV_MARK_PRUNE0, st)) return e;
+        hipLaunchKernelGGL(k_count_filter_runs<FIRST>, dim3(tuning_int("PVV_GRID_PER_CU_FILTER", 5) * num_cus()), dim3(kBlock), sizeof(int) * (size_t)p->B, st, coords, dirs,
+                           hyps, counts, tn, p->B, p->K, p->hn, p->cap, p->inlier_thresh, fc, a.target_filter, tuning_int("PVV_RUN_R", 0), sa);
+        return check_launch("k_count_filter_runs");
+    }
     LeadArgs la;
     la.tn_arr = tn; la.coords = coords; la.dirs = dirs; la.hyps = hyps; la.counts = counts; la.lead = lead;
     la.K = p->K; la.hn = p->hn; la.cap = p->cap;
     la.hstride = a.hstride > 0 ? a.hstride : p->hn;
-    la.kappa = fc.kappa; la.beta = 2.f * fc.beta2; la.eps = 2.f * fc.eps0;
+    la.kappa = fc.kappa; la.beta2 = fc.beta2; la.eps0 = fc.eps0;
     la.any_staged = sa.any_staged;
     la.nsplit = 16;
     while (la.nsplit > 1 && (long long)p->B * p->K * la.nsplit > 8ll * num_cus()) la.nsplit >>= 1;
@@ -418,14 +429,6 @@
     hipLaunchKernelGGL(k_lead<FIRST>, dim3(p->K * la.nsplit, p->B), dim3(kBlock), 0, st, la);
     if (int e = check_launch("k_lead")) return e;
     if (int e = mark(p, PVV_MARK_PRUNE0, st)) return e;
-    sa.lead = lead;
-    const long long rest = p->count_kernel == PVV_COUNT_AUTO ? stage_hint_rest_chunks(p, st, stage_rest_of(FIRST)) : -1;
-    const bool runs = rest < 0 || rest * p->K >= 2ll * a.target_filter || p->hn > 512;
-    if (tuning_int("PVV_FILTER_OLD", runs ? 0 : 1) == 0) {
-        hipLaunchKernelGGL(k_count_filter_runs<FIRST>, dim3(tuning_int("PVV_GRID_PER_CU_FILTER", 5) * num_cus()), dim3(kBlock), sizeof(int) * (size_t)p->B, st, coords, dirs,
-                           hyps, counts, tn, p->B, p->K, p->hn, p->cap, p->inlier_thresh, fc, a.target_filter, tuning_int("PVV_RUN_R", 0), sa);
-        return check_launch("k_count_filter_runs");
-    }
     hipLaunchKernelGGL((k_count_bf16<kCountFilter, FIRST>), dim3(a.per_cu_filter * num_cus()), dim3(kBlock), 0, st, coords, dirs, hyps, counts, tn,
                        p->B, p->K, p->hn, p->cap, p->inlier_thresh, fc, a.target_filter, a.dbg, sa);
     return check_launch("k_count_bf16<filter>");
@@ -608,6 +611,7 @@
     h.surv = (int *)(ws + L.surv);
     h.lead = L.lead ? (int *)(ws + L.lead) : nullptr;
     h.miss = L.miss ? (int *)(ws + L.miss) : nullptr;
+    h.extra = L.miss ? (int *)(ws + L.extra) : nullptr;
     return f;
 }
 
@@ -721,7 +725,8 @@
               hipStream_t st, int32_t *d_tn, const float *d_seg = nullptr, int64_t *d_mask_out = nullptr,
               const int32_t *d_idxs2 = nullptr, int hn_first = -1, uint32_t stream_first = 1u, uint32_t stream_rest = 3u,
               int stage_kind = 0 , const CountPlan *plan = nullptr,
-              const float *d_mean = nullptr )
+              const float *d_mean = nullptr ,
+              int *staged_out = nullptr )
 {
     if ((p->flags & PVV_FLAG_DEVICE_RNG) && (d_idxs || d_idxs2 || d_selection))
         return fail(PVV_E_ARG, "PVV_FLAG_DEVICE_RNG promises d_idxs = d_idxs_est = d_selection = NULL");
@@ -729,7 +734,8 @@
                          hn_first, stream_first, stream_rest);
     if (f.m.want_draws && L.tile_draw == 0) return fail(PVV_E_WORKSPACE, "workspace holds no draw storage for this call");
     const int staged = plan ? 1 : decide_staged(p, L, st, stage_kind);
-    if (!staged) { f.h.miss = nullptr; f.h.lead = nullptr; }
+    if (!staged) { f.h.miss = nullptr; f.h.extra = nullptr; f.h.lead = nullptr; }
+    if (staged_out) *staged_out = staged;
     if (int e = mark(p, PVV_MARK_BEGIN, st)) return e;
     SideJoin sj;
     SideStream *sg = (f.mask_deferred && tuning_int("PVV_MASK_DEFER", 1) != 0) ? side_get(st) : nullptr;
@@ -863,8 +869,9 @@
 }
 
 static int finish_v3(const pvv_problem *p, const Layout &L, char *ws, float *d_out, int32_t *d_win_counts,
-                     hipStream_t st, int hstride = 0)
-{
+                     hipStream_t st, int staged, int hstride = 0)
+{
+    const int *extra = (staged && L.extra) ? (const int *)(ws + L.extra) : nullptr;
     if (hstride <= 0) hstride = p->hn;
     int nsplit = kRefitSplitMax;
     while (nsplit > 1 && (long long)p->B * p->K * nsplit > 6ll * num_cus()) nsplit >>= 1;
@@ -875,7 +882,7 @@
         hipLaunchKernelGGL(kernel, dim3(p->K * nsplit, p->B), dim3(kBlock), 0, st,
                            (const int *)(ws + L.tn), (const float2 *)(ws + L.coords),
                            (const float2 *)(ws + L.dirs), (const float2 *)(ws + L.hyps),
-                           (const int *)(ws + L.counts), (double *)(ws + L.sums), d_win_counts, p->K, p->hn, hstride,
+                           (const int *)(ws + L.counts), extra, (double *)(ws + L.sums), d_win_counts, p->K, p->hn, hstride,
                            p->cap, p->inlier_thresh, nsplit, (float *)(ws + L.ratio), fc);
     };
     if (band) launch_refit(k_select_refit<true>); else launch_refit(k_select_refit<false>);
@@ -899,9 +906,10 @@
     if (!d_out) return fail(PVV_E_ARG, "d_out is NULL");
     hipStream_t st = (hipStream_t)stream;
     char *ws = (char *)d_workspace;
-    if (int e = run_front(p, 0, d_mask, d_vertex, d_idxs, d_selection, ws, L, st, d_tn, nullptr, nullptr, nullptr, -1, 1u, 3u, 1))
+    int staged = 0;
+    if (int e = run_front(p, 0, d_mask, d_vertex, d_idxs, d_selection, ws, L, st, d_tn, nullptr, nullptr, nullptr, -1, 1u, 3u, 1, nullptr, nullptr, &staged))
         return e;
-    return finish_v3(p, L, ws, d_out, d_win_counts, st);
+    return finish_v3(p, L, ws, d_out, d_win_counts, st, staged);
 }
 
 PVV_EXPORT int pvv_decode_keypoint_v3(const pvv_problem *p, const float *d_seg, const float *d_vertex,
@@ -916,9 +924,10 @@
     if (p->seg_classes < 1 || p->seg_classes > 256) return fail(PVV_E_ARG, "seg_classes must be in [1, 256]");
     hipStream_t st = (hipStream_t)stream;
     char *ws = (char *)d_workspace;
-    if (int e = run_front(p, 0, nullptr, d_vertex, d_idxs, d_selection, ws, L, st, d_tn, d_seg, d_mask_out, nullptr, -1, 1u, 3u, 1))
+    int staged = 0;
+    if (int e = run_front(p, 0, nullptr, d_vertex, d_idxs, d_selection, ws, L, st, d_tn, d_seg, d_mask_out, nullptr, -1, 1u, 3u, 1, nullptr, nullptr, &staged))
         return e;
-    return finish_v3(p, L, ws, d_out, d_win_counts, st);
+    return finish_v3(p, L, ws, d_out, d_win_counts, st, staged);
 }
 
 PVV_EXPORT int pvv_estimate_voting_distribution(const pvv_problem *p, const void *d_mask,
@@ -933,10 +942,12 @@
     if (!d_mean || !d_cov) return fail(PVV_E_ARG, "d_mean / d_cov is NULL");
     hipStream_t st = (hipStream_t)stream;
     char *ws = (char *)d_workspace;
-    if (int e = run_front(p, 1, d_mask, d_vertex, d_idxs, d_selection, ws, L, st, d_tn, nullptr, nullptr, nullptr, -1, 3u, 3u, d_counts ? 0 : 2, nullptr, d_mean)) return e;
+    int staged = 0;
+    if (int e = run_front(p, 1, d_mask, d_vertex, d_idxs, d_selection, ws, L, st, d_tn, nullptr, nullptr, nullptr, -1, 3u, 3u, d_counts ? 0 : 2, nullptr, d_mean, &staged)) return e;
     hipLaunchKernelGGL(k_covariance, dim3(p->K, p->B), dim3(kBlock), 0, st,
                        (const int *)(ws + L.tn), (const float2 *)(ws + L.hyps),
-                       (const int *)(ws + L.counts), (const float2 *)d_mean, d_cov, (float2 *)d_hyp,
+                       (const int *)(ws + L.counts), (staged && L.extra) ? (const int *)(ws + L.extra) : (const int *)nullptr,
+                       (const float2 *)d_mean, d_cov, (float2 *)d_hyp,
                        d_counts, d_weights, p->K, p->hn, p->hn, 0);
     if (int e = check_launch("k_covariance")) return e;
     return mark(p, PVV_MARK_END, st);
@@ -996,7 +1007,7 @@
         if (int e = run_front(&q, 0, nullptr, d_vertex, d_idxs, d_selection, ws, L, st, d_tn, d_seg, d_mask_out, d_idxs_est,
                               p->hn, 1u, 3u, 0, &plan))
             return e;
-        if (int e = finish_v3(p, L, ws, d_kpt, d_win_counts, st, q.hn)) return e;
+        if (int e = finish_v3(p, L, ws, d_kpt, d_win_counts, st, 1, q.hn)) return e;
         CountCols ec;
         ec.col0 = p->hn; ec.hstride = q.hn; ec.lead_set = 1; ec.mean = d_kpt;
         if (int e = launch_count_any(&pe, L, ws, st, est_staged, ec)) return e;
@@ -1004,10 +1015,11 @@
         if (int e = run_front(&q, 0, nullptr, d_vertex, d_idxs, d_selection, ws, L, st, d_tn, d_seg, d_mask_out, d_idxs_est,
                               p->hn))
             return e;
-        if (int e = finish_v3(p, L, ws, d_kpt, d_win_counts, st, q.hn)) return e;
+        if (int e = finish_v3(p, L, ws, d_kpt, d_win_counts, st, 0, q.hn)) return e;
     }
     hipLaunchKernelGGL(k_covariance, dim3(p->K, p->B), dim3(kBlock), 0, st, (const int *)(ws + L.tn),
-                       (const float2 *)(ws + L.hyps), (const int *)(ws + L.counts), (const float2 *)d_kpt, d_cov,
+                       (const float2 *)(ws + L.hyps), (const int *)(ws + L.counts),
+                       (est_staged && L.extra) ? (const int *)(ws + L.extra) : (const int *)nullptr, (const float2 *)d_kpt, d_cov,
                        (float2 *)nullptr, (int *)nullptr, d_weights, p->K, (int)hn_est, q.hn, p->hn);
     if (int e = check_launch("k_covariance")) return e;
     return PVV_OK;
@@ -1029,6 +1041,7 @@
         hipError_t e = hipMemsetAsync(ws + L.counts, 0, sizeof(int) * (size_t)p->B * p->K * p->hn, st);
         if (e == hipSuccess && L.lead) e = hipMemsetAsync(ws + L.lead, 0, sizeof(int) * lead_set_words(p), st);
         if (e == hipSuccess && L.miss) e = hipMemsetAsync(ws + L.miss, 0, sizeof(int) * (size_t)p->B * p->K * p->hn, st);
+        if (e == hipSuccess && L.extra) e = hipMemsetAsync(ws + L.extra, 0, sizeof(int) * (size_t)p->B * p->K * p->hn, st);
         if (e != hipSuccess) return fail((int)e, hipGetErrorString(e));
     }
     return launch_count_any(p, L, ws, st, decide_staged(p, L, st, v3));
diff --git a/clean-pvnet_amd/csrc/refit.hpp b/clean-pvnet_amd/csrc/refit.hpp
--- a/clean-pvnet_amd/csrc/refit.hpp
+++ b/clean-pvnet_amd/csrc/refit.hpp
@@ -6,7 +6,8 @@
 __global__ __launch_bounds__(kBlock) void k_select_refit(
     const int *__restrict__ tn_arr, const float2 *__restrict__ coords,
     const float2 *__restrict__ dirs, const float2 *__restrict__ hyps,
-    const int *__restrict__ counts, double *__restrict__ sums ,
+    const int *__restrict__ counts, const int *__restrict__ extra ,
+    double *__restrict__ sums ,
     int *__restrict__ win_counts , int K, int hn, int hstride ,
     int cap, float thresh, int nsplit, float *__restrict__ win_ratio ,
     Bf16Consts fc )
@@ -26,9 +27,10 @@
         return;
     }
     const int *cp = counts + (size_t)bk * hstride;
+    const int *ep = extra ? extra + (size_t)bk * hstride : nullptr;
     int best = -1, besti = 0x7fffffff;
     for (int h = threadIdx.x; h < hn; h += kBlock) {
-        int c = cp[h];
+        int c = cp[h] + (ep ? ep[h] : 0);
         if (c > best) { best = c; besti = h; }
     }
     wave_argmax_first(best, besti);
```

Result: slower. 318,600 images/s (-3.4%).
